# zhizdev/mvdfusion

Measured on AMD Instinct MI355X. Metric: denoising-steps/sec, higher is better.
Workload: dtype f16x3 (f16 MFMA operands split hi+lo, 3 partial products, fp32 accumulate); 1 GPU; BASELINE.json configs[1]: V=4 views x 256^2 images (32x32 latents), D=1, 50-step DDIM (eta 1), cfg 2.5, SD1.x UNet 320ch + 10 view-aligned transformers + GridAttn, random-init (deterministic fill) weights; views=4, latent=32, depth_samples=1, parallelism=single GPU, CFG pair batched as 2V, hipgraph=True, gemm_tuning=mvdfusion_amd/tuned/gemm_f16.json: 426 problems; 0 problems tuned in this run

## Files before the change

include/mvd_hip.h:

```cpp
#ifndef MVD_HIP_H
#define MVD_HIP_H
#include <stddef.h>
#include <stdint.h>
#ifdef __cplusplus
extern "C" {
#endif

typedef void* mvd_stream_t;

#define MVD_VERSION 100
#define MVD_PREC_X1 1
#define MVD_PREC_X3 3
#define MVD_PREC_X4 4

int mvd_version(void);
const char* mvd_last_error(void);
int mvd_operand_format(void);

size_t mvd_packed_weight_bytes(int N, int K);
int mvd_pack_linear_weight(const float* w, int N, int K, int ldw, int geglu, float scale, void* packed,
                           mvd_stream_t stream);
int mvd_pack_linear_weight_t(const float* wt, int N, int K, int ldw, float scale, void* packed, mvd_stream_t stream);
int mvd_pack_conv3x3_weight(const float* w, int Cout, int Cin, int cin_pad, float scale, void* packed,
                            mvd_stream_t stream);
// ... 51 lines not shown
  int ldr;
  void *q_hi, *q_lo, *k_hi, *k_lo, *vt_hi, *vt_lo;
  int heads, dhead, L, Lpad;
  float qscale;
  int splitk;
  float* workspace;
  size_t workspace_elems;
  int cfg;
  long long* gn_stats;
  int gn_hw, gn_groups;
  float* rs_out;
  int* rs_count;
  int rs_ld;
  const float* ln_stats;
  const int* ln_count;
  const float* ln_colsum;
  int ln_ld, ln_dim;
  float ln_eps;
  void* gna_out_sp;
  const float* gna_gamma;
  const float* gna_beta;
  float gna_eps;
  int gna_flags;
  const float* cat_b;
  int cat_cb;
  void* cat_raw_sp;
  const float* acc_scale_dev;
  const struct mvd_prefetch_item_s* pf_items;
  int pf_n;
  int tap_mode;
  const void* A2;
  int lda2, Cin2;
} mvd_gemm_desc;
#define MVD_TAPS_FULL 0
#define MVD_TAPS_UP4 1
#define MVD_TAPS_CENTRE_TAIL 2
#define MVD_GNA_SILU 1
#define MVD_GNA_ROUND_F16 2
#define MVD_GNA_OUT_UNUSED 4

int mvd_gemm(const mvd_gemm_desc* d, mvd_stream_t stream);
int mvd_gemm_cfg_supported(const mvd_gemm_desc* d, int cfg);

int mvd_split_planes(const float* x, void* sp, size_t rows, int cols, int ldx, int ldp, mvd_stream_t stream);
int mvd_split_planes_scaled(const float* x, void* sp, size_t rows, int cols, int ldx, int ldp, const float* scale_dev, mvd_stream_t stream);

int mvd_gemv(const float* W, const float* bias, const float* x, float* y, int M, int N, int K, int ldx, int ldy,
             int act_in, int act_out, mvd_stream_t stream);

int mvd_groupnorm_chunks(int HW);
int mvd_groupnorm_nhwc(const float* x, void* y_sp, const float* gamma, const float* beta, int B, int HW, int C,
                       int groups, float eps, int silu, double* ws, size_t ws_elems, mvd_stream_t stream);
int mvd_groupnorm_from_stats(const float* x, void* y_sp, const float* gamma, const float* beta, const long long* stats, int B, int HW,
                             int C, int groups, float eps, int silu, mvd_stream_t stream);
int mvd_softmax_rows(const float* x, void* y_sp, int rows, int cols, int ldx, float scale, float out_scale,
                     mvd_stream_t stream);

int mvd_layernorm(const float* x, void* y_sp, float* y_f32, const float* w, const float* b, int rows, int C, float eps,
                  int w_plus_one, mvd_stream_t stream);
int mvd_layernorm_groups(const float* x, void* y_sp, float* y_f32, const float* w, const float* b, int ldw, int rows, int rows_per_group,
                         int C, float eps, int w_plus_one, mvd_stream_t stream);

size_t mvd_attn_qk_plane_elems(int B, int heads, int L, int dhead);
size_t mvd_attn_vt_plane_elems(int B, int heads, int L, int dhead);
int mvd_attn_lpad(int L);
int mvd_attention(const void* q_hi, const void* q_lo, const void* k_hi, const void* k_lo, const void* vt_hi,
                  const void* vt_lo, void* out_sp, int ldo, int B, int heads, int L, int Lkeys, int dhead, int prec,
                  mvd_stream_t stream);

int mvd_pixel_cross_attn(const float* q, const float* k, const float* v, void* out_sp, int P, int D, int heads,
                         int dhead, mvd_stream_t stream);

int mvd_unet_input(const float* x, const float* input_latents, void* out_sp, int V, int S, int cpad, int cfg,
                   mvd_stream_t stream);
int mvd_unet_input_scenes(const float* x, const float* input_latents, void* out_sp, int nscene, int V, int S, int cpad, int cfg,
                          mvd_stream_t stream);
int mvd_concat_channels(const float* a, int Ca, const float* b, int Cb, float* out, void* out_sp, int rows, long long* gn_stats,
                        int gn_hw, int gn_groups, mvd_stream_t stream);
int mvd_concat_groupnorm_fits(int Ca, int Cb, int hw, int groups);
int mvd_concat_groupnorm(const float* a, int Ca, const float* b, int Cb, float* out, void* raw_sp, void* y_sp, const float* gamma,
                         const float* beta, long long* gn_stats, int B, int hw, int groups, float eps, int silu, mvd_stream_t stream);
int mvd_area_pool(const float* vol, void* out_sp, int B, int S, int D, int C, int factor, int ldp, mvd_stream_t stream);
int mvd_fill_zero(float* p, size_t n, mvd_stream_t stream);

#define MVD_STEP_STRIDE 8
int mvd_timestep_embedding(const float* steps, const int* iter, const float* freqs, float* out, int dim,
                           mvd_stream_t stream);
int mvd_timestep_embedding_scenes(const float* steps, const int* iter, const float* freqs, float* out, int dim, int nscene,
                                  int steps_scene_stride, mvd_stream_t stream);
int mvd_advance_iter(int* iter, mvd_stream_t stream);

#define MVD_CAM_RECORD 20
#define MVD_TOKEN_DIM 723
#define MVD_TOKEN_LD 736
int mvd_zembed(const float* lat, const float* w, const float* b, float* feat, int N, int S, mvd_stream_t stream);
int mvd_gridattn_tokens(const float* x, const float* depth_noise, const float* steps, const int* iter,
                        const float* grid_lin ,
                        const float* feat, const float* in_feat, const float* cams, const float* in_cam,
                        void* tokens_sp, int V, int q0, int Vq, int S, int D, float depth_scale, float depth_shift,
                        mvd_stream_t stream);
int mvd_gridattn_tokens_scenes(const float* x, const float* depth_noise, const float* steps, const int* iter, const float* grid_lin,
                               const float* feat, const float* in_feat, const float* cams, const float* in_cam, void* tokens_sp,
                               int nscene, int V, int q0, int Vq, int S, int D, float depth_scale, float depth_shift,
                               mvd_stream_t stream);
int mvd_gridattn_tokens_scenes_t(const float* x, const float* depth_noise, const float* steps, const int* iter, const float* grid_lin,
                                 const float* feat, const float* in_feat, const float* cams, const float* in_cam, void* tokens_sp,
                                 int nscene, int V, int q0, int Vq, int S, int D, float depth_scale, float depth_shift,
                                 int steps_scene_stride, mvd_stream_t stream);
int mvd_gridattn_fused_slots(void);
size_t mvd_gridattn_fused_stream_bytes(void);
size_t mvd_gridattn_fused_vec_floats(void);
int mvd_gridattn_fused(const float* x, const float* depth_noise, const float* steps, const int* iter, const float* grid_lin,
                       const float* feat, const float* in_feat, const float* cams, const float* in_cam, const void* wstream,
                       const float* vecs, void* pooled_sp, int V, int q0, int Vq, int S, int D, float depth_scale,
                       float depth_shift, int prec ,
                       mvd_stream_t stream);
int mvd_gridattn_fused_scenes(const float* x, const float* depth_noise, const float* steps, const int* iter, const float* grid_lin,
                              const float* feat, const float* in_feat, const float* cams, const float* in_cam, const void* wstream,
                              const float* vecs, void* pooled_sp, int nscene, int V, int q0, int Vq, int S, int D, float depth_scale,
                              float depth_shift, int prec, mvd_stream_t stream);
int mvd_gridattn_fused_scenes_t(const float* x, const float* depth_noise, const float* steps, const int* iter, const float* grid_lin,
                                const float* feat, const float* in_feat, const float* cams, const float* in_cam, const void* wstream,
                                const float* vecs, void* pooled_sp, int nscene, int V, int q0, int Vq, int S, int D, float depth_scale,
                                float depth_shift, int prec, int steps_scene_stride, int vecs_scene_stride, mvd_stream_t stream);
int mvd_gridattn_tokens_window(const float* x, const float* depth_noise, const float* steps, const int* iter, const float* grid_lin,
                               const float* feat, const float* in_feat, const float* cams, const float* in_cam, void* tokens_sp,
                               int nscene, int V, int q0, int Vq, int S, int D, float depth_scale, float depth_shift,
                               int steps_scene_stride, int window, mvd_stream_t stream);
int mvd_gridattn_fused_window(const float* x, const float* depth_noise, const float* steps, const int* iter, const float* grid_lin,
                              const float* feat, const float* in_feat, const float* cams, const float* in_cam, const void* wstream,
                              const float* vecs, void* pooled_sp, int nscene, int V, int q0, int Vq, int S, int D, float depth_scale,
                              float depth_shift, int prec, int steps_scene_stride, int vecs_scene_stride, int window,
                              mvd_stream_t stream);
int mvd_view_mha(const float* qkv, void* out_sp, int Nseq, int V, int heads, int dhead,
                 mvd_stream_t stream);
int mvd_view_pool(const float* x, const float* w, const float* b, void* out_sp, int Nseq, int V, int C,
                  mvd_stream_t stream);

int mvd_cfg_ddim_update(const float* eps_nhwc, int ldc, float* x, float* x0, float* eps_out,
                        const float* ddim_noise, size_t noise_stride ,
                        const float* steps, const int* iter, int V, int S, int cfg, float cfg_scale, int do_update,
                        mvd_stream_t stream);

int mvd_pin_views(float* x, float* x0, const float* known, const float* noise, size_t noise_stride ,
                  const float* steps, const int* iter, int groups, int group_views, int K, int S, int mode, mvd_stream_t stream);

#define MVD_FUSE_FOREGROUND 1
#define MVD_FUSE_STAGE_AUTO 0
#define MVD_FUSE_STAGE_GLOBAL 1
#define MVD_FUSE_STAGE_LDS 2
int mvd_fuse_points(const float* lat, const float* rgb, const float* cams, const float* ndc_lin, float* xyz, float* color,
                    uint8_t* support, uint8_t* conflict, uint8_t* flags, int nscene, int V, int S, int up, float depth_scale,
                    float depth_shift, float lo, float hi, float tau, int stage, mvd_stream_t stream);
size_t mvd_compact_points_scratch(size_t npts);
int mvd_compact_points(const float* xyz, const float* color, const uint8_t* support, const uint8_t* conflict, const uint8_t* flags,
                       size_t npts, int min_support, int max_conflicts, float* out_xyz, float* out_color, uint8_t* out_support,
                       int* out_index, unsigned* count, void* scratch, size_t scratch_bytes, mvd_stream_t stream);

int mvd_graph_begin(mvd_stream_t stream);
int mvd_graph_end(mvd_stream_t stream, void** graph_exec);
int mvd_graph_launch(void* graph_exec, mvd_stream_t stream);
int mvd_graph_destroy(void* graph_exec);
int mvd_event_create(void** ev);
int mvd_event_record(void* ev, mvd_stream_t stream);
int mvd_event_elapsed_ms(void* start, void* stop, float* ms);
int mvd_event_destroy(void* ev);
// ... 49 lines not shown
```

mvdfusion_amd/csrc/elementwise.hip:

```cpp
#include "common.hpp"
#include "../../include/mvd_hip.h"

namespace {

__device__ __forceinline__ float act_apply(float v, int act) {
  if (act == MVD_ACT_GELU) return gelu_erf(v);
  if (act == MVD_ACT_SILU) return silu_f(v);
  return v;
}

template <int MR>
__global__ __launch_bounds__(256) void gemv_kernel(const float* __restrict__ W, const float* __restrict__ bias,
                                                   const float* __restrict__ x, float* __restrict__ y, int M, int N, int K, int ldx,
                                                   int ldy, int act_in, int act_out) {
  const int lane = threadIdx.x & 63;
  const int n = blockIdx.x * 4 + (threadIdx.x >> 6);
  if (n >= N) return;
  float acc[MR];
#pragma unroll
  for (int m = 0; m < MR; ++m) acc[m] = 0.f;
  const float* wr = W + (size_t)n * K;
  if ((K & 3) == 0) {
    for (int k = lane * 4; k < K; k += 256) {
      const float4 w4 = *(const float4*)(wr + k);
#pragma unroll
      for (int m = 0; m < MR; ++m) {
        if (m < M) {
          float4 x4 = *(const float4*)(x + (size_t)m * ldx + k);
          if (act_in) {
            x4.x = act_apply(x4.x, act_in);
            x4.y = act_apply(x4.y, act_in);
            x4.z = act_apply(x4.z, act_in);
            x4.w = act_apply(x4.w, act_in);
          }
          acc[m] += w4.x * x4.x + w4.y * x4.y + w4.z * x4.z + w4.w * x4.w;
        }
      }
    }
  } else {
    for (int k = lane; k < K; k += 64) {
      const float w1 = wr[k];
#pragma unroll
      for (int m = 0; m < MR; ++m)
        if (m < M) acc[m] += w1 * act_apply(x[(size_t)m * ldx + k], act_in);
    }
  }
#pragma unroll
  for (int m = 0; m < MR; ++m) {
    if (m < M) {
      float v = wave_sum(acc[m]);
      if (lane == 0) {
        if (bias) v += bias[n];
        y[(size_t)m * ldy + n] = act_apply(v, act_out);
      }
    }
  }
}

__global__ __launch_bounds__(256) void unet_input_kernel(const float* __restrict__ x, const float* __restrict__ il,
                                                         u16* __restrict__ out_sp, int V, int Vs, int S, int cpad, int nb) {
  const int SS = S * S;
  const size_t total = (size_t)nb * SS * cpad;
  for (size_t e = (size_t)blockIdx.x * 256 + threadIdx.x; e < total; e += (size_t)gridDim.x * 256) {
    const int c = (int)(e % cpad);
    const int pix = (int)((e / cpad) % SS);
    const int b = (int)(e / ((size_t)cpad * SS));
    const int v = b < V ? b : b - V;
    float o = 0.f;
    if (c < 5) {
      o = x[((size_t)v * 5 + c) * SS + pix];
    } else if (c < 10 && b < V) {
      const float t = il[((size_t)(b / Vs) * 5 + (c - 5)) * SS + pix];
      o = (c < 9) ? t / 0.18215f : t;
    }
    store_sp1(out_sp, e / cpad, cpad, c, o);
  }
}

__global__ __launch_bounds__(256) void concat_kernel(const float4* __restrict__ a, int ca4, const float4* __restrict__ b, int cb4,
                                                     float4* __restrict__ out, u16* __restrict__ out_sp, size_t rows) {
  const int c4 = ca4 + cb4;
  const size_t total = rows * c4;
  for (size_t e = (size_t)blockIdx.x * 256 + threadIdx.x; e < total; e += (size_t)gridDim.x * 256) {
    const size_t r = e / c4;
    const int c = (int)(e - r * c4);
    const float4 v = c < ca4 ? a[r * ca4 + c] : b[r * cb4 + (c - ca4)];
    out[e] = v;
    if (out_sp) store_sp4(out_sp, r, c4 * 4, c * 4, v.x, v.y, v.z, v.w);
  }
}

__global__ __launch_bounds__(256) void concat_stats_kernel(const float4* __restrict__ a, int ca4, const float4* __restrict__ b, int cb4,
                                                           float4* __restrict__ out, u16* __restrict__ out_sp, long long* __restrict__ stats,
                                                           int hw, int groups) {
  __shared__ float cs[2][4][256];
  const int c4n = ca4 + cb4, C = c4n * 4;
  const size_t m0 = (size_t)blockIdx.x * 16;
  const int n0 = blockIdx.y * 256;
  const int c4 = blockIdx.y * 64 + (threadIdx.x & 63), rg = threadIdx.x >> 6;
  float4 s = make_float4(0.f, 0.f, 0.f, 0.f), q = make_float4(0.f, 0.f, 0.f, 0.f);
  if (c4 < c4n) {
    float4 v[4];
#pragma unroll
    for (int r = 0; r < 4; ++r) {
      const size_t row = m0 + rg * 4 + r;
      v[r] = c4 < ca4 ? a[row * ca4 + c4] : b[row * cb4 + (c4 - ca4)];
    }
#pragma unroll
    for (int r = 0; r < 4; ++r) {
      const size_t row = m0 + rg * 4 + r;
      out[row * c4n + c4] = v[r];
      if (out_sp) store_sp4(out_sp, row, C, c4 * 4, v[r].x, v[r].y, v[r].z, v[r].w);
      s.x += v[r].x; s.y += v[r].y; s.z += v[r].z; s.w += v[r].w;
      q.x += v[r].x * v[r].x; q.y += v[r].y * v[r].y; q.z += v[r].z * v[r].z; q.w += v[r].w * v[r].w;
    }
  }
  *(float4*)&cs[0][rg][(threadIdx.x & 63) * 4] = s;
  *(float4*)&cs[1][rg][(threadIdx.x & 63) * 4] = q;
  __syncthreads();
  const int c = threadIdx.x, nn = n0 + c;
  const float cs_ = cs[0][0][c] + cs[0][1][c] + cs[0][2][c] + cs[0][3][c];
  const float cq_ = cs[1][0][c] + cs[1][1][c] + cs[1][2][c] + cs[1][3][c];
  __syncthreads();
  cs[0][0][c] = cs_;
  cs[1][0][c] = cq_;
  __syncthreads();
  if (nn >= C) return;
  const int cg = C / groups;
  const int g = nn / cg, pos = nn - g * cg;
  if (c != 0 && pos != 0) return;
  int len = cg - pos;
  if (len > 256 - c) len = 256 - c;
  float ss = 0.f, qq = 0.f;
  for (int j = 0; j < len; ++j) {
    ss += cs[0][0][c + j];
    qq += cs[1][0][c + j];
  }
  gn_stats_add(stats, (int)(m0 / hw), g, groups, ss, qq);
}

#define MVD_CGN_THREADS 1024
__global__ __launch_bounds__(MVD_CGN_THREADS) void concat_gn_kernel(const float* __restrict__ a, int ca, const float* __restrict__ b, int cb,
                                                                    float* __restrict__ out, u16* __restrict__ raw_sp, u16* __restrict__ y_sp,
                                                                    const float* __restrict__ gamma, const float* __restrict__ beta,
                                                                    long long* __restrict__ stats, int hw, int groups, float eps, int flags) {
  constexpr int NT = MVD_CGN_THREADS, NWV = NT / 64, U = 4;
  extern __shared__ float s_val[];
  __shared__ double s_red[2][NWV];
  __shared__ float s_coef[2][128];
  const int C = ca + cb, cg = C / groups, cg2 = cg >> 1;
  int g, img;
  {
    const int bid = blockIdx.x;
    if ((groups & 7) == 0) {
      const int gpx = groups >> 3, x = bid & 7, r = bid >> 3;
      g = x * gpx + r % gpx;
      img = r / gpx;
    } else {
      g = bid % groups;
// ... 27 lines not shown
        }
      }
#pragma unroll
      for (int u = 0; u < U; ++u) {
        const size_t m = m0 + rr[u];
        const int n = c0 + 2 * jj[u];
        v[u] = *(const float2*)(n < ca ? a + m * ca + n : b + m * cb + (n - ca));
      }
#pragma unroll
      for (int u = 0; u < U; ++u) {
        if (ok[u]) {
          const size_t m = m0 + rr[u];
          const int n = c0 + 2 * jj[u];
          if (out) *(float2*)(out + m * C + n) = v[u];
          if (raw_sp) {
            uint32_t hh, ll;
            split_op16x2(v[u].x, v[u].y, hh, ll);
            u16* pp = raw_sp + sp_index(m, C, n);
            *(uint32_t*)pp = hh;
            *(uint32_t*)(pp + 32) = ll;
          }
          *(float2*)(s_val + 2 * (e0 + u * NT)) = v[u];
          s += v[u].x + v[u].y;
          q += v[u].x * v[u].x + v[u].y * v[u].y;
        }
      }
    }
  }
  {
    const double sd = wave_sum_d((double)s), qd = wave_sum_d((double)q);
    if (lane == 0) {
      s_red[0][wave] = sd;
      s_red[1][wave] = qd;
    }
  }
  __syncthreads();
  double S1 = 0.0, S2 = 0.0;
#pragma unroll
  for (int w = 0; w < NWV; ++w) {
    S1 += s_red[0][w];
    S2 += s_red[1][w];
  }
  const double cnt = (double)hw * cg;
  const double mean = S1 / cnt;
  double var = S2 / cnt - mean * mean;
  if (var < 0.0) var = 0.0;
  const float rstd = (float)(1.0 / sqrt(var + (double)eps));
  if (tid < cg) {
    const float aa = rstd * gamma[c0 + tid];
    s_coef[0][tid] = aa;
    s_coef[1][tid] = beta[c0 + tid] - (float)mean * aa;
  }
  if (tid == 0 && stats) gn_stats_add(stats, img, g, groups, (float)S1, (float)S2);
  __syncthreads();
  {
    int r = rs, j = js;
    for (int e = tid; e < total; e += NT) {
      float2 v = *(const float2*)(s_val + 2 * e);
      v.x = v.x * s_coef[0][2 * j] + s_coef[1][2 * j];
      v.y = v.y * s_coef[0][2 * j + 1] + s_coef[1][2 * j + 1];
      if (flags & 2) {
        v.x = (float)(_Float16)v.x;
        v.y = (float)(_Float16)v.y;
      }
      if (flags & 1) {
        v.x = silu_f(v.x);
        v.y = silu_f(v.y);
      }
      uint32_t hh, ll;
      split_op16x2(v.x, v.y, hh, ll);
      u16* pp = y_sp + sp_index(m0 + r, C, c0 + 2 * j);
      *(uint32_t*)pp = hh;
      *(uint32_t*)(pp + 32) = ll;
      r += dq;
      j += dj;
      if (j >= cg2) {
        j -= cg2;
        ++r;
      }
    }
  }
}

__global__ __launch_bounds__(256) void area_pool_kernel(const float4* __restrict__ vol, u16* __restrict__ out_sp, int B, int S,
                                                        int D, int C4, int f, int ldp) {
  const int So = S / f;
  const size_t total = (size_t)B * So * So * D * C4;
  const float inv = 1.0f / (float)(f * f);
  for (size_t e = (size_t)blockIdx.x * 256 + threadIdx.x; e < total; e += (size_t)gridDim.x * 256) {
    const int c = (int)(e % C4);
    size_t r = e / C4;
    const int d = (int)(r % D);
    r /= D;
    const int ox = (int)(r % So);
    r /= So;
    const int oy = (int)(r % So);
    const int b = (int)(r / So);
    float4 acc = make_float4(0.f, 0.f, 0.f, 0.f);
    for (int dy = 0; dy < f; ++dy)
#pragma unroll 8
      for (int dx = 0; dx < f; ++dx) {
        const float4 v = vol[((((size_t)b * S + oy * f + dy) * S + ox * f + dx) * D + d) * C4 + c];
        acc.x += v.x;
        acc.y += v.y;
        acc.z += v.z;
        acc.w += v.w;
      }
    store_sp4(out_sp, e / C4, ldp, c * 4, acc.x * inv, acc.y * inv, acc.z * inv, acc.w * inv);
  }
}

__global__ __launch_bounds__(256) void fill_zero_kernel(float* p, size_t n) {
  for (size_t e = (size_t)blockIdx.x * 256 + threadIdx.x; e < n; e += (size_t)gridDim.x * 256) p[e] = 0.f;
}

__global__ void timestep_embedding_kernel(const float* __restrict__ steps, const int* __restrict__ iter,
                                          const float* __restrict__ freqs, float* __restrict__ out, int dim, int steps_scene_stride) {
  const float t = steps[((size_t)iter[0] + (size_t)blockIdx.x * steps_scene_stride) * MVD_STEP_STRIDE + 0];
  out += (size_t)blockIdx.x * dim;
  const int half = dim / 2;
  for (int i = threadIdx.x; i < half; i += blockDim.x) {
    const float a = t * freqs[i];
    out[i] = cosf(a);
    out[half + i] = sinf(a);
  }
}

__global__ void advance_iter_kernel(int* iter) {
  if (threadIdx.x == 0) iter[0] += 1;
}

__global__ __launch_bounds__(256) void cfg_ddim_kernel(const float* __restrict__ eps_nhwc, int ldc, float* __restrict__ x,
                                                       float* __restrict__ x0, float* __restrict__ eps_out,
                                                       const float* __restrict__ noise, const float* __restrict__ steps,
                                                       const int* __restrict__ iter, int V, int S, int cfg, float cfg_scale,
                                                       int do_update, size_t noise_stride) {
  const int it = iter[0];
  const float* st = steps + (size_t)it * MVD_STEP_STRIDE;
  const float a_t = st[3], a_prev = st[4], sigma = st[5], s1m = st[6], has_noise = st[7];
  const int SS = S * S;
  const size_t total = (size_t)V * 5 * SS;
  for (size_t e = (size_t)blockIdx.x * 256 + threadIdx.x; e < total; e += (size_t)gridDim.x * 256) {
    const int pix = (int)(e % SS);
    const int c = (int)((e / SS) % 5);
    const int b = (int)(e / ((size_t)5 * SS));
    float ep = eps_nhwc[((size_t)b * SS + pix) * ldc + c];
    if (cfg) {
      const float eu = eps_nhwc[((size_t)(V + b) * SS + pix) * ldc + c];
      ep = eu + cfg_scale * (ep - eu);
    }
    if (eps_out) eps_out[e] = ep;
    if (do_update) {
      const float xv = x[e];
      const float px0 = (xv - s1m * ep) / sqrtf(a_t);
      const float dir = sqrtf(fmaxf(1.0f - a_prev - sigma * sigma, 1e-7f)) * ep;
      float xp = sqrtf(a_prev) * px0 + dir;
      if (has_noise != 0.f) xp = xp + sigma * noise[(size_t)it * noise_stride + e];
      x0[e] = px0;
      x[e] = xp;
    }
  }
}

template <typename T>
__device__ __forceinline__ T pin_axpy(float sa, const T& k, float s1, const T& n);
template <>
__device__ __forceinline__ float pin_axpy<float>(float sa, const float& k, float s1, const float& n) {
  return sa * k + s1 * n;
}
template <>
__device__ __forceinline__ float4 pin_axpy<float4>(float sa, const float4& k, float s1, const float4& n) {
  return make_float4(sa * k.x + s1 * n.x, sa * k.y + s1 * n.y, sa * k.z + s1 * n.z, sa * k.w + s1 * n.w);
}

template <typename T>
__global__ __launch_bounds__(256) void pin_views_kernel(T* __restrict__ x, T* __restrict__ x0, const T* __restrict__ known,
                                                        const T* __restrict__ noise, size_t nstride, const float* __restrict__ steps,
                                                        const int* __restrict__ iter, int group_views, int K, size_t rowlen, size_t total,
                                                        int mode) {
  float sa = 1.f, s1 = 0.f;
  size_t nbase = 0;
  if (mode == 1) {
    const int it = iter[0];
    const float* st = steps + (size_t)it * MVD_STEP_STRIDE;
    sa = st[1];
    s1 = st[6];
    nbase = (size_t)it * nstride;
  }
  for (size_t e = (size_t)blockIdx.x * 256 + threadIdx.x; e < total; e += (size_t)gridDim.x * 256) {
    const size_t p = e / rowlen;
    const size_t off = e - p * rowlen;
    const size_t dst = ((p / K) * group_views + p % K) * rowlen + off;
    const T kv = known[e];
    if (mode == 1) {
      x[dst] = pin_axpy<T>(sa, kv, s1, noise[nbase + e]);
      x0[dst] = kv;
// ... 33 lines not shown
  MVD_CHECK_ARG(x && input_latents && out_sp && cpad % 32 == 0 && V > 0 && S > 0 && cpad >= 10, "mvd_unet_input: bad arguments");
  MVD_CHECK_ARG(nscene >= 1 && (long long)nscene * V <= 0x3fffffff, "mvd_unet_input_scenes: nscene=%d (>= 1)", nscene);
  const int NV = nscene * V;
  const int nb = cfg ? 2 * NV : NV;
  const size_t total = (size_t)nb * S * S * cpad;
  hipLaunchKernelGGL(unet_input_kernel, dim3(grid_for(total)), dim3(256), 0, (hipStream_t)stream, x, input_latents, (u16*)out_sp, NV, V,
                     S, cpad, nb);
  MVD_CHECK_LAUNCH("mvd_unet_input");
  return 0;
}

extern "C" int mvd_unet_input(const float* x, const float* input_latents, void* out_sp, int V, int S, int cpad, int cfg,
                              mvd_stream_t stream) {
  return mvd_unet_input_scenes(x, input_latents, out_sp, 1, V, S, cpad, cfg, stream);
}

extern "C" int mvd_concat_channels(const float* a, int Ca, const float* b, int Cb, float* out, void* out_sp, int rows,
                                   long long* gn_stats, int gn_hw, int gn_groups, mvd_stream_t stream) {
  if (out_sp) MVD_CHECK_ARG((Ca + Cb) % 32 == 0, "mvd_concat_channels: split-planes output needs (Ca+Cb) %% 32 == 0");
  MVD_CHECK_ARG(a && b && out && rows > 0 && Ca > 0 && Cb > 0 && Ca % 4 == 0 && Cb % 4 == 0,
                "mvd_concat_channels: bad arguments (channel counts must be multiples of 4)");
  if (gn_stats) {
    MVD_CHECK_ARG(rows % 16 == 0 && gn_hw > 0 && gn_hw % 16 == 0 && gn_groups > 0 && (Ca + Cb) % gn_groups == 0,
                  "mvd_concat_channels: gn_stats needs rows %% 16 == 0, gn_hw %% 16 == 0, C %% groups == 0");
    hipLaunchKernelGGL(concat_stats_kernel, dim3(rows / 16, (Ca + Cb + 255) / 256), dim3(256), 0, (hipStream_t)stream, (const float4*)a, Ca / 4,
                       (const float4*)b, Cb / 4, (float4*)out, (u16*)out_sp, gn_stats, gn_hw, gn_groups);
    MVD_CHECK_LAUNCH("mvd_concat_channels/stats");
    return 0;
  }
  const size_t total = (size_t)rows * (Ca + Cb) / 4;
  hipLaunchKernelGGL(concat_kernel, dim3(grid_for(total)), dim3(256), 0, (hipStream_t)stream, (const float4*)a, Ca / 4,
                     (const float4*)b, Cb / 4, (float4*)out, (u16*)out_sp, (size_t)rows);
  MVD_CHECK_LAUNCH("mvd_concat_channels");
  return 0;
}

extern "C" int mvd_concat_groupnorm_fits(int Ca, int Cb, int hw, int groups) {
  const int C = Ca + Cb;
  if (groups <= 0 || C % groups || (Ca & 1) || (Cb & 1)) return 0;
  const int cg = C / groups;
  return (cg & 1) == 0 && cg <= 128 && (size_t)hw * cg * 4 <= 128 * 1024 ? 1 : 0;
}

extern "C" int mvd_concat_groupnorm(const float* a, int Ca, const float* b, int Cb, float* out, void* raw_sp, void* y_sp, const float* gamma,
                                    const float* beta, long long* gn_stats, int B, int hw, int groups, float eps, int silu,
                                    mvd_stream_t stream) {
  MVD_CHECK_ARG(a && b && y_sp && gamma && beta && B > 0 && hw > 0, "mvd_concat_groupnorm: null pointer / bad shape");
  MVD_CHECK_ARG((Ca + Cb) % 32 == 0 && mvd_concat_groupnorm_fits(Ca, Cb, hw, groups),
                "mvd_concat_groupnorm: needs (Ca+Cb) %% 32 == 0, even Ca / Cb / group width <= 128 and hw * (C / groups) * 4 <= 128 KiB of LDS "
                "(Ca=%d Cb=%d hw=%d groups=%d): use mvd_concat_channels + mvd_groupnorm_from_stats", Ca, Cb, hw, groups);
  MVD_CHECK_ARG(((uintptr_t)a & 7) == 0 && ((uintptr_t)b & 7) == 0 && ((uintptr_t)out & 7) == 0 && ((uintptr_t)y_sp & 127) == 0 &&
                    ((uintptr_t)raw_sp & 127) == 0, "mvd_concat_groupnorm: alignment");
  const size_t lds = (size_t)hw * ((Ca + Cb) / groups) * 4;
  {
    static unsigned long long raised = 0;
    const hipError_t e = mvd_raise_dynamic_lds((const void*)concat_gn_kernel, 128 * 1024, &raised);
    MVD_CHECK_ARG(e == hipSuccess, "mvd_concat_groupnorm: hipFuncSetAttribute(MaxDynamicSharedMemorySize): %s", hipGetErrorString(e));
  }
  hipLaunchKernelGGL(concat_gn_kernel, dim3(B * groups), dim3(MVD_CGN_THREADS), lds, (hipStream_t)stream, a, Ca, b, Cb, out, (u16*)raw_sp,
                     (u16*)y_sp, gamma, beta, gn_stats, hw, groups, eps, silu);
  MVD_CHECK_LAUNCH("mvd_concat_groupnorm");
  return 0;
}

extern "C" int mvd_area_pool(const float* vol, void* out_sp, int B, int S, int D, int C, int factor, int ldp,
                             mvd_stream_t stream) {
  MVD_CHECK_ARG(vol && out_sp && C % 32 == 0 && B > 0 && S > 0 && D > 0 && C % 4 == 0 && factor >= 1 && S % factor == 0,
                "mvd_area_pool: bad arguments");
  if (ldp == 0) ldp = C;
  MVD_CHECK_ARG(ldp >= C && ldp % 32 == 0 && ((uintptr_t)out_sp & 127) == 0, "mvd_area_pool: ldp=%d must be >= C, %% 32 == 0", ldp);
  const int So = S / factor;
  const size_t total = (size_t)B * So * So * D * (C / 4);
  hipLaunchKernelGGL(area_pool_kernel, dim3(grid_for(total)), dim3(256), 0, (hipStream_t)stream, (const float4*)vol,
                     (u16*)out_sp, B, S, D, C / 4, factor, ldp);
  MVD_CHECK_LAUNCH("mvd_area_pool");
  return 0;
}

extern "C" int mvd_fill_zero(float* p, size_t n, mvd_stream_t stream) {
  MVD_CHECK_ARG(p != nullptr, "mvd_fill_zero: null pointer");
  if (n == 0) return 0;
  hipLaunchKernelGGL(fill_zero_kernel, dim3(grid_for(n)), dim3(256), 0, (hipStream_t)stream, p, n);
  MVD_CHECK_LAUNCH("mvd_fill_zero");
  return 0;
}

extern "C" int mvd_timestep_embedding(const float* steps, const int* iter, const float* freqs, float* out, int dim,
                                      mvd_stream_t stream) {
  MVD_CHECK_ARG(steps && iter && freqs && out && dim > 0 && dim % 2 == 0, "mvd_timestep_embedding: bad arguments");
  hipLaunchKernelGGL(timestep_embedding_kernel, dim3(1), dim3(256), 0, (hipStream_t)stream, steps, iter, freqs, out, dim, 0);
  MVD_CHECK_LAUNCH("mvd_timestep_embedding");
  return 0;
}

extern "C" int mvd_timestep_embedding_scenes(const float* steps, const int* iter, const float* freqs, float* out, int dim, int nscene,
                                             int steps_scene_stride, mvd_stream_t stream) {
  MVD_CHECK_ARG(steps && iter && freqs && out && dim > 0 && dim % 2 == 0, "mvd_timestep_embedding: bad arguments");
  MVD_CHECK_ARG(nscene >= 1 && nscene <= 65535 && steps_scene_stride >= 0 && (nscene > 1 || steps_scene_stride == 0),
                "mvd_timestep_embedding_scenes: nscene=%d (1 ... 65535), steps_scene_stride=%d (>= 0; 0 when nscene = 1)", nscene,
                steps_scene_stride);
  hipLaunchKernelGGL(timestep_embedding_kernel, dim3(nscene), dim3(256), 0, (hipStream_t)stream, steps, iter, freqs, out, dim,
                     steps_scene_stride);
  MVD_CHECK_LAUNCH("mvd_timestep_embedding_scenes");
  return 0;
}

extern "C" int mvd_advance_iter(int* iter, mvd_stream_t stream) {
  MVD_CHECK_ARG(iter != nullptr, "mvd_advance_iter: null pointer");
  hipLaunchKernelGGL(advance_iter_kernel, dim3(1), dim3(64), 0, (hipStream_t)stream, iter);
  MVD_CHECK_LAUNCH("mvd_advance_iter");
  return 0;
}

extern "C" int mvd_cfg_ddim_update(const float* eps_nhwc, int ldc, float* x, float* x0, float* eps_out,
                                   const float* ddim_noise, size_t noise_stride, const float* steps, const int* iter, int V,
                                   int S, int cfg, float cfg_scale, int do_update, mvd_stream_t stream) {
  MVD_CHECK_ARG(eps_nhwc && steps && iter && V > 0 && S > 0 && ldc >= 5, "mvd_cfg_ddim_update: bad arguments");
  if (do_update) MVD_CHECK_ARG(x && x0 && ddim_noise, "mvd_cfg_ddim_update: update needs x, x0, ddim_noise");
  const size_t total = (size_t)V * 5 * S * S;
  hipLaunchKernelGGL(cfg_ddim_kernel, dim3(grid_for(total)), dim3(256), 0, (hipStream_t)stream, eps_nhwc, ldc, x, x0, eps_out,
                     ddim_noise, steps, iter, V, S, cfg, cfg_scale, do_update, noise_stride);
  MVD_CHECK_LAUNCH("mvd_cfg_ddim_update");
  return 0;
}

extern "C" int mvd_pin_views(float* x, float* x0, const float* known, const float* noise, size_t noise_stride, const float* steps,
                             const int* iter, int groups, int group_views, int K, int S, int mode, mvd_stream_t stream) {
  MVD_CHECK_ARG(x && known && groups > 0 && group_views > 0 && S > 0 && (mode == 0 || mode == 1),
                "mvd_pin_views: bad arguments (null x / known, groups=%d, group_views=%d, S=%d, mode=%d)", groups, group_views, S, mode);
  MVD_CHECK_ARG(K > 0 && K <= group_views, "mvd_pin_views: K=%d pinned views of a %d-view group (0 < K <= group_views)", K, group_views);
  MVD_CHECK_ARG((long long)groups * group_views <= 0x3fffffff, "mvd_pin_views: groups * group_views too large");
  const size_t row = (size_t)5 * S * S;
  if (mode == 1)
    MVD_CHECK_ARG(x0 && noise && steps && iter && noise_stride >= (size_t)groups * K * row,
                  "mvd_pin_views: mode 1 needs x0, noise, steps, iter and noise_stride >= groups * K * 5 * S * S");
  const size_t total = (size_t)groups * K * row;
  hipStream_t s = (hipStream_t)stream;
  if (((size_t)S * S) % 4 == 0) {
    MVD_CHECK_ARG(((uintptr_t)x & 15) == 0 && ((uintptr_t)known & 15) == 0, "mvd_pin_views: x / known must be 16-byte aligned");
    if (mode == 1)
      MVD_CHECK_ARG(((uintptr_t)x0 & 15) == 0 && ((uintptr_t)noise & 15) == 0 && noise_stride % 4 == 0,
                    "mvd_pin_views: x0 / noise must be 16-byte aligned and noise_stride a multiple of 4");
    hipLaunchKernelGGL(pin_views_kernel<float4>, dim3(grid_for(total / 4)), dim3(256), 0, s, (float4*)x, (float4*)x0, (const float4*)known,
                       (const float4*)noise, noise_stride / 4, steps, iter, group_views, K, row / 4, total / 4, mode);
  } else {
    hipLaunchKernelGGL(pin_views_kernel<float>, dim3(grid_for(total)), dim3(256), 0, s, x, x0, known, noise, noise_stride, steps, iter,
                       group_views, K, row, total, mode);
  }
  MVD_CHECK_LAUNCH("mvd_pin_views");
  return 0;
}
```

mvdfusion_amd/csrc/gemm.hip:

```cpp
#include "gemm_device.hpp"

namespace {

__global__ __launch_bounds__(256) void splitk_reduce_kernel(GemmParams p) {
  const mvd_gemm_desc& d = p.d;
  const size_t MN = (size_t)d.M * d.N;
  if (d.epi == MVD_EPI_GEGLU) {
    const size_t total = (size_t)d.M * (d.N >> 1);
    for (size_t e = (size_t)blockIdx.x * 256 + threadIdx.x; e < total; e += (size_t)gridDim.x * 256) {
      const int m = (int)(e / (d.N >> 1));
      const int col = (int)(e - (size_t)m * (d.N >> 1));
      const int pv = (col >> 4) * 32 + (col & 15);
      float v = 0.f, g = 0.f;
      for (int z = 0; z < p.splits; ++z) {
        v += d.workspace[z * MN + (size_t)m * d.N + pv];
        g += d.workspace[z * MN + (size_t)m * d.N + pv + 16];
      }
      epi_geglu_elem(d, m, pv, v, g);
    }
    return;
  }
  if (d.epi == MVD_EPI_STORE) {
    const size_t MN4 = MN >> 2;
    const float inv = 1.0f / gemm_acc_scale(d);
// ... 138 lines not shown
  const int rs = tid / cg2, js = tid - rs * cg2;
  const int r0 = tid < total ? rs : 0, j0 = tid < total ? js : 0;
  const float* const zero2 = (const float*)g_zero_page;
  const bool has_bias = d.bias != nullptr, has_bb = d.bias_b != nullptr, has_res = d.res != nullptr;
  const float ascale = gemm_acc_scale(d);
  float s = 0.f, q = 0.f;
  {
    int r = rs, j = js;
    for (int e0 = tid; e0 < total; e0 += NT * U) {
      int rr[U], jj[U];
      bool ok[U];
#pragma unroll
      for (int u = 0; u < U; ++u) {
        ok[u] = e0 + u * NT < total;
        rr[u] = ok[u] ? r : r0;
        jj[u] = ok[u] ? j : j0;
        r += dq;
        j += dj;
        if (j >= cg2) {
          j -= cg2;
          ++r;
        }
      }
      float2 acc[U], tb[U], tbb[U], tr[U];
      float2 t[ZC][U];
      const int nz0 = p.splits < ZC ? p.splits : ZC;
      bool own[U];
      float2 tc[U];
#pragma unroll
      for (int u = 0; u < U; ++u) {
        const int m = m0 + rr[u], nn = c0 + 2 * jj[u];
        own[u] = nn < d.N;
        const int n = own[u] ? nn : 0;
        tb[u] = *(const float2*)(has_bias ? d.bias + n : zero2);
        tbb[u] = *(const float2*)(has_bb ? d.bias_b + (size_t)(m / d.rows_per_batch) * d.ldbb + n : zero2);
        tr[u] = *(const float2*)(has_res ? d.res + (size_t)m * d.ldr + n : zero2);
        tc[u] = *(const float2*)(own[u] ? zero2 : d.cat_b + (size_t)m * d.cat_cb + (nn - d.N));
#pragma unroll
        for (int z = 0; z < ZC; ++z) {
          const float* w = d.workspace + (size_t)(z < nz0 ? z : 0) * MN + (size_t)m * d.N + n;
          t[z][u] = *(const float2*)w;
        }
      }
#pragma unroll
      for (int u = 0; u < U; ++u) {
        acc[u] = make_float2(0.f, 0.f);
#pragma unroll
        for (int z = 0; z < ZC; ++z)
          if (z < nz0) {
            acc[u].x += t[z][u].x;
            acc[u].y += t[z][u].y;
          }
      }
      for (int zb = ZC; zb < p.splits; zb += ZC) {
        const int nz = p.splits - zb < ZC ? p.splits - zb : ZC;
#pragma unroll
        for (int u = 0; u < U; ++u) {
          const int m = m0 + rr[u], n = own[u] ? c0 + 2 * jj[u] : 0;
#pragma unroll
          for (int z = 0; z < ZC; ++z) t[z][u] = *(const float2*)(d.workspace + (size_t)(zb + (z < nz ? z : 0)) * MN + (size_t)m * d.N + n);
        }
#pragma unroll
        for (int u = 0; u < U; ++u)
#pragma unroll
          for (int z = 0; z < ZC; ++z)
            if (z < nz) {
              acc[u].x += t[z][u].x;
              acc[u].y += t[z][u].y;
            }
      }
#pragma unroll
      for (int u = 0; u < U; ++u) {
        float2 v = acc[u];
        v.x = v.x * ascale + tb[u].x + tbb[u].x + tr[u].x;
        v.y = v.y * ascale + tb[u].y + tbb[u].y + tr[u].y;
        if (!own[u]) v = tc[u];
        if (ok[u]) {
          const int m = m0 + rr[u], n = c0 + 2 * jj[u];
          if (put_out && own[u]) *(float2*)(d.out + (size_t)m * d.ldo + n) = v;
          if (d.cat_raw_sp) {
            uint32_t hh, ll;
            split_op16x2(v.x, v.y, hh, ll);
            u16* pp = (u16*)d.cat_raw_sp + sp_index((size_t)m, CT, n);
            *(uint32_t*)pp = hh;
            *(uint32_t*)(pp + 32) = ll;
          }
          *(float2*)(s_val + 2 * (e0 + u * NT)) = v;
          s += v.x + v.y;
          q += v.x * v.x + v.y * v.y;
        }
      }
    }
  }
  unsigned pf_sink = 0;
  if (d.pf_items != nullptr) {
    const __attribute__((address_space(4))) mvd_prefetch_item* tab = (const __attribute__((address_space(4))) mvd_prefetch_item*)d.pf_items;
    const int gw = blockIdx.x * NWV + wave, GW = gridDim.x * NWV;
    for (int it = 0; it < d.pf_n; ++it) {
      const unsigned char* base = (const unsigned char*)tab[it].ptr;
      const long lines = (long)((tab[it].bytes + 127) >> 7);
      for (long l = (long)gw * 64 + lane; l < lines; l += (long)GW * 64) {
        const unsigned char* a = base + (l << 7);
        asm volatile("global_load_dword %0, %1, off" : "+v"(pf_sink) : "v"(a) : "memory");
      }
    }
  }
  {
    const double sd = wave_sum_d((double)s), qd = wave_sum_d((double)q);
    if (lane == 0) {
      s_red[0][wave] = sd;
      s_red[1][wave] = qd;
    }
  }
  __syncthreads();
  double S1 = 0.0, S2 = 0.0;
#pragma unroll
  for (int w = 0; w < NWV; ++w) {
    S1 += s_red[0][w];
    S2 += s_red[1][w];
  }
  const double cnt = (double)HW * cg;
  const double mean = S1 / cnt;
  double var = S2 / cnt - mean * mean;
  if (var < 0.0) var = 0.0;
  const float rstd = (float)(1.0 / sqrt(var + (double)d.gna_eps));
  if (tid < cg) {
    const float a = rstd * d.gna_gamma[c0 + tid];
    s_coef[0][tid] = a;
    s_coef[1][tid] = d.gna_beta[c0 + tid] - (float)mean * a;
  }
  if (tid == 0 && d.gn_stats) gn_stats_add(d.gn_stats, b, g, G, (float)S1, (float)S2);
  __syncthreads();
  u16* const ysp = (u16*)d.gna_out_sp;
  const int fl = d.gna_flags;
  {
    int r = rs, j = js;
    for (int e = tid; e < total; e += NT) {
      float2 v = *(const float2*)(s_val + 2 * e);
      v.x = v.x * s_coef[0][2 * j] + s_coef[1][2 * j];
      v.y = v.y * s_coef[0][2 * j + 1] + s_coef[1][2 * j + 1];
      if (fl & MVD_GNA_ROUND_F16) {
        v.x = (float)(_Float16)v.x;
        v.y = (float)(_Float16)v.y;
      }
      if (fl & MVD_GNA_SILU) {
        v.x = silu_f(v.x);
        v.y = silu_f(v.y);
      }
      uint32_t hh, ll;
      split_op16x2(v.x, v.y, hh, ll);
      u16* pp = ysp + sp_index((size_t)(m0 + r), CT, c0 + 2 * j);
      *(uint32_t*)pp = hh;
      *(uint32_t*)(pp + 32) = ll;
      r += dq;
      j += dj;
      if (j >= cg2) {
        j -= cg2;
        ++r;
      }
    }
  }
  asm volatile("" ::"v"(pf_sink));
}

struct TileInfo {
  int bm, bn, waves;
// ... 143 lines not shown
  }
  if (d.gn_stats)
    MVD_CHECK_ARG(d.epi == MVD_EPI_STORE && d.n_store == d.N && d.M % 16 == 0 && d.gn_hw > 0 && d.gn_hw % 16 == 0 && d.gn_groups > 0 &&
                      d.N % d.gn_groups == 0,
                  "mvd_gemm: gn_stats needs MVD_EPI_STORE, n_store == N, M %% 16 == 0, gn_hw %% 16 == 0, N %% gn_groups == 0 (N=%d M=%d hw=%d)",
                  d.N, d.M, d.gn_hw);
  if (d.gna_out_sp)
    MVD_CHECK_ARG(d.gn_stats && d.out && d.ldo == d.N && d.gna_gamma && d.gna_beta && d.N % 32 == 0 && d.M % d.gn_hw == 0 &&
                      ((uintptr_t)d.gna_out_sp & 127) == 0,
                  "mvd_gemm: gna_out_sp (GroupNorm apply behind the GEMM) needs gn_stats, out with ldo == N, gamma / beta, N %% 32 == 0, M %% gn_hw == 0");
  if (d.cat_b)
    MVD_CHECK_ARG(d.gna_out_sp && d.cat_cb > 0 && d.cat_cb % 2 == 0 && (d.N + d.cat_cb) % 32 == 0 && (d.N + d.cat_cb) % d.gn_groups == 0 &&
                      ((uintptr_t)d.cat_b & 7) == 0 && ((uintptr_t)d.cat_raw_sp & 127) == 0 &&
                      mvd_concat_groupnorm_fits(d.N, d.cat_cb, d.gn_hw, d.gn_groups),
                  "mvd_gemm: cat_b (GroupNorm over [out | cat_b]) needs gna_out_sp, an even cat_cb, (N + cat_cb) %% 32 == 0 and a shape "
                  "mvd_concat_groupnorm_fits() accepts (N=%d cat_cb=%d hw=%d)", d.N, d.cat_cb, d.gn_hw);
  long long* const gna_stats = d.gn_stats;
  if (d.cat_b) d.gn_stats = nullptr;
  if (d.b_mode == MVD_B_PLANES)
    MVD_CHECK_ARG(d.ldb >= d.K && d.ldb % 32 == 0, "mvd_gemm: B planes need ldb=%d >= K=%d, a multiple of 32", d.ldb, d.K);
  else
    MVD_CHECK_ARG(d.b_mode == MVD_B_PACKED, "mvd_gemm: bad b_mode %d", d.b_mode);
  if (d.acc_scale == 0.f) d.acc_scale = 1.f;
  p.nk = d.K / 32;
  p.nt16 = d.N / 16;
  int tile, loop = 0, order = -1;
  MVD_CHECK_ARG(d.cfg >= 0 && d.cfg <= MVD_GEMM_CFG_STRIDE * MVD_GEMM_TILES, "mvd_gemm: bad cfg %d", d.cfg);
  if (d.cfg >= 1) {
    tile = (d.cfg - 1) / MVD_GEMM_CFG_STRIDE;
    loop = ((d.cfg - 1) % MVD_GEMM_CFG_STRIDE) >> 1;
    order = (d.cfg - 1) & 1;
    MVD_CHECK_ARG(cfg_supported(d, d.cfg), "mvd_gemm: cfg %d (tile %d, loop %d) does not serve this problem (include/mvd_hip.h: cfg)", d.cfg, tile,
                  loop);
  } else {
    const long tiles128 = (long)cdiv(d.M, 128) * cdiv(d.N, 128);
    tile = (tiles128 >= 128 && (d.N >= 512 || d.K >= 2048)) ? 1 : 0;
  }
  const TileInfo& ti = kTiles[tile];
  p.tiles_n = cdiv(d.N, ti.bn);
  p.tiles_m = cdiv(d.M, ti.bm);
  const bool up4 = d.a_mode == MVD_A_CONV3X3 && d.tap_mode == MVD_TAPS_UP4;
  if (up4) {
    p.up4_mq = d.B * d.Hin * d.Win;
    p.up4_tpp = cdiv(p.up4_mq, ti.bm);
    p.tiles_m = 4 * p.up4_tpp;
  }
  if (order < 0) {
    const int est_tm = up4 ? p.up4_tpp : p.tiles_m;
    const double W = (double)d.N * d.K * 4.0;
    const double A = (double)(up4 ? p.up4_mq : d.M) * d.K * 4.0 / (d.a_mode == MVD_A_CONV3X3 ? (up4 ? 4.0 : 9.0) : 1.0);
    const double rep_m = est_tm < 8 ? est_tm : 8, rep_n = p.tiles_n < 8 ? p.tiles_n : 8;
    order = (W + A * rep_n) < (W * rep_m + A) ? 1 : 0;
  }
  p.m_fastest = order;
  int splits = d.splitk;
  const long tiles = (long)p.tiles_m * p.tiles_n;
  if (splits == 0) splits = choose_splits(tiles, p.nk, ti, loop, (size_t)d.M * d.N);
  if (splits < 1) splits = 1;
  if (splits > p.nk) splits = p.nk;
  if (splits > 1) {
    if (d.workspace == nullptr) splits = 1;
    else {
      const size_t cap = d.workspace_elems / ((size_t)d.M * d.N);
      if ((size_t)splits > cap) splits = cap < 1 ? 1 : (int)cap;
    }
  }
  p.kt_per_split = cdiv(p.nk, splits);
  if (loop == 6) p.kt_per_split = 9 * cdiv(p.nk / 9, splits);
  p.splits = cdiv(p.nk, p.kt_per_split);
  hipStream_t s = (hipStream_t)stream;
  bool launched;
  if (loop == 6) launched = mvd_gemm_launch_patch(tile, p, s, patch_shares(d, ti));
  else if (loop == 7) launched = mvd_gemm_launch_ws(tile, p, s);
  else if (tile == 0) launched = mvd_gemm_launch_plain_t0(loop, p, s);
  else if (tile == 1) launched = mvd_gemm_launch_plain_t1(loop, p, s);
  else if (tile == 2) launched = mvd_gemm_launch_plain_t2(loop, p, s);
  else if (tile == 3) launched = mvd_gemm_launch_plain_t3(loop, p, s);
  else launched = mvd_gemm_launch_plain_t4(loop, p, s);
  MVD_CHECK_ARG(launched, "mvd_gemm: no kernel for tile %d loop %d", tile, loop);
  MVD_CHECK_LAUNCH("mvd_gemm");
  const int gna_ct = d.N + (d.cat_b ? d.cat_cb : 0);
  const int gna_cg = d.gna_out_sp ? gna_ct / d.gn_groups : 0;
  const size_t gna_lds = (size_t)d.gn_hw * gna_cg * 4;
  const bool gna_fused = d.gna_out_sp && p.splits > 1 && !d.rs_out && !d.out_sp && !d.colscale && d.act == MVD_ACT_NONE && (gna_cg & 1) == 0 &&
                         gna_cg <= 128 && gna_lds <= 128 * 1024 && d.ldo % 2 == 0 && (!d.res || d.ldr % 2 == 0) && (!d.bias_b || d.ldbb % 2 == 0) &&
                         d.N % 2 == 0;
  if (gna_fused) {
    {
      static unsigned long long raised = 0;
      const hipError_t e = mvd_raise_dynamic_lds((const void*)splitk_gn_kernel, 128 * 1024, &raised);
      MVD_CHECK_ARG(e == hipSuccess, "mvd_gemm: hipFuncSetAttribute(MaxDynamicSharedMemorySize): %s", hipGetErrorString(e));
    }
    p.d.gn_stats = gna_stats;
    if (loop == 7) p.d.pf_items = nullptr;
    hipLaunchKernelGGL(splitk_gn_kernel, dim3((d.M / d.gn_hw) * d.gn_groups), dim3(MVD_GNK_THREADS), gna_lds, s, p);
    MVD_CHECK_LAUNCH("mvd_gemm/splitk_gn");
    return 0;
  }
  if (p.splits > 1) {
    if (d.rs_out) {
      hipLaunchKernelGGL(splitk_reduce_rows_kernel, dim3(cdiv(d.M, 4), cdiv(d.N, 256)), dim3(256), 0, s, p);
    } else if (d.gn_stats) {
      const int spans = (d.N + 255) / 256;
      if ((d.M / 16) * spans >= 1024)
        hipLaunchKernelGGL(splitk_reduce_stats_kernel<4>, dim3(d.M / 16, spans), dim3(256), 0, s, p);
      else
        hipLaunchKernelGGL(splitk_reduce_stats_kernel<2>, dim3(d.M / 8, spans), dim3(256), 0, s, p);
    } else {
      const size_t total = (size_t)d.M * d.N;
      int blocks = (int)((total + 255) / 256);
      if (blocks > 2048) blocks = 2048;
      hipLaunchKernelGGL(splitk_reduce_kernel, dim3(blocks), dim3(256), 0, s, p);
    }
    MVD_CHECK_LAUNCH("mvd_gemm/splitk_reduce");
  }
  if (d.gna_out_sp && d.cat_b)
    return mvd_concat_groupnorm(d.out, d.N, d.cat_b, d.cat_cb, nullptr, d.cat_raw_sp, d.gna_out_sp, d.gna_gamma, d.gna_beta, gna_stats,
                                d.M / d.gn_hw, d.gn_hw, d.gn_groups, d.gna_eps, d.gna_flags & (MVD_GNA_SILU | MVD_GNA_ROUND_F16), stream);
  if (d.gna_out_sp)
    return mvd_groupnorm_from_stats(d.out, d.gna_out_sp, d.gna_gamma, d.gna_beta, d.gn_stats, d.M / d.gn_hw, d.gn_hw, d.N, d.gn_groups,
                                    d.gna_eps, d.gna_flags & (MVD_GNA_SILU | MVD_GNA_ROUND_F16), stream);
  return 0;
}

namespace {
__global__ __launch_bounds__(256) void pack_kernel(const float* __restrict__ w, u16* __restrict__ out, int N, int K,
                                                   int Np, int Kp, int ldw, int geglu, int conv_cin, int trans,
                                                   float scale) {
  const int nt16 = Np >> 4;
  const size_t total = (size_t)(Kp >> 5) * nt16 * 64;
  for (size_t e = (size_t)blockIdx.x * 256 + threadIdx.x; e < total; e += (size_t)gridDim.x * 256) {
    const size_t mt = e >> 6;
    const int l = (int)(e & 63);
    const int kt = (int)(mt / nt16), nt = (int)(mt - (size_t)kt * nt16);
    const int n = nt * 16 + (l & 15);
    const int k = kt * 32 + (l >> 4) * 8;
    int src_n = n;
    if (geglu) {
      const int blk = n >> 5, within = n & 31;
      src_n = within < 16 ? blk * 16 + within : (N >> 1) + blk * 16 + (within - 16);
    }
    float v[8];
#pragma unroll
    for (int j = 0; j < 8; ++j) v[j] = 0.f;
    if (src_n < N) {
      if (conv_cin > 0) {
        const int cb = kt / 9, tap = kt - cb * 9;
        const int ci0 = cb * 32 + (k & 31);
#pragma unroll
        for (int j = 0; j < 8; ++j)
          if (ci0 + j < conv_cin) v[j] = w[((size_t)src_n * conv_cin + ci0 + j) * 9 + tap];
      } else if (trans) {
#pragma unroll
        for (int j = 0; j < 8; ++j)
          if (k + j < K) v[j] = w[(size_t)(k + j) * ldw + src_n];
      } else {
        const float* src = w + (size_t)src_n * ldw + k;
        if (k + 7 < K && (ldw & 3) == 0 && ((uintptr_t)w & 15) == 0) {
          const float4 a = *(const float4*)src, b = *(const float4*)(src + 4);
          v[0] = a.x; v[1] = a.y; v[2] = a.z; v[3] = a.w; v[4] = b.x; v[5] = b.y; v[6] = b.z; v[7] = b.w;
        } else {
#pragma unroll
          for (int j = 0; j < 8; ++j)
            if (k + j < K) v[j] = src[j];
        }
      }
    }
// ... 87 lines not shown
```

mvdfusion_amd/csrc/gridattn.hip:

```cpp
#include "gridattn_common.hpp"

namespace {

__device__ __forceinline__ float harmonic(const float* vec, int dim, int e) {
  const int n = dim * 7;
  if (e >= 2 * n) return vec[e - 2 * n];
  const int ee = e < n ? e : e - n;
  const int di = ee / 7, k = ee - di * 7;
  const float w = 0.1f * (float)(1 << k);
  const float a = vec[di] * w;
  return e < n ? sinf(a) : cosf(a);
}
__device__ __forceinline__ void embed105(const Plucker& pl, float depth, int lane, float& v0, float& v1) {
  const float p6[6] = {pl.a, pl.b, pl.c, pl.d, pl.e, pl.f}, dp[1] = {depth};
  const int e0 = lane, e1 = lane + 64;
  v0 = e0 < 90 ? harmonic(p6, 6, e0) : harmonic(dp, 1, e0 - 90);
  v1 = e1 >= 105 ? 0.f : e1 < 90 ? harmonic(p6, 6, e1) : harmonic(dp, 1, e1 - 90);
}

__global__ __launch_bounds__(256) void tokens_kernel(GridGeom g, const float* __restrict__ feat, const float* __restrict__ in_feat,
                                                     u16* __restrict__ tok) {
  const int lane = threadIdx.x & 63;
  const int S = g.S, SS = S * S, W = slots_per_point(g);
  const size_t pt = (size_t)blockIdx.x * 4 + (threadIdx.x >> 6);
  if (pt >= num_points(g)) return;
  const GeomPoint q = decode_point(g, pt, wave_scene(g, pt));
  const Cam cb = view_cam(g, q, q.b);
  float X[3], dir[3];
  const float depth = world_point(g, q, cb, X, dir);
  float qe0, qe1;
  embed105(plucker(dir[0], dir[1], dir[2], cb.C), depth, lane, qe0, qe1);
  const float4 fin = bilinear4(in_feat + (size_t)q.scene * SS * 256, view_taps(input_cam(g, q), X, S), lane * 4);
  for_each_slot(g, q.b, [&](int slot, int vr) {
    const Cam cv = view_cam(g, q, vr);
    const float4 fr = bilinear4(feat + (size_t)(q.gv0 + vr) * SS * 256, view_taps(cv, X, S), lane * 4);
    const Plucker rpl = plucker_to(cv, X);
    float re0, re1;
    embed105(rpl, rpl.norm, lane, re0, re1);
    const size_t row = pt * W + slot;
    store_sp4(tok, row, MVD_TOKEN_LD, lane * 4, fr.x, fr.y, fr.z, fr.w);
    store_sp4(tok, row, MVD_TOKEN_LD, 256 + lane * 4, fin.x, fin.y, fin.z, fin.w);
    store_sp1(tok, row, MVD_TOKEN_LD, 512 + lane, re0);
    if (lane + 64 < 105) store_sp1(tok, row, MVD_TOKEN_LD, 512 + lane + 64, re1);
    store_sp1(tok, row, MVD_TOKEN_LD, 617 + lane, qe0);
    if (lane + 64 < 105) store_sp1(tok, row, MVD_TOKEN_LD, 617 + lane + 64, qe1);
    if (lane < MVD_TOKEN_LD - 722) store_sp1(tok, row, MVD_TOKEN_LD, 722 + lane, lane == 0 ? 1.0f : 0.0f);
  });
}

__global__ __launch_bounds__(256) void zembed_kernel(const float* __restrict__ lat, const float* __restrict__ w,
                                                     const float* __restrict__ bias, float* __restrict__ feat, int N, int SS) {
  const int lane = threadIdx.x & 63;
  const size_t p = (size_t)blockIdx.x * 4 + (threadIdx.x >> 6);
  if (p >= (size_t)N * SS) return;
  const int n = (int)(p / SS), pix = (int)(p % SS);
  float in[5];
#pragma unroll
  for (int c = 0; c < 5; ++c) in[c] = lat[((size_t)n * 5 + c) * SS + pix];
  float o[4];
#pragma unroll
  for (int j = 0; j < 4; ++j) {
    const int ch = lane * 4 + j;
    float a = 0.f;
#pragma unroll
    for (int c = 0; c < 5; ++c) a += in[c] * w[ch * 5 + c];
    o[j] = gelu_erf(a + bias[ch]);
  }
  *(float4*)(feat + p * 256 + lane * 4) = make_float4(o[0], o[1], o[2], o[3]);
}

__device__ __forceinline__ void scatter4(long long* __restrict__ acc, const Taps& t, int ch, float4 g, float scale) {
#pragma unroll
  for (int k = 0; k < 4; ++k) {
    if (t.pix[k] < 0) continue;
    unsigned long long* p = (unsigned long long*)(acc + (size_t)t.pix[k] * 256 + ch);
    const float w = t.w[k] * scale;
    atomicAdd(p + 0, (unsigned long long)(long long)llrintf(g.x * w));
    atomicAdd(p + 1, (unsigned long long)(long long)llrintf(g.y * w));
    atomicAdd(p + 2, (unsigned long long)(long long)llrintf(g.z * w));
    atomicAdd(p + 3, (unsigned long long)(long long)llrintf(g.w * w));
  }
}

__global__ __launch_bounds__(256) void tokens_bwd_kernel(GridGeom g, const float* __restrict__ dtok, int ldt, long long* __restrict__ dfeat,
                                                         long long* __restrict__ din_feat, float scale) {
  const int lane = threadIdx.x & 63;
  const int S = g.S, SS = S * S, W = slots_per_point(g);
  const size_t pt = (size_t)blockIdx.x * 4 + (threadIdx.x >> 6);
  if (pt >= num_points(g)) return;
  const GeomPoint q = decode_point(g, pt, wave_scene(g, pt));
  float X[3], dir[3];
  world_point(g, q, view_cam(g, q, q.b), X, dir);
  float4 gin = make_float4(0.f, 0.f, 0.f, 0.f);
  for_each_slot(g, q.b, [&](int slot, int vr) {
    const float* row = dtok + (pt * W + slot) * (size_t)ldt;
    const float4 gr = *(const float4*)(row + lane * 4);
    scatter4(dfeat + (size_t)(q.gv0 + vr) * SS * 256, view_taps(view_cam(g, q, vr), X, S), lane * 4, gr, scale);
    const float4 gi = *(const float4*)(row + 256 + lane * 4);
    gin.x += gi.x; gin.y += gi.y; gin.z += gi.z; gin.w += gi.w;
  });
  scatter4(din_feat + (size_t)q.scene * SS * 256, view_taps(input_cam(g, q), X, S), lane * 4, gin, scale);
}

}

extern "C" int mvd_zembed(const float* lat, const float* w, const float* b, float* feat, int N, int S, mvd_stream_t stream) {
  MVD_CHECK_ARG(lat && w && b && feat && N > 0 && S > 0, "mvd_zembed: bad arguments");
  const size_t npix = (size_t)N * S * S;
  hipLaunchKernelGGL(zembed_kernel, dim3(cdiv(npix, 4)), dim3(256), 0, (hipStream_t)stream, lat, w, b, feat, N, S * S);
  MVD_CHECK_LAUNCH("mvd_zembed");
  return 0;
}

extern "C" int mvd_gridattn_tokens_window(const float* x, const float* depth_noise, const float* steps, const int* iter,
                                          const float* grid_lin, const float* feat, const float* in_feat, const float* cams,
                                          const float* in_cam, void* tokens_sp, int nscene, int V, int q0, int Vq, int S, int D,
                                          float depth_scale, float depth_shift, int steps_scene_stride, int window, mvd_stream_t stream) {
  const GridGeom g = {x, depth_noise, steps, iter, grid_lin, cams, in_cam, nscene, V, q0, Vq, S, D, depth_scale, depth_shift, steps_scene_stride, window};
  if (const int e = check_geom("mvd_gridattn_tokens_window", g)) return e;
  MVD_CHECK_ARG(feat && in_feat && tokens_sp, "mvd_gridattn_tokens_window: null pointer");
  const size_t npts = num_points(g);
  MVD_CHECK_ARG((npts + 3) / 4 <= 0x7fffffff, "mvd_gridattn_tokens_window: grid too large");
  hipLaunchKernelGGL(tokens_kernel, dim3(cdiv(npts, 4)), dim3(256), 0, (hipStream_t)stream, g, feat, in_feat, (u16*)tokens_sp);
  MVD_CHECK_LAUNCH("mvd_gridattn_tokens_window");
  return 0;
}

extern "C" int mvd_gridattn_tokens_scenes_t(const float* x, const float* depth_noise, const float* steps, const int* iter,
                                            const float* grid_lin, const float* feat, const float* in_feat, const float* cams,
                                            const float* in_cam, void* tokens_sp, int nscene, int V, int q0, int Vq, int S, int D,
                                            float depth_scale, float depth_shift, int steps_scene_stride, mvd_stream_t stream) {
  return mvd_gridattn_tokens_window(x, depth_noise, steps, iter, grid_lin, feat, in_feat, cams, in_cam, tokens_sp, nscene, V, q0, Vq, S, D,
                                    depth_scale, depth_shift, steps_scene_stride, 0, stream);
}

extern "C" int mvd_gridattn_tokens_scenes(const float* x, const float* depth_noise, const float* steps, const int* iter,
                                          const float* grid_lin, const float* feat, const float* in_feat, const float* cams,
                                          const float* in_cam, void* tokens_sp, int nscene, int V, int q0, int Vq, int S, int D,
                                          float depth_scale, float depth_shift, mvd_stream_t stream) {
  return mvd_gridattn_tokens_scenes_t(x, depth_noise, steps, iter, grid_lin, feat, in_feat, cams, in_cam, tokens_sp, nscene, V, q0, Vq, S,
                                      D, depth_scale, depth_shift, 0, stream);
}

extern "C" int mvd_gridattn_tokens(const float* x, const float* depth_noise, const float* steps, const int* iter,
                                   const float* grid_lin, const float* feat, const float* in_feat, const float* cams,
                                   const float* in_cam, void* tokens_sp, int V, int q0, int Vq, int S, int D, float depth_scale,
                                   float depth_shift, mvd_stream_t stream) {
  return mvd_gridattn_tokens_scenes(x, depth_noise, steps, iter, grid_lin, feat, in_feat, cams, in_cam, tokens_sp, 1, V, q0, Vq, S, D,
                                    depth_scale, depth_shift, stream);
}

// ... 34 lines not shown
```

mvdfusion_amd/csrc/gridattn_common.hpp:

```cpp
#pragma once
#include "common.hpp"
#include "../../include/mvd_hip.h"

namespace {

struct GridGeom {
  const float *x, *depth_noise, *steps;
  const int* iter;
  const float *grid_lin, *cams, *in_cam;
  int nscene, V, q0, Vq, S, D;
  float depth_scale, depth_shift;
  int steps_scene_stride, window;
};

__host__ __device__ inline int slots_per_point(const GridGeom& g) { return g.window ? g.window : g.V; }
__host__ __device__ inline size_t num_points(const GridGeom& g) { return (size_t)g.nscene * g.Vq * g.S * g.S * g.D; }
__host__ __device__ inline int window_view(int b, int j, int W, int V) { return ((b + j - W / 2) % V + V) % V; }

inline int check_geom(const char* fn, const GridGeom& g) {
  MVD_CHECK_ARG(g.x && g.depth_noise && g.steps && g.iter && g.grid_lin && g.cams && g.in_cam, "%s: null pointer", fn);
  MVD_CHECK_ARG(g.nscene >= 1, "%s: nscene=%d (>= 1)", fn, g.nscene);
  MVD_CHECK_ARG(g.steps_scene_stride >= 0 && (g.nscene > 1 || g.steps_scene_stride == 0),
                "%s: steps_scene_stride=%d (>= 0; 0 when nscene = 1)", fn, g.steps_scene_stride);
  MVD_CHECK_ARG(g.window == 0 || (g.window >= 1 && (g.window & 1)), "%s: window=%d (0 = all views, else odd)", fn, g.window);
  MVD_CHECK_ARG(g.V > 0 && slots_per_point(g) <= 16, "%s: %d rows per point outside [1, 16] (V=%d, window=%d)", fn, slots_per_point(g), g.V,
                g.window);
  MVD_CHECK_ARG(g.S > 1 && g.D > 0, "%s: bad shape S=%d, D=%d", fn, g.S, g.D);
  MVD_CHECK_ARG(g.q0 >= 0 && g.Vq > 0 && g.q0 + g.Vq <= g.V, "%s: bad query-view range [%d, %d) of %d", fn, g.q0, g.q0 + g.Vq, g.V);
  MVD_CHECK_ARG((size_t)g.nscene * g.V <= 0x7fffffff, "%s: grid too large", fn);
  return 0;
}

struct GeomPoint {
  int scene, b, pix, d;
  int gv0;
  size_t srow, noise;
};
__device__ __forceinline__ int wave_scene(const GridGeom& g, size_t pt) {
  return __builtin_amdgcn_readfirstlane((int)(pt / ((size_t)g.D * g.S * g.S)) / g.Vq);
}
__device__ __forceinline__ GeomPoint decode_point(const GridGeom& g, size_t pt, int scene) {
  const int SS = g.S * g.S;
  GeomPoint q;
  q.scene = scene;
  q.d = (int)(pt % g.D);
  q.pix = (int)((pt / g.D) % SS);
  q.b = g.q0 + (int)(pt / ((size_t)g.D * SS)) - scene * g.Vq;
  q.gv0 = scene * g.V;
  const int it = g.iter[0];
  q.srow = (size_t)it + (size_t)scene * g.steps_scene_stride;
  q.noise = (((size_t)it * g.nscene * g.V + q.gv0 + q.b) * g.D + q.d) * SS + q.pix;
  return q;
}

template <class F>
__device__ __forceinline__ void for_each_slot(const GridGeom& g, int b, F&& f) {
  const int W = slots_per_point(g);
  int vr = g.window ? window_view(b, 0, W, g.V) : 0;
  for (int slot = 0; slot < W; ++slot, vr = vr + 1 == g.V ? 0 : vr + 1) f(slot, vr);
}

struct Cam {
  float R[9], T[3], f[2], p[2], C[3];
};

__device__ __forceinline__ Cam load_cam(const float* rec) {
  Cam c;
#pragma unroll
  for (int i = 0; i < 9; ++i) c.R[i] = rec[i];
#pragma unroll
  for (int i = 0; i < 3; ++i) c.T[i] = rec[9 + i];
  c.f[0] = rec[12];
  c.f[1] = rec[13];
  c.p[0] = rec[14];
  c.p[1] = rec[15];
#pragma unroll
  for (int i = 0; i < 3; ++i) c.C[i] = rec[16 + i];
  return c;
}
__device__ __forceinline__ Cam view_cam(const GridGeom& g, const GeomPoint& q, int view) {
  return load_cam(g.cams + (size_t)(q.gv0 + view) * MVD_CAM_RECORD);
}
__device__ __forceinline__ Cam input_cam(const GridGeom& g, const GeomPoint& q) { return load_cam(g.in_cam + (size_t)q.scene * MVD_CAM_RECORD); }

__device__ __forceinline__ void unproject(const Cam& c, float x, float y, float d, float* w) {
  const float xc[3] = {(x - c.p[0]) * d / c.f[0] - c.T[0], (y - c.p[1]) * d / c.f[1] - c.T[1], d - c.T[2]};
#pragma unroll
// ... 99 lines not shown
```

mvdfusion_amd/engine.py:

```python
import os

import torch

from . import hip


GN_SLOTS = 256
GN_SLOT_ELEMS = 64 * 32 * 2


class Workspace:

    def __init__(self, device):
        self.device = torch.device(device)
        self.bufs = {}
        self.frozen = False

    def get(self, tag, shape, dtype=torch.float32, zero=False):
        key = (tag, tuple(int(s) for s in shape), dtype)
        t = self.bufs.get(key)
        if t is None:
            assert not self.frozen, f"workspace buffer {key} requested during graph capture (the eager warm-up step must " \
                                    "allocate every buffer the captured step uses)"
            t = (torch.zeros if zero else torch.empty)(key[1], dtype=dtype, device=self.device)
            self.bufs[key] = t
        return t

    def planes(self, tag, rows, cols):
        assert cols % 32 == 0, (tag, cols)
        return self.get(tag, (rows, 2 * cols), torch.int16)

    def attn_planes(self, B, heads, L, dhead):
        key = ("attn_planes", B, heads, L, dhead)
        t = self.bufs.get(key)
        if t is None:
            assert not self.frozen, f"attention planes {key} requested during graph capture"
            t = hip.alloc_attn_planes(B, heads, L, dhead, self.device)
            self.bufs[key] = t
        return t

    def nbytes(self):
        n = 0
        for v in self.bufs.values():
            for t in (v if isinstance(v, tuple) else (v,)):
                n += t.numel() * t.element_size()
        return n


class Ctx:
    gn_from_producer = True
    ln_fold = True
    gn_fuse = True

    def __init__(self, device, prec=hip.PREC_X4, policy=None):
        self.device = torch.device(device)
        self.ws = Workspace(device)
        self.prec = prec
        self.policy = dict(policy or {})
        self.B = 0
        self.D = 1
        self.context = None
        self.vol_levels = None
        self.emb_bias = None
        self._rot = {}
        self.capturing = False
        self.gemm_ws = torch.empty(64 * 1024 * 1024, dtype=torch.float32, device=self.device)
        self.gn_arena = torch.zeros(GN_SLOTS * GN_SLOT_ELEMS, dtype=torch.int64, device=self.device)
        self._gn_next = 0
        self._gn = {}
        self._rs = {}
        self.next_gn = None
        self._gn_done = {}
        self._unwritten = set()
        self.next_cat = None
        self._cat_done = set()
        self.keep_fp32 = False

    def begin_step(self):
        self._rot.clear()
        self._gn.clear()
        self._gn_done.clear()
        self._unwritten.clear()
        self._cat_done.clear()
        self.next_gn = None
        self.next_cat = None
        self._gn_next = 0
        if self.gn_from_producer:
            hip.check(hip.lib().mvd_fill_zero(hip.ptr(self.gn_arena), self.gn_arena.numel() * 2, hip.stream()))

    def gn_slot(self, out, B, HW, C):
        n = B * 32 * 2
        if n > GN_SLOT_ELEMS or self._gn_next >= GN_SLOTS:
            return None
        st = self.gn_arena[self._gn_next * GN_SLOT_ELEMS:self._gn_next * GN_SLOT_ELEMS + n]
        self._gn_next += 1
        self._gn[out.data_ptr()] = (st, B, HW, C)
        return st

    def _forget(self, out):
        ptr = out.data_ptr()
        self._gn.pop(ptr, None)
        self._unwritten.discard(ptr)
        if self._gn_done:
            for k in [k for k in self._gn_done if k[0] == ptr]:
                del self._gn_done[k]

    def row_stats(self, tag, rows, width):
        key = (tag, int(rows), int(width))
        rs = self._rs.get(key)
        if rs is None:
            assert not self.ws.frozen, f"row statistics {key} requested during graph capture"
            rs = hip.RowStats(rows, width, self.device)
            self._rs[key] = rs
        return rs

    def act(self, shape):
        key = tuple(int(s) for s in shape)
        i = self._rot.get(key, 0)
        self._rot[key] = (i + 1) % 3
        return self.ws.get(f"act{i}", key)

    def prec_of(self, kind):
        return self.policy.get(kind, self.prec)

    def ln_fold_enabled(self):
        return (self.ln_fold and hip.OPERAND_FORMAT == "f16" and self.prec_of("qkv") >= hip.PREC_X3 and
                self.prec_of("geglu") >= hip.PREC_X3 and self.prec_of("proj") >= hip.PREC_X3)

    def gemm(self, A, W, out, gn=None, kind=None, gn_apply=None, **kw):
        kw.setdefault("prec", self.prec_of(kind))
        kw.setdefault("workspace", self.gemm_ws)
        applied = False
        if out is not None:
            self._forget(out)
            handled = False
            if gn is not None and gn_apply is None and self.next_cat is not None and self.gn_fuse and self.gn_from_producer and \
                    gn[1] % 16 == 0 and out.is_contiguous():
                sk, cat, catp, norm, pname, silu = self.next_cat
                N, cb = out.shape[-1], sk.shape[-1]
                if norm.num_groups == 32 and norm.num_channels == N + cb and sk.shape[0] == out.shape[0] == gn[0] * gn[1] and \
                        sk.is_contiguous() and hip.lib().mvd_concat_groupnorm_fits(N, cb, gn[1], 32):
                    st = self.gn_slot(cat, gn[0], gn[1], N + cb)
                    if st is not None:
                        planes = self.ws.planes(pname, out.shape[0], N + cb)
                        kw.update(gn_stats=st, gn_hw=gn[1], gn_groups=32, cat=(sk, catp),
                                  gn_apply=(norm.weight, norm.bias, norm.eps, (hip.GNA_SILU if silu else 0) | hip.GNA_OUT_UNUSED, planes))
                        self._gn.pop(cat.data_ptr(), None)
                        self._gn_done[(cat.data_ptr(), id(norm))] = (planes, bool(silu))
                        self._unwritten.add(cat.data_ptr())
                        self._unwritten.add(out.data_ptr())
                        self._cat_done.add(cat.data_ptr())
                        handled = True
            if not handled and gn is not None and self.gn_from_producer and gn[1] % 16 == 0 and out.shape[-1] % 32 == 0:
                st = self.gn_slot(out, gn[0], gn[1], out.shape[-1])
                if st is not None:
                    kw.update(gn_stats=st, gn_hw=gn[1], gn_groups=32)
                    if gn_apply is not None and self.gn_fuse and gn_apply[0].num_groups == 32 and out.is_contiguous():
                        norm, planes, silu, unused = gn_apply
                        kw["gn_apply"] = (norm.weight, norm.bias, norm.eps, (hip.GNA_SILU if silu else 0) | (hip.GNA_OUT_UNUSED if unused else 0),
                                          planes)
                        applied = True
                    elif gn_apply is None and self.next_gn is not None and self.gn_fuse and out.is_contiguous():
                        norm, pname, silu = self.next_gn
                        if norm.num_groups == 32 and norm.num_channels == out.shape[-1] and out.shape[0] == gn[0] * gn[1]:
                            planes = self.ws.planes(pname, out.shape[0], out.shape[-1])
                            kw["gn_apply"] = (norm.weight, norm.bias, norm.eps, hip.GNA_SILU if silu else 0, planes)
                            self._gn_done[(out.data_ptr(), id(norm))] = (planes, bool(silu))
        if gn is not None:
            if os.environ.get("MVD_GN_DEBUG") and not self.capturing:
                print(f"[gn] kind={kind} M={out.shape[0]} N={out.shape[-1]} explicit={gn_apply is not None} hint={self.next_gn is not None} "
                      f"cat={self.next_cat is not None} -> fused_apply={'gn_apply' in kw} cat={'cat' in kw}", flush=True)
            if gn_apply is None:
                self.next_gn = None
                self.next_cat = None
        r = hip.gemm(A, W, out, **kw)
        if gn_apply is not None and not applied:
            self.groupnorm(out, gn_apply[1], gn_apply[0], gn[0], gn[1], out.shape[-1], gn_apply[2])
        return r

    def groupnorm(self, x, y, norm, B, HW, C, silu):
        done = self._gn_done.pop((x.data_ptr(), id(norm)), None)
        if done is not None and done[0].data_ptr() == y.data_ptr() and done[0].shape == y.shape and done[1] == bool(silu) and silu in (True, False):
            return y
        if x.data_ptr() in self._unwritten:
            raise RuntimeError("GroupNorm of a tensor whose fused producer left the fp32 data unwritten (Ctx.concat(need_out=False))")
        ent = self._gn.get(x.data_ptr())
        if ent is not None and ent[1:] == (B, HW, C) and norm.num_groups == 32:
            return hip.groupnorm_from_stats(x, y, norm.weight, norm.bias, ent[0], B, HW, C, norm.eps, silu)
        ws = self.ws.get("gn_ws", (B * hip.lib().mvd_groupnorm_chunks(HW) * 32 * 2,), torch.float64)
        return hip.groupnorm(x, y, norm.weight, norm.bias, B, HW, C, norm.eps, silu, ws)

    def concat(self, a, ca, b, cb, out, out_planes, B, HW, gn_apply=None, need_out=True):
        self._forget(out)
        st = None
        if gn_apply is not None and self.gn_fuse and self.gn_from_producer and HW % 16 == 0 and (ca + cb) % 32 == 0 and \
                gn_apply[0].num_groups == 32 and gn_apply[0].num_channels == ca + cb and \
                hip.lib().mvd_concat_groupnorm_fits(ca, cb, HW, 32):
            norm, pname, silu = gn_apply
            st = self.gn_slot(out, B, HW, ca + cb)
            planes = self.ws.planes(pname, B * HW, ca + cb)
            hip.check(hip.lib().mvd_concat_groupnorm(hip.ptr(a), ca, hip.ptr(b), cb, hip.ptr(out) if need_out else None, hip.ptr(out_planes),
                                                     hip.ptr(planes), hip.ptr(norm.weight), hip.ptr(norm.bias),
                                                     hip.ptr(st) if st is not None else None, B, HW, 32, norm.eps, 1 if silu else 0,
                                                     hip.stream()))
            if not need_out:
                self._gn.pop(out.data_ptr(), None)
                self._unwritten.add(out.data_ptr())
            self._gn_done[(out.data_ptr(), id(norm))] = (planes, bool(silu))
            return out
        if self.gn_from_producer and HW % 16 == 0 and (ca + cb) % 32 == 0:
            st = self.gn_slot(out, B, HW, ca + cb)
        hip.check(hip.lib().mvd_concat_channels(hip.ptr(a), ca, hip.ptr(b), cb, hip.ptr(out), hip.ptr(out_planes), B * HW,
                                                hip.ptr(st) if st is not None else None, HW, 32, hip.stream()))
        return out

    def layernorm(self, x, y, norm, rows, C):
        return hip.layernorm(x, y, norm.weight, norm.bias, rows, C, norm.eps)

    def gemv_rows(self, W, bias, x, y, act_in=hip.ACT_NONE, act_out=hip.ACT_NONE):
        for r in range(0, x.shape[0], 16):
            hip.gemv(W, bias, x[r:r + 16], y[r:r + 16], act_in, act_out)
        return y


def ddim_step_table(scheduler_tables, ddim, iters):
    rows = []
    for index in iters:
        t = int(ddim["timesteps"][index])
        sac = float(scheduler_tables["sqrt_alphas_cumprod"][t])
        s1m = float(scheduler_tables["sqrt_one_minus_alphas_cumprod"][t])
        dstd = (scheduler_tables["sqrt_one_minus_alphas_cumprod"][t] / scheduler_tables["sqrt_alphas_cumprod"][t] / 10.0)
        rows.append([float(t), sac, float(dstd), float(ddim["alphas"][index]), float(ddim["alphas_prev"][index]),
                     float(ddim["sigmas"][index]), float(ddim["sqrt_one_minus_alphas"][index]),
                     1.0 if index > 0 else 0.0])
        del s1m
    return torch.tensor(rows, dtype=torch.float32)
```

mvdfusion_amd/hip.py:

```python
import ctypes as C
import os

import torch

_HERE = os.path.dirname(os.path.abspath(__file__))
LIB_PATHS = {"f16": os.path.join(_HERE, "csrc", "libmvd_hip.so"), "bf16": os.path.join(_HERE, "csrc", "libmvd_hip_bf16.so")}
if os.environ.get("MVD_HIP_LIB"):
    LIB_PATHS["f16"] = os.environ["MVD_HIP_LIB"]
LIB_PATH = LIB_PATHS["f16"]
OPERAND_FORMAT = os.environ.get("MVD_OPERAND_FORMAT", "f16")

PREC_X1, PREC_X3, PREC_X4 = 1, 3, 4
PREC_KINDS = ("conv", "skip", "proj", "qkv", "attn", "out", "geglu", "ffproj", "xattn", "ga")


def parse_precision(name):
    base, _, over = name.partition(":")
    names = {"f16": ("f16", PREC_X1), "bf16": ("bf16", PREC_X1), "f16x3": ("f16", PREC_X3), "f16x4": ("f16", PREC_X4),
             "bf16x3": ("bf16", PREC_X3), "bf16x4": ("bf16", PREC_X4)}
    if base not in names:
        raise ValueError(f"precision '{name}': base must be one of {sorted(names)}")
    fmt, default = names[base]
    policy = {}
    for item in filter(None, over.split(",")):
        k, _, v = item.partition("=")
        k = k.strip()
        if k not in PREC_KINDS or int(v) not in (PREC_X1, PREC_X3, PREC_X4):
            raise ValueError(f"precision policy '{name}': '{item}' is not <kind>=<1|3|4> with kind in {PREC_KINDS}")
        policy[k] = int(v)
    return fmt, default, policy
A_DENSE, A_CONV3X3 = 0, 1
TAPS_FULL, TAPS_CENTRE_TAIL = 0, 2
TAPS_UP4 = 1
EPI_STORE, EPI_GEGLU, EPI_QKV = 0, 1, 2
ACT_NONE, ACT_GELU, ACT_SILU, ACT_QUICKGELU = 0, 1, 2, 3
STEP_STRIDE = 8
CAM_RECORD = 20
TOKEN_DIM, TOKEN_LD = 723, 736
FUSE_FOREGROUND = 1
FUSE_STAGE_AUTO, FUSE_STAGE_GLOBAL, FUSE_STAGE_LDS = 0, 1, 2

_vp, _i, _f, _sz = C.c_void_p, C.c_int, C.c_float, C.c_size_t
c_void_p = C.c_void_p


class GemmDesc(C.Structure):
    _fields_ = [
        ("M", _i), ("N", _i), ("K", _i),
        ("A", _vp), ("lda", _i), ("a_mode", _i),
        ("B", _i), ("Hin", _i), ("Win", _i), ("Cin", _i), ("Hout", _i), ("Wout", _i), ("stride", _i), ("upsample", _i), ("no_pad_tl", _i),
        ("Wp", _vp), ("b_mode", _i), ("ldb", _i), ("acc_scale", _f), ("prec", _i),
        ("epi", _i), ("act", _i), ("out", _vp), ("ldo", _i), ("out_sp", _vp), ("ldp", _i),
        ("n_store", _i),
        ("bias", _vp), ("bias_b", _vp), ("rows_per_batch", _i), ("ldbb", _i), ("colscale", _vp), ("res", _vp), ("ldr", _i),
        ("q_hi", _vp), ("q_lo", _vp), ("k_hi", _vp), ("k_lo", _vp), ("vt_hi", _vp), ("vt_lo", _vp),
        ("heads", _i), ("dhead", _i), ("L", _i), ("Lpad", _i), ("qscale", _f),
        ("splitk", _i), ("workspace", _vp), ("workspace_elems", _sz), ("cfg", _i),
        ("gn_stats", _vp), ("gn_hw", _i), ("gn_groups", _i),
        ("rs_out", _vp), ("rs_count", _vp), ("rs_ld", _i),
        ("ln_stats", _vp), ("ln_count", _vp), ("ln_colsum", _vp), ("ln_ld", _i), ("ln_dim", _i), ("ln_eps", _f),
        ("gna_out_sp", _vp), ("gna_gamma", _vp), ("gna_beta", _vp), ("gna_eps", _f), ("gna_flags", _i),
        ("cat_b", _vp), ("cat_cb", _i), ("cat_raw_sp", _vp),
        ("acc_scale_dev", _vp), ("pf_items", _vp), ("pf_n", _i),
        ("tap_mode", _i), ("A2", _vp), ("lda2", _i), ("Cin2", _i),
    ]


class PrefetchItem(C.Structure):
    _fields_ = [("ptr", _vp), ("bytes", C.c_ulonglong), ("start_after", _i), ("consumer", _i)]


SIGNATURES = {
    "mvd_version": (_i, []),
    "mvd_last_error": (C.c_char_p, []),
    "mvd_packed_weight_bytes": (_sz, [_i, _i]),
    "mvd_operand_format": (_i, []),
    "mvd_pack_linear_weight": (_i, [_vp, _i, _i, _i, _i, _f, _vp, _vp]),
    "mvd_pack_linear_weight_t": (_i, [_vp, _i, _i, _i, _f, _vp, _vp]),
    "mvd_pack_conv3x3_weight": (_i, [_vp, _i, _i, _i, _f, _vp, _vp]),
    "mvd_gemm": (_i, [C.POINTER(GemmDesc), _vp]),
    "mvd_gemm_cfg_supported": (_i, [C.POINTER(GemmDesc), _i]),
    "mvd_split_planes": (_i, [_vp, _vp, _sz, _i, _i, _i, _vp]),
    "mvd_gemv": (_i, [_vp, _vp, _vp, _vp, _i, _i, _i, _i, _i, _i, _i, _vp]),
    "mvd_groupnorm_chunks": (_i, [_i]),
    "mvd_groupnorm_nhwc": (_i, [_vp, _vp, _vp, _vp, _i, _i, _i, _i, _f, _i, _vp, _sz, _vp]),
    "mvd_layernorm": (_i, [_vp, _vp, _vp, _vp, _vp, _i, _i, _f, _i, _vp]),
    "mvd_layernorm_groups": (_i, [_vp, _vp, _vp, _vp, _vp, _i, _i, _i, _i, _f, _i, _vp]),
    "mvd_softmax_rows": (_i, [_vp, _vp, _i, _i, _i, _f, _f, _vp]),
    "mvd_attn_qk_plane_elems": (_sz, [_i, _i, _i, _i]),
    "mvd_attn_vt_plane_elems": (_sz, [_i, _i, _i, _i]),
    "mvd_attn_lpad": (_i, [_i]),
    "mvd_attention": (_i, [_vp] * 7 + [_i, _i, _i, _i, _i, _i, _i, _vp]),
    "mvd_pixel_cross_attn": (_i, [_vp, _vp, _vp, _vp, _i, _i, _i, _i, _vp]),
    "mvd_unet_input": (_i, [_vp, _vp, _vp, _i, _i, _i, _i, _vp]),
    "mvd_unet_input_scenes": (_i, [_vp, _vp, _vp, _i, _i, _i, _i, _i, _vp]),
    "mvd_concat_channels": (_i, [_vp, _i, _vp, _i, _vp, _vp, _i, _vp, _i, _i, _vp]),
    "mvd_concat_groupnorm_fits": (_i, [_i, _i, _i, _i]),
    "mvd_concat_groupnorm": (_i, [_vp, _i, _vp, _i, _vp, _vp, _vp, _vp, _vp, _vp, _i, _i, _i, _f, _i, _vp]),
    "mvd_transpose_planes": (_i, [_vp, _i, _i, _i, _i, _vp, _i, _vp]),
    "mvd_im2col3x3_t_planes": (_i, [_vp, _i, _i, _i, _i, _vp, _i, _vp]),
    "mvd_col_sum_workspace_doubles": (_sz, [_i, _i]),
    "mvd_col_sum": (_i, [_vp, _i, _i, _i, _vp, _vp, _sz, _vp]),
    "mvd_col_sum_groups_workspace_doubles": (_sz, [_i, _i, _i]),
    "mvd_col_sum_groups": (_i, [_vp, _i, _i, _i, _i, _vp, _vp, _sz, _vp]),
    "mvd_col_sum_pow2": (_i, [_vp, _i, _i, _i, _vp, _vp, _sz, _vp, _vp, _vp]),
    "mvd_gridattn_tokens_backward": (_i, [_vp, _vp, _vp, _vp, _vp, _vp, _vp, _vp, _i, _vp, _vp, _f, _i, _i, _i, _i, _i, _f, _f, _vp]),
    "mvd_gridattn_tokens_backward_scenes": (_i, [_vp, _vp, _vp, _vp, _vp, _vp, _vp, _vp, _i, _vp, _vp, _f, _i, _i, _i, _i, _i, _i, _f, _f, _i,
                                                 _vp]),
    "mvd_gridattn_tokens_backward_window": (_i, [_vp, _vp, _vp, _vp, _vp, _vp, _vp, _vp, _i, _vp, _vp, _f, _i, _i, _i, _i, _i, _i, _f, _f, _i,
                                                 _i, _vp]),
    "mvd_layernorm_backward": (_i, [_vp, _vp, _vp, _i, _i, _f, _vp, _vp, _vp]),
    "mvd_layernorm_backward_groups": (_i, [_vp, _vp, _vp, _i, _i, _i, _i, _f, _vp, _vp, _vp, _vp, _vp, _sz, _vp]),
    "mvd_geglu_backward": (_i, [_vp, _vp, _i, _i, _vp, _vp]),
    "mvd_act_planes": (_i, [_vp, _vp, _vp, _sz, _i, _i, _i, _i, _i, _vp]),
    "mvd_act_backward": (_i, [_vp, _vp, _vp, _sz, _i, _vp]),
    "mvd_attention_backward": (_i, [_vp, _vp, _vp, _vp, _i, _i, _i, _i, _vp, _vp, _vp, _vp, _sz, _vp]),
    "mvd_pixel_cross_attn_backward": (_i, [_vp, _vp, _vp, _vp, _i, _i, _i, _i, _vp, _vp, _vp, _vp]),
    "mvd_groupnorm_backward": (_i, [_vp, _vp, _vp, _vp, _i, _i, _i, _i, _f, _i, _vp, _vp, _vp, _vp, _sz, _vp]),
    "mvd_groupnorm_from_stats": (_i, [_vp, _vp, _vp, _vp, _vp, _i, _i, _i, _i, _f, _i, _vp]),
    "mvd_area_pool": (_i, [_vp, _vp, _i, _i, _i, _i, _i, _i, _vp]),
    "mvd_fill_zero": (_i, [_vp, _sz, _vp]),
    "mvd_pow2_scale": (_i, [_vp, _sz, _vp, _vp, _vp]),
    "mvd_split_planes_scaled": (_i, [_vp, _vp, _sz, _i, _i, _i, _vp, _vp]),
    "mvd_transpose_planes_scaled": (_i, [_vp, _i, _i, _i, _vp, _i, _vp, _vp]),
    "mvd_adamw_multi": (_i, [_vp, _i, _i, _f, _f, _f, _f, _f, _f, _f, _f, _vp]),
    "mvd_timestep_embedding": (_i, [_vp, _vp, _vp, _vp, _i, _vp]),
    "mvd_timestep_embedding_scenes": (_i, [_vp, _vp, _vp, _vp, _i, _i, _i, _vp]),
    "mvd_advance_iter": (_i, [_vp, _vp]),
    "mvd_zembed": (_i, [_vp, _vp, _vp, _vp, _i, _i, _vp]),
    "mvd_gridattn_tokens": (_i, [_vp] * 10 + [_i, _i, _i, _i, _i, _f, _f, _vp]),
    "mvd_gridattn_tokens_scenes": (_i, [_vp] * 10 + [_i, _i, _i, _i, _i, _i, _f, _f, _vp]),
    "mvd_gridattn_tokens_scenes_t": (_i, [_vp] * 10 + [_i, _i, _i, _i, _i, _i, _f, _f, _i, _vp]),
    "mvd_gridattn_fused_slots": (_i, []),
    "mvd_gridattn_fused_stream_bytes": (_sz, []),
    "mvd_gridattn_fused_vec_floats": (_sz, []),
    "mvd_gridattn_fused": (_i, [_vp] * 12 + [_i, _i, _i, _i, _i, _f, _f, _i, _vp]),
    "mvd_gridattn_fused_scenes": (_i, [_vp] * 12 + [_i, _i, _i, _i, _i, _i, _f, _f, _i, _vp]),
    "mvd_gridattn_fused_scenes_t": (_i, [_vp] * 12 + [_i, _i, _i, _i, _i, _i, _f, _f, _i, _i, _i, _vp]),
    "mvd_gridattn_tokens_window": (_i, [_vp] * 10 + [_i, _i, _i, _i, _i, _i, _f, _f, _i, _i, _vp]),
    "mvd_gridattn_fused_window": (_i, [_vp] * 12 + [_i, _i, _i, _i, _i, _i, _f, _f, _i, _i, _i, _i, _vp]),
    "mvd_view_mha": (_i, [_vp, _vp, _i, _i, _i, _i, _vp]),
    "mvd_view_pool": (_i, [_vp, _vp, _vp, _vp, _i, _i, _i, _vp]),
    "mvd_cfg_ddim_update": (_i, [_vp, _i, _vp, _vp, _vp, _vp, _sz, _vp, _vp, _i, _i, _i, _f, _i, _vp]),
    "mvd_pin_views": (_i, [_vp, _vp, _vp, _vp, _sz, _vp, _vp, _i, _i, _i, _i, _i, _vp]),
    "mvd_fuse_points": (_i, [_vp] * 9 + [_i, _i, _i, _i, _f, _f, _f, _f, _f, _i, _vp]),
    "mvd_compact_points_scratch": (_sz, [_sz]),
    "mvd_compact_points": (_i, [_vp] * 5 + [_sz, _i, _i, _vp, _vp, _vp, _vp, _vp, _vp, _sz, _vp]),
    "mvd_graph_begin": (_i, [_vp]),
    "mvd_graph_end": (_i, [_vp, C.POINTER(_vp)]),
    "mvd_graph_launch": (_i, [_vp, _vp]),
    "mvd_graph_destroy": (_i, [_vp]),
    "mvd_event_create": (_i, [C.POINTER(_vp)]),
    "mvd_event_record": (_i, [_vp, _vp]),
    "mvd_event_elapsed_ms": (_i, [_vp, _vp, C.POINTER(_f)]),
    "mvd_event_destroy": (_i, [_vp]),
}

_lib = None


def lib():
    global _lib
    if _lib is None:
        path = LIB_PATHS[OPERAND_FORMAT]
        if not os.path.exists(path):
            raise RuntimeError(
                f"{path} not found: build it with `python -m mvdfusion_amd.csrc.build` "
                "(or `python -c 'import __graft_entry__ as g; g.build()'`). mvdfusion_amd has no CPU fallback.")
        l = C.CDLL(path)
        for name, (res, args) in SIGNATURES.items():
            fn = getattr(l, name)
            fn.restype, fn.argtypes = res, args
        assert l.mvd_operand_format() == {"f16": 0xf16, "bf16": 0xbf16}[OPERAND_FORMAT]
        _lib = l
        load_default_tuned()
    return _lib


def set_operand_format(fmt):
    global OPERAND_FORMAT
    assert fmt in LIB_PATHS
    if _lib is not None and fmt != OPERAND_FORMAT:
        raise RuntimeError(f"operand format already fixed to {OPERAND_FORMAT} for this process")
    OPERAND_FORMAT = fmt


def check(rc):
    if rc != 0:
        raise RuntimeError(f"mvd_hip error {rc}: {lib().mvd_last_error().decode()}")


try:
    _raw_stream = torch._C._cuda_getCurrentRawStream
    _cur_device = torch._C._cuda_getDevice
except AttributeError:
    _raw_stream = None


def stream():
    if _raw_stream is not None:
        return C.c_void_p(_raw_stream(_cur_device()))
    return C.c_void_p(torch.cuda.current_stream().cuda_stream)


# ... 785 lines not shown
```

mvdfusion_amd/unet.py:

```python
import math

import torch
import torch.nn as nn

from . import hip
from .attention import SpatialTransformer, ViewAlignedFeatureTransformer
from .engine import Ctx


class GroupNorm32(nn.GroupNorm):
    pass


def normalization(channels):
    return GroupNorm32(32, channels)


class TimestepBlock(nn.Module):
    pass


class Upsample(nn.Module):
    def __init__(self, channels, use_conv, dims=2, out_channels=None, padding=1):
        super().__init__()
        self.channels, self.out_channels = channels, out_channels or channels
        self.conv = nn.Conv2d(self.channels, self.out_channels, 3, padding=padding)
        self._p = self._p4 = None

    def run(self, ctx, x, H, W, out=None):
        if hip.use_up4(ctx.B, H, W, training=ctx.keep_fp32):
            if self._p4 is None:
                self._p4 = hip.pack_conv3x3_up4(self.conv.weight, self.conv.bias)
            wp = self._p4
        else:
            if self._p is None:
                self._p = hip.pack_conv3x3(self.conv.weight, self.conv.bias)
            wp = self._p
        if out is None:
            out = ctx.act((ctx.B * 4 * H * W, self.out_channels))
        xp = hip.split_planes(x, ctx.ws.planes("updown.x", ctx.B * H * W, self.channels))
        ctx.gemm(xp, wp, out, conv=dict(B=ctx.B, Hin=H, Win=W, Cin=self.channels, Hout=2 * H, Wout=2 * W,
                                            stride=1, upsample=1), gn=(ctx.B, 4 * H * W), kind="conv")
        return out, 2 * H, 2 * W


class Downsample(nn.Module):
    def __init__(self, channels, use_conv, dims=2, out_channels=None, padding=1):
        super().__init__()
        self.channels, self.out_channels = channels, out_channels or channels
        self.op = nn.Conv2d(self.channels, self.out_channels, 3, stride=2, padding=padding)
        self._p = None

    def run(self, ctx, x, H, W, out=None):
        if self._p is None:
            self._p = hip.pack_conv3x3(self.op.weight, self.op.bias)
        Ho, Wo = H // 2, W // 2
        if out is None:
            out = ctx.act((ctx.B * Ho * Wo, self.out_channels))
        xp = hip.split_planes(x, ctx.ws.planes("updown.x", ctx.B * H * W, self.channels))
        ctx.gemm(xp, self._p, out, conv=dict(B=ctx.B, Hin=H, Win=W, Cin=self.channels, Hout=Ho, Wout=Wo, stride=2,
                                            upsample=0), gn=(ctx.B, Ho * Wo), kind="conv")
        return out, Ho, Wo


class ResBlock(TimestepBlock):

    def __init__(self, channels, emb_channels, dropout, out_channels=None, dims=2, use_checkpoint=False,
                 use_scale_shift_norm=False):
        super().__init__()
        assert not use_scale_shift_norm
        self.channels, self.out_channels = channels, out_channels or channels
        self.in_layers = nn.Sequential(normalization(channels), nn.SiLU(),
                                       nn.Conv2d(channels, self.out_channels, 3, padding=1))
        self.emb_layers = nn.Sequential(nn.SiLU(), nn.Linear(emb_channels, self.out_channels))
        self.out_layers = nn.Sequential(normalization(self.out_channels), nn.SiLU(), nn.Dropout(p=dropout),
                                        nn.Conv2d(self.out_channels, self.out_channels, 3, padding=1))
        self.skip_connection = nn.Identity() if self.out_channels == channels else \
            nn.Conv2d(channels, self.out_channels, 1)
        self._p = None

    def packed(self, fuse_skip=True):
        c1, c2, sk = self.in_layers[2], self.out_layers[3], self.skip_connection
        fuse = bool(fuse_skip) and not isinstance(sk, nn.Identity)
        if self._p is None:
            self._p = (hip.pack_conv3x3(c1.weight, None), None, None)
        if self._p[1] is None or bool(self._p[1].tail_cin) != fuse:
            w2 = hip.pack_conv3x3_tail(c2.weight, c2.bias, sk.weight, sk.bias) if fuse else hip.pack_conv3x3(c2.weight, c2.bias)
            wsk = None if fuse or isinstance(sk, nn.Identity) else hip.pack_linear(sk.weight, sk.bias)
            self._p = (self._p[0], w2, wsk)
        return self._p

    def run(self, ctx, x, H, W, out=None, x_planes=None):
        B, Ci, Co = ctx.B, self.channels, self.out_channels
        M = B * H * W
        w1, w2, wsk = self.packed(fuse_skip=ctx.prec_of("skip") == ctx.prec_of("conv"))
        geo = dict(B=B, Hin=H, Win=W, Hout=H, Wout=W, stride=1, upsample=0)
        a = ctx.ws.planes("res.a", M, Ci)
        ctx.groupnorm(x, a, self.in_layers[0], B, H * W, Ci, silu=True)
        h = ctx.ws.get("res.h", (M, Co))
        a2 = ctx.ws.planes("res.a2", M, Co)
        eb = ctx.emb_bias[self]
        ctx.gemm(a, w1, h, conv=dict(Cin=Ci, **geo), bias=False, bias_b=eb, rows_per_batch=M // eb.shape[0],
                 gn=(B, H * W), kind="conv",
                 gn_apply=(self.out_layers[0], a2, True, True))
        if (wsk is not None or w2.tail_cin) and x_planes is None:
            x_planes = hip.split_planes(x, ctx.ws.planes("res.xp", M, Ci))
        if out is None:
            out = ctx.act((M, Co))
        if w2.tail_cin:
            ctx.gemm(a2, w2, out, conv=dict(Cin=Co, **geo), a2=x_planes, gn=(B, H * W), kind="conv")
            return out
        skip = x
        if wsk is not None:
            skip = ctx.ws.get("res.skip", (M, Co))
            ctx.gemm(x_planes, wsk, skip, kind="skip")
        ctx.gemm(a2, w2, out, conv=dict(Cin=Co, **geo), res=skip, gn=(B, H * W), kind="conv")
        return out


def gn_hint(layer):
    from .attention import SpatialTransformer, ViewAlignedFeatureTransformer
    if isinstance(layer, tuple):
        return layer
    if isinstance(layer, ResBlock):
        return layer.in_layers[0], "res.a", True
    if isinstance(layer, SpatialTransformer):
        return layer.norm, "tf.n", False
    if isinstance(layer, ViewAlignedFeatureTransformer):
        return layer.aligned_attn_norm, "tf.n", False
    return None


class TimestepEmbedSequential(nn.Sequential, TimestepBlock):
    def run(self, ctx, x, H, W, out=None, x_planes=None, next_layer=None, next_cat=None):
        n = len(self)
        for i, layer in enumerate(self):
            dst = out if i == n - 1 else None
            ctx.next_gn = gn_hint(self[i + 1] if i + 1 < n else next_layer)
            ctx.next_cat = next_cat if i == n - 1 else None
            if isinstance(layer, (Upsample, Downsample)):
                x, H, W = layer.run(ctx, x, H, W, out=dst)
            elif isinstance(layer, ResBlock):
                x = layer.run(ctx, x, H, W, out=dst, x_planes=x_planes if i == 0 else None)
            else:
                x = layer.run(ctx, x, H, W, out=dst)
            ctx.next_gn = None
            ctx.next_cat = None
        return x, H, W


class _StemConv(nn.Conv2d):
    _p = None

    def run(self, ctx, x, H, W, out):
        if self._p is None:
            self._p = hip.pack_conv3x3(self.weight, self.bias)
        ctx.gemm(x, self._p, out, conv=dict(B=ctx.B, Hin=H, Win=W, Cin=self._p.conv_cin, Hout=H, Wout=W, stride=1,
                                            upsample=0), gn=(ctx.B, H * W), kind="conv")
        return out


class UNetModel(nn.Module):
    def __init__(self, image_size, in_channels, model_channels, out_channels, num_res_blocks, attention_resolutions,
                 dropout=0, channel_mult=(1, 2, 4, 8), conv_resample=True, dims=2, num_classes=None,
                 use_checkpoint=False, use_fp16=False, num_heads=-1, num_head_channels=-1, num_heads_upsample=-1,
                 use_scale_shift_norm=False, resblock_updown=False, use_new_attention_order=False,
                 use_spatial_transformer=True, use_view_aligned_transformer=True, transformer_depth=1,
                 context_dim=None, n_embed=None, legacy=True):
        super().__init__()
        assert use_view_aligned_transformer and use_spatial_transformer and context_dim is not None
        assert dims == 2 and num_classes is None and not resblock_updown and n_embed is None and conv_resample
        assert num_heads != -1 and num_head_channels == -1, "this build supports the num_heads form (configs/*.yaml)"
        if isinstance(context_dim, (list, tuple)) or type(context_dim).__name__ == "ListConfig":
            context_dim = list(context_dim)[0]
        channel_mult = tuple(channel_mult)
        attention_resolutions = tuple(attention_resolutions)
        self.image_size, self.in_channels, self.model_channels = image_size, in_channels, model_channels
        self.out_channels, self.num_res_blocks, self.channel_mult = out_channels, num_res_blocks, channel_mult
        self.attention_resolutions, self.num_heads, self.context_dim = attention_resolutions, num_heads, context_dim
        ted = model_channels * 4
        self.time_embed = nn.Sequential(nn.Linear(model_channels, ted), nn.SiLU(), nn.Linear(ted, ted))

        def res(cin, cout):
            return ResBlock(cin, ted, dropout, out_channels=cout, use_checkpoint=use_checkpoint)

        def st(c):
            return SpatialTransformer(c, num_heads, c // num_heads, depth=transformer_depth, context_dim=context_dim)

        def vaft(c):
            return ViewAlignedFeatureTransformer(c, num_heads, c // num_heads, depth=transformer_depth,
                                                 context_dim=context_dim, image_size=image_size)

        self.input_blocks = nn.ModuleList([TimestepEmbedSequential(_StemConv(in_channels, model_channels, 3, padding=1))])
        skip_chans = [model_channels]
        ch, ds = model_channels, 1
        for level, mult in enumerate(channel_mult):
            for _ in range(num_res_blocks):
                layers = [res(ch, mult * model_channels)]
                ch = mult * model_channels
                if ds in attention_resolutions:
                    layers.append(st(ch))
                self.input_blocks.append(TimestepEmbedSequential(*layers))
                skip_chans.append(ch)
            if level != len(channel_mult) - 1:
                self.input_blocks.append(TimestepEmbedSequential(Downsample(ch, True, out_channels=ch)))
                skip_chans.append(ch)
                ds *= 2
        self.middle_block = TimestepEmbedSequential(res(ch, ch), st(ch), vaft(ch), res(ch, ch))
        self.output_blocks = nn.ModuleList([])
        for level, mult in list(enumerate(channel_mult))[::-1]:
            for i in range(num_res_blocks + 1):
                layers = [res(ch + skip_chans.pop(), model_channels * mult)]
                ch = model_channels * mult
                if ds in attention_resolutions:
                    layers += [st(ch), vaft(ch)]
                if level and i == num_res_blocks:
                    layers.append(Upsample(ch, True, out_channels=ch))
                    ds //= 2
                self.output_blocks.append(TimestepEmbedSequential(*layers))
        self.out = nn.Sequential(normalization(ch), nn.SiLU(), nn.Conv2d(model_channels, out_channels, 3, padding=1))
        self._head = None
        self._temb = None
        self._xattn = None
        self._head_saved = None
        self._record = None

    def get_cross_attn_parameters(self, finetune_cross_attn, finetune_view_attn):
        out = []
        for name, p in self.named_parameters():
            if finetune_cross_attn and any(k in name for k in (".norm.", ".proj_in.", ".transformer_blocks.", ".proj_out.")):
                out.append(p)
            if finetune_view_attn and ".aligned_attn_" in name:
                out.append(p)
        return out

    def disable_unet_grad(self):
        for name, p in self.named_parameters():
            if ".aligned_attn_" not in name:
                p.requires_grad_(False)

    def _resblocks(self):
        return [m for m in self.modules() if isinstance(m, ResBlock)]

    def time_biases(self, ctx, t_sin):
        if self._temb is None:
            blocks = self._resblocks()
            w = torch.cat([b.emb_layers[1].weight.detach() for b in blocks], 0).contiguous()
            bias = torch.cat([b.emb_layers[1].bias.detach() + b.in_layers[2].bias.detach() for b in blocks], 0).contiguous()
            offs, o = {}, 0
            for b in blocks:
                offs[b] = (o, o + b.out_channels)
                o += b.out_channels
            self._temb = (w, bias, offs)
        w, bias, offs = self._temb
        ted = self.model_channels * 4
        R = t_sin.shape[0]
        e1, emb = ctx.ws.get("temb.e1", (R, ted)), ctx.ws.get("temb.emb", (R, ted))
        out = ctx.ws.get("temb.bias", (R, w.shape[0]))
        ctx.gemv_rows(self.time_embed[0].weight, self.time_embed[0].bias, t_sin, e1, act_out=hip.ACT_SILU)
        ctx.gemv_rows(self.time_embed[2].weight, self.time_embed[2].bias, e1, emb)
        ctx.gemv_rows(w, bias, emb, out, act_in=hip.ACT_SILU)
        ctx.emb_bias = {b: out[:, lo:hi] for b, (lo, hi) in offs.items()}

    def cross_attn_vectors(self, ctx):
        if self._xattn is None:
            sts = [m for m in self.modules() if isinstance(m, SpatialTransformer)]
            ws, bs, offs, o = [], [], {}, 0
            for st in sts:
                a2 = st.transformer_blocks[0].attn2
                wo, wv = a2.to_out[0].weight.detach().double(), a2.to_v.weight.detach().double()
                ws.append((wo @ wv).float())
                bs.append(a2.to_out[0].bias.detach().float())
                offs[st] = (o, o + st.in_channels)
                o += st.in_channels
            self._xattn = (torch.cat(ws, 0).contiguous(), torch.cat(bs, 0).contiguous(), offs, o)
        w, bias, offs, total = self._xattn
        out = ctx.ws.get("xattn.vec", (ctx.context.shape[0], total))
        ctx.gemv_rows(w, bias, ctx.context, out)
        ctx.xattn_vec = {st: out[:, lo:hi] for st, (lo, hi) in offs.items()}

    def run(self, ctx, x_in, t_sin, S):
        B = ctx.B
        self.time_biases(ctx, t_sin)
        self.cross_attn_vectors(ctx)
        hs = []
        H = W = S
        h = x_in
        rec = self._record
        for bi, blk in enumerate(self.input_blocks):
            if rec is not None:
                rec.append((blk, h.clone(), H, W, 0))
            if bi == 0:
                o = ctx.ws.get("hs0", (B * H * W, self.model_channels))
                ctx.next_gn = gn_hint(self.input_blocks[1][0])
                h = blk[0].run(ctx, h, H, W, o)
                ctx.next_gn = None
            else:
                last = blk[-1]
                Ho, Wo = (H // 2, W // 2) if isinstance(last, Downsample) else (H, W)
                co = last.out_channels if isinstance(last, (ResBlock, Downsample)) else last.in_channels
                o = ctx.ws.get(f"hs{bi}", (B * Ho * Wo, co))
                nxt = self.input_blocks[bi + 1][0] if bi + 1 < len(self.input_blocks) else self.middle_block[0]
                h, H, W = blk.run(ctx, h, H, W, out=o, next_layer=nxt)
            hs.append((h, H, W))
        if rec is not None:
            rec.append((self.middle_block, h.clone(), H, W, 0))
        keep = rec is not None or ctx.keep_fp32

        def cat_hint(nblk, co, Hn, Wn):
            first = nblk[0]
            if keep or not isinstance(first, ResBlock) or isinstance(first.skip_connection, nn.Identity):
                return None
            nsk = hs[-1][0]
            Mn = B * Hn * Wn
            return (nsk, ctx.ws.get("cat", (Mn, co + nsk.shape[-1])), ctx.ws.planes("catp", Mn, co + nsk.shape[-1])) + gn_hint(first)

        def out_geometry(blk, H, W):
            last = blk[-1]
            co = last.out_channels if isinstance(last, (ResBlock, Upsample)) else last.in_channels
            return (co, 2 * H, 2 * W) if isinstance(last, Upsample) else (co, H, W)

        h, H, W = self.middle_block.run(ctx, h, H, W, next_cat=cat_hint(self.output_blocks[0], *out_geometry(self.middle_block, H, W)))
        for bi, blk in enumerate(self.output_blocks):
            sk, _, _ = hs.pop()
            M = B * H * W
            ca, cb = h.shape[-1], sk.shape[-1]
            cat = ctx.ws.get("cat", (M, ca + cb))
            catp = ctx.ws.planes("catp", M, ca + cb)
            first = blk[0]
            if cat.data_ptr() in ctx._cat_done:
                ctx._cat_done.discard(cat.data_ptr())
            else:
                need_cat = keep or not isinstance(first, ResBlock) or isinstance(first.skip_connection, nn.Identity)
                ctx.concat(h, ca, sk, cb, cat, catp, B, H * W, gn_apply=gn_hint(first), need_out=need_cat)
            if rec is not None:
                rec.append((blk, cat.clone(), H, W, ca))
            last_blk = bi + 1 == len(self.output_blocks)
            h, H, W = blk.run(ctx, cat, H, W, x_planes=catp, next_layer=(self.out[0], "res.a", True) if last_blk else None,
                              next_cat=None if last_blk else cat_hint(self.output_blocks[bi + 1], *out_geometry(blk, H, W)))
        if self._head is None:
            self._head = hip.pack_conv3x3(self.out[2].weight, self.out[2].bias)
        M = B * H * W
        a = ctx.ws.planes("res.a", M, self.model_channels)
        ctx.groupnorm(h, a, self.out[0], B, H * W, self.model_channels, silu=True)
        y = ctx.ws.get("head", (M, 8))
        ctx.gemm(a, self._head, y, conv=dict(B=B, Hin=H, Win=W, Cin=self.model_channels, Hout=H, Wout=W, stride=1,
                                             upsample=0), ldo=8, kind="conv")
        self._head_saved = (h, a)
        return y


class UNetWrapper(nn.Module):

    def __init__(self, unet_config, unet_path=None, drop_conditions=False, drop_scheme="default", use_zero_123=False,
                 finetune_unet=False, finetune_cross_attn=False, finetune_view_attn=True, remove_keys=()):
        super().__init__()
        params = unet_config.get("params", unet_config) if hasattr(unet_config, "get") else unet_config
        self.unet_model = UNetModel(**dict(params))
        if unet_path:
            from .load_model import load_unet_checkpoint
            load_unet_checkpoint(self.unet_model, unet_path, remove_keys=remove_keys)
        if not finetune_unet:
            self.unet_model.disable_unet_grad()
        self.drop_conditions, self.drop_scheme, self.use_zero_123 = drop_conditions, drop_scheme, use_zero_123
        self.finetune_unet, self.finetune_cross_attn, self.finetune_view_attn = \
            finetune_unet, finetune_cross_attn, finetune_view_attn

    def get_trainable_parameters(self):
        if self.finetune_unet:
            return self.unet_model.parameters()
        return self.unet_model.get_cross_attn_parameters(finetune_cross_attn=self.finetune_cross_attn,
                                                         finetune_view_attn=self.finetune_view_attn)

    def level_channels(self):
        u = self.unet_model
        return [u.model_channels * m for m in u.channel_mult]

    def level0_operand(self, ctx, B, S, D):
        rows = B * S * S * D
        if D == 1:
            c0 = self.level_channels()[0]
            return ctx.ws.get("ovol0", (rows, 2 * (c0 + 768)), torch.int16, zero=True), c0
        return ctx.ws.get("vol0", (rows, 2 * 768), torch.int16, zero=True), 0

    def volume_pyramid(self, ctx, vol, B, S, D):
        levels = [self.level0_operand(ctx, B, S, D)]
        Cc = vol.shape[-1]
        chans = self.level_channels()
        for i in range(1, len(self.unet_model.channel_mult)):
            f = 2 ** i
            rows = B * (S // f) * (S // f) * D
            if D == 1:
                ld, col = chans[i] + Cc, chans[i]
                o = ctx.ws.get(f"ovol{i}", (rows, 2 * ld), torch.int16, zero=True)
            else:
                ld, col = Cc, 0
                o = ctx.ws.planes(f"vol{i}", rows, Cc)
            hip.check(hip.lib().mvd_area_pool(hip.ptr(vol), hip.c_void_p(o.data_ptr() + 4 * col), B, S, D, Cc, f, ld, hip.stream()))
            levels.append((o, col))
        return levels
```

mvdfusion_amd/view_attn_efficient2.py:

```python
import torch
import torch.nn as nn

from . import hip
from .cameras import pack_cameras


_G4_VEC_BLOCK, _G4_VEC_MISC = 3328, 3 * 3328


def window_size(keep_top_k_views, top_k):
    return 2 * (int(top_k) // 2) + 1 if keep_top_k_views else 0


def window_view_table(V, top_k):
    half = int(top_k) // 2
    return (torch.arange(-half, half + 1)[:, None] + torch.arange(int(V))[None, :]) % int(V)


_MT_INDEX = {}


def _microtile_index(dev):
    t = _MT_INDEX.get(str(dev))
    if t is None:
# ... 104 lines not shown
        if self._p is None:
            self._p = (hip.pack_linear(self.attn.qkv.weight, self.attn.qkv.bias),
                       hip.pack_linear(self.attn.proj.weight, self.attn.proj.bias),
                       hip.pack_linear(self.mlp.fc1.weight, self.mlp.fc1.bias),
                       hip.pack_linear(self.mlp.fc2.weight, self.mlp.fc2.bias))
        return self._p

    def run(self, ctx, h, h_alt, c, T, V):
        C = self.hidden_size
        wqkv, wproj, wfc1, wfc2 = self.packed()
        lin = self.adaLN_modulation[1]
        mod = ctx.ws.get("ga.mod", (1, 6 * C))
        hip.gemv(lin.weight, lin.bias, c, mod, act_in=hip.ACT_SILU)
        sh1, sc1, g1, sh2, sc2, g2 = (mod[0, i * C:(i + 1) * C] for i in range(6))
        ln = ctx.ws.planes("ga.ln", T, C)
        hip.layernorm(h, ln, sc1, sh1, T, C, eps=1e-6, w_plus_one=True)
        qkv = ctx.ws.get("ga.qkv", (T, 3 * C))
        ctx.gemm(ln, wqkv, qkv, kind="ga")
        att = ctx.ws.planes("ga.att", T, C)
        hip.check(hip.lib().mvd_view_mha(hip.ptr(qkv), hip.ptr(att), T // V, V, self.num_heads, C // self.num_heads,
                                         hip.stream()))
        ctx.gemm(att, wproj, h_alt, res=h, colscale=g1, kind="ga")
        hip.layernorm(h_alt, ln, sc2, sh2, T, C, eps=1e-6, w_plus_one=True)
        f1 = ctx.ws.planes("ga.f1", T, wfc1.N)
        ctx.gemm(ln, wfc1, None, act=hip.ACT_GELU, out_planes=f1, kind="ga")
        ctx.gemm(f1, wfc2, h, res=h_alt, colscale=g2, kind="ga")
        return h


class AggregationTransformer(nn.Module):
    def __init__(self, hidden_size, num_layers=3, num_heads=8, mlp_ratio=2.0, use_t=False):
        super().__init__()
        if not use_t:
            raise NotImplementedError
        self.use_t = use_t
        self.layer_list = nn.ModuleList([DiTBlock(hidden_size, num_heads=num_heads, mlp_ratio=mlp_ratio)
                                         for _ in range(num_layers)])
        self.weight_layer = nn.Linear(hidden_size, 1)


class _TimestepEmbedder(nn.Module):
    def __init__(self, hidden_size, frequency_embedding_size=256):
        super().__init__()
        self.mlp = nn.Sequential(nn.Linear(frequency_embedding_size, hidden_size, bias=True), nn.SiLU(),
                                 nn.Linear(hidden_size, hidden_size, bias=True))


class GridAttn(nn.Module):
    def __init__(self, input_size=32, in_channels=4, hidden_size=256, output_dim=768, num_heads=8, mlp_ratio=2.0,
                 num_layers=3, side_length=32, world_scale=0.6, z_near_far_scale=0.8, depth_scale=2.0,
                 depth_shift=0.5, n_pts_per_ray=3, use_t=True, keep_top_k_views=False, top_k=4, device="cpu"):
        super().__init__()
        self.keep_top_k_views, self.top_k = bool(keep_top_k_views), int(top_k)
        assert not self.keep_top_k_views or 1 <= self.window <= 16, f"top_k={top_k}: the window {self.window} exceeds 16 rows per 3-D point"
        assert hidden_size == 256, "the token kernel is specialised for 256-channel feature maps"
        assert in_channels == 5, "mvd_zembed reads 4 VAE + 1 depth latent channels (configs/*.yaml: in_channels: 5)"
        self.input_size, self.hidden_size, self.output_dim = input_size, hidden_size, output_dim
        self.depth_scale, self.depth_shift, self.n_pts_per_ray = depth_scale, depth_shift, n_pts_per_ray
        self.z_near_far_scale = z_near_far_scale
        self.z_embedder = nn.Sequential(nn.Linear(in_channels, 256), nn.GELU())
        self.t_embedder = _TimestepEmbedder(hidden_size)
        self.use_t = use_t
        self.pre_layer_b = nn.Sequential(nn.Linear(256 * 2 + 90 * 2 + 15 * 2 + 1, hidden_size), nn.GELU())
        self.aggregation_transformer = AggregationTransformer(hidden_size, num_layers, num_heads, mlp_ratio, use_t)
        self.final_layer_b = nn.Linear(hidden_size, output_dim)
        for blk in self.aggregation_transformer.layer_list:
            nn.init.constant_(blk.adaLN_modulation[-1].weight, 0)
            nn.init.constant_(blk.adaLN_modulation[-1].bias, 0)
        self._p = None
        self._fused = None

    def packed(self):
        if self._p is None:
            self._p = (hip.pack_linear(self.pre_layer_b[0].weight, self.pre_layer_b[0].bias),
                       hip.pack_linear(self.final_layer_b.weight, self.final_layer_b.bias))
        return self._p

    def packed_fused(self, device):
        if self._fused is None:
            stream, vecs = pack_fused_stream(self, bf16=hip.OPERAND_FORMAT == "bf16")
            self._fused = (stream.to(device), vecs.to(device))
        return self._fused

    @property
    def window(self):
        return window_size(self.keep_top_k_views, self.top_k)

    def rows_per_point(self, V):
        return self.window or int(V)

    def fused_supported(self, V, T):
        blocks = self.aggregation_transformer.layer_list
        R = self.rows_per_point(V)
        Vp = 1 << max(R - 1, 0).bit_length()
        return (V >= 1 and 1 <= R <= 16 and (T // R * Vp) % 64 == 0 and T % R == 0 and self.hidden_size == 256 and len(blocks) == 3 and
                all(b.num_heads == 8 and b.mlp.fc1.out_features == 512 for b in blocks))

    def run(self, ctx, x, depth_noise, steps, it, cams_rec, in_cam_rec, input_latents, c, vol_out, V, S, D, q0=0, Vq=None,
            vol_planes=None, vol_planes_col=0, fused=None, depth_src=None, depth_steps=None, scenes=1, steps_scene_stride=0):
        Vq = V if Vq is None else Vq
        N = int(scenes)
        L = hip.lib()
        assert x.shape[1] == 5, "depth wise efficient attention requires 4+1 channels"
        assert N == 1 or (N > 1 and x.shape[0] == N * V and input_latents.shape[0] == N and q0 == 0 and Vq == V), \
            (N, V, q0, Vq, tuple(x.shape), tuple(input_latents.shape))
        w_pre, w_fin = self.packed()
        z = self.z_embedder[0]
        feat = ctx.ws.get("ga.feat", (N * V, S, S, 256))
        in_feat = ctx.ws.get("ga.infeat", (N, S, S, 256))
        hip.check(L.mvd_zembed(hip.ptr(x), hip.ptr(z.weight), hip.ptr(z.bias), hip.ptr(feat), N * V, S, hip.stream()))
        hip.check(L.mvd_zembed(hip.ptr(input_latents), hip.ptr(z.weight), hip.ptr(z.bias), hip.ptr(in_feat), N, S,
                               hip.stream()))
        nseq = N * Vq * S * S * D
        W = self.window
        R = self.rows_per_point(V)
        T = nseq * R
        dsrc = x if depth_src is None else depth_src
        dsteps = steps if depth_steps is None else depth_steps
        assert (depth_src is None) == (depth_steps is None) and dsrc.shape == x.shape
        grid_lin = ctx.ws.bufs.get(("ga.lin", S))
        if grid_lin is None:
            half = 1.0 / float(S)
            grid_lin = torch.linspace(1.0 - half, -1.0 + half, S, dtype=torch.float32).to(ctx.device)
            ctx.ws.bufs[("ga.lin", S)] = grid_lin
        if fused is None:
            fused = self.fused_supported(V, T // N)
        sst = int(steps_scene_stride)
        if sst:
            assert N > 1 and c.shape[0] == N, (N, tuple(c.shape))
            if fused is False or not self.fused_supported(V, T // N):
                raise NotImplementedError(f"GridAttn.run: per-scene timesteps need the fused aggregation kernel (V={V}, T={T // N} per scene); "
                                          "the unfused chain shares one adaLN modulation")
            fused = True
        if fused:
            assert self.fused_supported(V, T // N), (V, T // N)
            stream, vecs = self.packed_fused(ctx.device)
            nv = vecs.numel()
            vecs = vecs.view(1, nv)
            if sst:
                vecs = ctx.ws.get("ga.vecs_scenes", (N, nv)).copy_(vecs.expand(N, nv))
            for bi, blk in enumerate(self.aggregation_transformer.layer_list):
                lin = blk.adaLN_modulation[1]
                ctx.gemv_rows(lin.weight, lin.bias, c, vecs[:, bi * _G4_VEC_BLOCK:bi * _G4_VEC_BLOCK + 1536], act_in=hip.ACT_SILU)
            pool = ctx.ws.planes("ga.pool", nseq, self.hidden_size)
            hip.check(L.mvd_gridattn_fused_window(hip.ptr(dsrc), hip.ptr(depth_noise), hip.ptr(dsteps), hip.ptr(it), hip.ptr(grid_lin),
                                                  hip.ptr(feat), hip.ptr(in_feat), hip.ptr(cams_rec), hip.ptr(in_cam_rec), hip.ptr(stream),
                                                  hip.ptr(vecs), hip.ptr(pool), N, V, q0, Vq, S, D, float(self.depth_scale),
                                                  float(self.depth_shift), 3 if ctx.prec_of("ga") == 3 else 4, sst, sst * nv, W, hip.stream()))
            ctx.gemm(pool, w_fin, vol_out, M=nseq, out_planes=vol_planes, out_planes_col=vol_planes_col, kind="ga")
            return vol_out
        tokens = ctx.ws.planes("ga.tokens", T, hip.TOKEN_LD)
        hip.check(L.mvd_gridattn_tokens_window(hip.ptr(dsrc), hip.ptr(depth_noise), hip.ptr(dsteps), hip.ptr(it), hip.ptr(grid_lin),
                                               hip.ptr(feat), hip.ptr(in_feat), hip.ptr(cams_rec), hip.ptr(in_cam_rec),
                                               hip.ptr(tokens), N, V, q0, Vq, S, D, float(self.depth_scale), float(self.depth_shift),
                                               0, W, hip.stream()))
        h = ctx.ws.get("ga.h", (T, self.hidden_size))
        h_alt = ctx.ws.get("ga.h_alt", (T, self.hidden_size))
        ctx.gemm(tokens, w_pre, h, act=hip.ACT_GELU, kind="ga")
        for blk in self.aggregation_transformer.layer_list:
            h = blk.run(ctx, h, h_alt, c, T, R)
        wl = self.aggregation_transformer.weight_layer
        pool = ctx.ws.planes("ga.pool", nseq, self.hidden_size)
        hip.check(L.mvd_view_pool(hip.ptr(h), hip.ptr(wl.weight), hip.ptr(wl.bias), hip.ptr(pool), nseq, R, self.hidden_size,
                                  hip.stream()))
        ctx.gemm(pool, w_fin, vol_out, M=nseq, out_planes=vol_planes, out_planes_col=vol_planes_col, kind="ga")
        return vol_out
```

mvdfusion_amd/viewfusion_zero_depth_rgb.py:

```python
import math

import torch
import torch.nn as nn

from . import hip
from .cameras import Cameras, get_camera_slice, get_relative_camera, pack_cameras
from .engine import Ctx, ddim_step_table
from .sampler import DDIMSampler
from .scheduler import DDPMScheduler
from .unet import UNetWrapper
from .view_attn_efficient2 import GridAttn

import os

PREFETCH_WEIGHTS = os.environ.get("MVD_PREFETCH", "ws")
PREFETCH_OPTIONS = {k: int(v) for k, v in (kv.split("=") for kv in os.environ.get("MVD_PREFETCH_OPTS", "").split(",") if kv)}


def _sinusoid_freqs(dim, max_period=10000):
    half = dim // 2
    return torch.exp(-math.log(max_period) * torch.arange(start=0, end=half, dtype=torch.float32) / half)


class StepEngine:

    def __init__(self, model, V, S, D, cfg, device, prec, q0=0, Vq=None, policy=None, scenes=1):
        self.m, self.V, self.S, self.D, self.cfg = model, V, S, D, bool(cfg)
        self.q0, self.Vq = q0, (V if Vq is None else Vq)
        self.N = N = int(scenes)
        if N < 1 or (N > 1 and (self.q0 != 0 or self.Vq != V)):
            raise ValueError(f"StepEngine(scenes={scenes}, q0={q0}, Vq={Vq}, V={V}): view-parallel sharding is single-scene only")
        NV = N * V
        self.ctx = Ctx(device, prec, policy)
        dev = self.ctx.device
        B = 2 * N * self.Vq if cfg else N * self.Vq
        self.B = B
        z = lambda *s: torch.zeros(*s, dtype=torch.float32, device=dev)
        self.x = z(NV, 5, S, S)
        self.x0 = z(NV, 5, S, S)
        self.eps = z(NV, 5, S, S)
        self.input_latents = z(N, 5, S, S)
        self.clip_v_embed = z(NV, 796)
        self.cams = z(NV, hip.CAM_RECORD)
        self.in_cam = z(N, hip.CAM_RECORD)
        self.context = z(B, 768)
        self.vol = z(B * S * S * D, 768)
        self.vol_planes, self.vol_col = model.unet_model.level0_operand(self.ctx, B, S, D)
        self.x_in = torch.zeros(B * S * S, 2 * 32, dtype=torch.int16, device=dev)
        self.iter = torch.zeros(1, dtype=torch.int32, device=dev)
        self.steps = z(1, hip.STEP_STRIDE)
        self.steps_nodiv = z(1, hip.STEP_STRIDE)
        self.prev = z(NV, 5, S, S)
        self.depth_mode = 0
        self.pin = None
        self.known = z(1, 5, S, S)
        self.pin_noise = None
        self.depth_noise = z(1, NV, D, S, S)
        self.ddim_noise = z(1, NV, 5, S, S)
        self.f256 = _sinusoid_freqs(256).to(dev)
        self.funet = _sinusoid_freqs(model.unet_model.unet_model.model_channels).to(dev)
        self.graphs = {}
        self.prefetchers = {}
        self.drop_masks = None
        self.n_rows = 1
        self.steps_scene_stride = 0
        self.done = 0

    def set_conditioning(self, batch_cameras, input_latents, input_cameras, clip_v_embed):
        self.set_conditioning_scenes([(batch_cameras, input_latents, input_cameras, clip_v_embed)])

    def set_conditioning_scenes(self, conds):
        if len(conds) != self.N:
            raise ValueError(f"set_conditioning_scenes: {len(conds)} scenes for a {self.N}-scene engine")
        V, S = self.V, self.S
        for n, (bc, il, ic, ce) in enumerate(conds):
            self.cams[n * V:(n + 1) * V].copy_(pack_cameras(bc).to(self.cams.device))
            self.in_cam[n:n + 1].copy_(pack_cameras(ic).to(self.cams.device))
            self.input_latents[n:n + 1].copy_(il.reshape(1, 5, S, S))
            self.clip_v_embed[n * V:(n + 1) * V].copy_(ce.reshape(V, 796))

    def set_schedule(self, steps_table, depth_noise, ddim_noise):
        self._set_tables(steps_table, depth_noise, ddim_noise, scene_stride=0)

    def set_schedule_scenes(self, steps_table, depth_noise, ddim_noise=None):
        if self.cfg:
            raise ValueError("StepEngine.set_schedule_scenes: per-scene timesteps need a cfg=False engine (the training step); "
                             "guided sampling steps share one timestep")
        if tuple(steps_table.shape) != (self.N, hip.STEP_STRIDE):
            raise ValueError(f"StepEngine.set_schedule_scenes: step table {tuple(steps_table.shape)} for {self.N} scenes "
                             f"(expected ({self.N}, {hip.STEP_STRIDE}))")
        if ddim_noise is None:
            ddim_noise = torch.zeros(1, self.N * self.V, 5, self.S, self.S)
        self._set_tables(steps_table, depth_noise, ddim_noise, scene_stride=1 if self.N > 1 else 0)

    def _set_tables(self, steps_table, depth_noise, ddim_noise, scene_stride):
        dev = self.ctx.device
        if self.steps.shape != steps_table.shape:
            self.graphs.clear()
            self.prefetchers.clear()
            self.steps = steps_table.to(dev).contiguous()
            self.steps_nodiv = self.steps.clone()
            self.depth_noise = depth_noise.to(dev).contiguous()
            self.ddim_noise = ddim_noise.to(dev).contiguous()
        else:
            self.steps.copy_(steps_table)
            self.depth_noise.copy_(depth_noise)
            self.ddim_noise.copy_(ddim_noise)
        self.steps_nodiv.copy_(self.steps)
        self.steps_nodiv[:, 1] = 1.0
        self.steps_scene_stride = scene_stride
        self.n_rows = int(steps_table.shape[0]) - (self.N - 1) * scene_stride
        self.rewind()

    def set_pin(self, mode, known, noise=None):
        dev = self.ctx.device
        nk = int(known.shape[0])
        K = nk // self.N
        if mode not in (0, 1) or K < 1 or K * self.N != nk or K > self.V or tuple(known.shape[1:]) != (5, self.S, self.S):
            raise ValueError(f"StepEngine.set_pin: mode {mode}, known {tuple(known.shape)} for {self.N} scene(s) of {self.V} views at "
                             f"S = {self.S} (expected (N*K, 5, S, S), 1 <= K <= V)")
        if mode == 1 and (noise is None or tuple(noise.shape) != (int(self.steps.shape[0]), nk, 5, self.S, self.S)):
            raise ValueError(f"StepEngine.set_pin: mode 1 needs noise ({int(self.steps.shape[0])}, {nk}, 5, {self.S}, {self.S}), got "
                             f"{None if noise is None else tuple(noise.shape)}")
        if self.known.shape != known.shape:
            self.graphs.clear()
            self.prefetchers.clear()
            self.known = known.to(dev, torch.float32).contiguous().clone()
        else:
            self.known.copy_(known)
        if mode == 1:
            if self.pin_noise is None or self.pin_noise.shape != noise.shape:
                self.graphs.clear()
                self.prefetchers.clear()
                self.pin_noise = noise.to(dev, torch.float32).contiguous().clone()
            else:
                self.pin_noise.copy_(noise)
        self.pin = (int(mode), K)

    def clear_pin(self):
        self.pin = None

    def rewind(self, it=0):
        assert 0 <= it < self.n_rows
        self.iter.fill_(it)
        self.done = it

    def depth_geo(self):
        if self.depth_mode == 0:
            return self.x, self.steps
        return (self.x0 if self.depth_mode == 1 else self.prev), self.steps_nodiv

    def enqueue(self, cfg_scale, do_update, prefetcher=None):
        m, ctx, L = self.m, self.ctx, hip.lib()
        V, S, D, B, q0, Vq, N = self.V, self.S, self.D, self.B, self.q0, self.Vq, self.N
        NVq = N * Vq
        ctx.B, ctx.D = B, D
        ctx.begin_step()
        st = hip.stream
        sst, R = self.steps_scene_stride, self.t_rows
        if sst and do_update:
            raise ValueError("StepEngine: per-scene timesteps (set_schedule_scenes) are a training step: no DDIM update")
        if self.pin is not None:
            mode, K = self.pin
            pn = self.pin_noise if mode == 1 else None
            hip.check(L.mvd_pin_views(hip.ptr(self.x), hip.ptr(self.x0), hip.ptr(self.known), hip.ptr(pn), N * K * 5 * S * S,
                                      hip.ptr(self.steps), hip.ptr(self.iter), N, V, K, S, mode, st()))
        ts = ctx.ws.get("vf.tsin", (R, 256))
        te1 = ctx.ws.get("vf.te1", (R, 256))
        c = ctx.ws.get("vf.c", (R, 256))
        hip.check(L.mvd_timestep_embedding_scenes(hip.ptr(self.steps), hip.ptr(self.iter), hip.ptr(self.f256), hip.ptr(ts), 256, R, sst,
                                                  st()))
        ctx.gemv_rows(m.time_embed[0].weight, m.time_embed[0].bias, ts, te1, act_out=hip.ACT_SILU)
        ctx.gemv_rows(m.time_embed[2].weight, m.time_embed[2].bias, te1, c)
        dsrc, dsteps = self.depth_geo()
        m.view_attn.run(ctx, self.x, self.depth_noise, self.steps, self.iter, self.cams, self.in_cam,
                        self.input_latents, c, self.vol, V, S, D, q0=q0, Vq=Vq, vol_planes=self.vol_planes,
                        vol_planes_col=self.vol_col, depth_src=None if self.depth_mode == 0 else dsrc,
                        depth_steps=None if self.depth_mode == 0 else dsteps, scenes=N, steps_scene_stride=sst)
        p = m.cc_projection
        c1 = ctx.ws.get("vf.cc1", (NVq, 768))
        c2 = ctx.ws.get("vf.cc2", (NVq, 768))
        ctx.gemv_rows(p[0].weight, p[0].bias, self.clip_v_embed[q0:q0 + NVq], c1, act_out=hip.ACT_SILU)
        ctx.gemv_rows(p[2].weight, p[2].bias, c1, c2, act_out=hip.ACT_SILU)
        ctx.gemv_rows(p[4].weight, p[4].bias, c2, self.context[:NVq])
        if self.drop_masks is not None:
            clip_m, vol_m, cat_m = self.drop_masks
            self.context[:NVq] *= clip_m[:, None]
            self.vol.view(B, -1)[:NVq] *= vol_m[:, None]
            vp = self.vol_planes.view(B, S * S * D, -1)
            vp[:NVq, :, 2 * self.vol_col:] *= vol_m.to(torch.int16)[:, None, None]
        ctx.context = self.context
        xq, x0q, epsq = self.x[q0:q0 + NVq], self.x0[q0:q0 + NVq], self.eps[q0:q0 + NVq]
        hip.check(L.mvd_unet_input_scenes(hip.ptr(xq), hip.ptr(self.input_latents), hip.ptr(self.x_in), N, Vq, S, 32,
                                          int(self.cfg), st()))
        if self.drop_masks is not None:
            xin = self.x_in.view(B, S * S, 64)
            cm = self.drop_masks[2].to(torch.int16)[:, None, None]
            xin[:NVq, :, 5:10] *= cm
            xin[:NVq, :, 37:42] *= cm
        unet = m.unet_model.unet_model
        ctx.vol_levels = m.unet_model.volume_pyramid(ctx, self.vol.view(B, S, S, D, 768), B, S, D)
        tsu = ctx.ws.get("vf.tsin_unet", (R, unet.model_channels))
        hip.check(L.mvd_timestep_embedding_scenes(hip.ptr(self.steps), hip.ptr(self.iter), hip.ptr(self.funet), hip.ptr(tsu),
                                                  unet.model_channels, R, sst, st()))
        y = unet.run(ctx, self.x_in, tsu, S)
        hip.check(L.mvd_cfg_ddim_update(hip.ptr(y), 8, hip.ptr(xq), hip.ptr(x0q), hip.ptr(epsq),
                                        hip.ptr(self.ddim_noise[:, q0:q0 + NVq]), N * V * 5 * S * S, hip.ptr(self.steps),
                                        hip.ptr(self.iter), NVq, S, int(self.cfg), float(cfg_scale), int(do_update), st()))
        if do_update:
            hip.check(L.mvd_advance_iter(hip.ptr(self.iter), st()))

    @property
    def t_rows(self):
        return self.N if self.steps_scene_stride else 1

    def step(self, cfg_scale, do_update, use_graph=True):
        key = (float(cfg_scale), bool(do_update), int(self.depth_mode), self.steps_scene_stride, self.pin)
        if self.done >= self.n_rows:
            raise IndexError(f"StepEngine.step: iteration {self.done} is past the {self.n_rows}-row step table "
                             "(set_schedule() / rewind() before stepping again)")
        if do_update:
            self.done += 1
        if not use_graph:
            return self.enqueue(cfg_scale, do_update)
        g = self.graphs.get(key)
        if g is None:
            it0 = self.iter.clone()
            x_keep, x0_keep = self.x.clone(), self.x0.clone()
            hip.AUTOTUNE = True
            try:
                self.enqueue(cfg_scale, do_update)
            finally:
                hip.AUTOTUNE = False
                hip.release_tuning_buffers()
            torch.cuda.synchronize()
            pf = None
            if PREFETCH_WEIGHTS == "ws":
                pf = hip.WeightPrefetcher(self.x.device, **PREFETCH_OPTIONS)
                self.iter.copy_(it0)
                self.x.copy_(x_keep)
                self.x0.copy_(x0_keep)
                with pf.following(record=True):
                    self.enqueue(cfg_scale, do_update)
                torch.cuda.synchronize()
            self.iter.copy_(it0)
            self.x.copy_(x_keep)
            self.x0.copy_(x0_keep)
            g = hip.Graph()
            self.ctx.ws.frozen = True
            try:
                with g:
                    if pf is None:
                        self.enqueue(cfg_scale, do_update)
                    else:
                        with pf.following():
                            self.enqueue(cfg_scale, do_update, prefetcher=pf)
            finally:
                self.ctx.ws.frozen = False
            self.graphs[key] = g
            self.prefetchers[key] = pf
        g.launch()


class _HipTrainingLoss(torch.autograd.Function):

    @staticmethod
    def forward(ctx, model, batch, trainer_config, names, *params):
        loss, grads = model.gradients(batch, trainer_config, noise_source=getattr(model, "_noise_source", None), only_trainable=True)
        ctx.grads = [grads.get(n) for n in names]
        ctx.shapes = [p.shape for p in params]
        return loss.clone()

    @staticmethod
    def backward(ctx, grad_out):
        if getattr(ctx, "_scaled", False):
            raise RuntimeError("_HipTrainingLoss.backward ran twice on one node: the step's gradient buffers were already scaled in place "
                               "(call model(batch, cfg) again instead of retain_graph=True)")
        ctx._scaled = True
        live, seen, spans = [], set(), []
        for g in ctx.grads:
            if g is None:
                continue
            key = (g.untyped_storage().data_ptr(), g.storage_offset(), tuple(g.shape), tuple(g.stride()))
            if key in seen:
                continue
            seen.add(key)
            live.append(g)
            spans.append((g.data_ptr(), g.data_ptr() + g.numel() * g.element_size()) if g.is_contiguous() else None)
        disjoint = all(sp is not None for sp in spans)
        if disjoint:
            srt = sorted(spans)
            disjoint = all(srt[i][1] <= srt[i + 1][0] for i in range(len(srt) - 1))
        if live and disjoint:
            torch._foreach_mul_(live, grad_out.to(live[0].dtype))
            pick = lambda g: g
        else:
            pick = lambda g: g * grad_out.to(g.dtype)
        outs = [torch.zeros(s, dtype=grad_out.dtype, device=grad_out.device) if g is None else pick(g).reshape(s)
                for g, s in zip(ctx.grads, ctx.shapes)]
        return (None, None, None, None, *outs)


class ViewFusion(nn.Module):
    def __init__(self, view_attn_config, unet_config, ddpm_config, vae_config=None, unet_path="", vae_path="",
                 clip_path="", unet_cc_path="", z_scale_factor=0.18215, vae_max_batch=8, objective="noise",
                 loss_type="l2", embed_camera_pose=True, finetune_projection=False, finetune_unet=False,
                 finetune_cross_attn=True, finetune_view_attn=True, feed_prev_depth=False, drop_conditions=False,
                 vae=None, clip_image_encoder=None, precision=None, reference_eval_dropout=False, overwrite_x_noisy=False, **kwargs):
        super().__init__()
        assert embed_camera_pose, "this build implements the embed_camera_pose=True configuration of configs/*.yaml"
        self.finetune_projection, self.finetune_unet, self.z_scale_factor = finetune_projection, finetune_unet, z_scale_factor
        self.vae_max_batch, self.objective, self.loss_type = vae_max_batch, objective, loss_type
        self.embed_camera_pose, self.finetune_cross_attn, self.finetune_view_attn = \
            embed_camera_pose, finetune_cross_attn, finetune_view_attn
        self.feed_prev_depth, self.drop_conditions = feed_prev_depth, drop_conditions
        self.reference_eval_dropout = bool(reference_eval_dropout)
        from .configs import DEFAULT_PRECISION
        precision = precision or DEFAULT_PRECISION
        fmt, self.precision, self.precision_policy = hip.parse_precision(precision)
        hip.set_operand_format(fmt)
        self.precision_name = precision

        def params(cfg):
            return dict(cfg.get("params", cfg)) if hasattr(cfg, "get") else dict(cfg)

        self.view_attn = GridAttn(**params(view_attn_config))
        self.unet_model = UNetWrapper(unet_config, unet_path=unet_path or None, drop_conditions=drop_conditions,
                                      drop_scheme="default", finetune_unet=finetune_unet,
                                      finetune_cross_attn=finetune_cross_attn, finetune_view_attn=finetune_view_attn,
                                      use_zero_123=True,
                                      remove_keys=["input_blocks.0.0.weight", "out.2.weight", "out.2.bias"])
        self.scheduler = DDPMScheduler(**params(ddpm_config))
        if vae is not None:
            self.vae = vae
        elif vae_config is not None:
            from .load_model import instantiate_from_config
            self.vae = instantiate_from_config(vae_config)
            if vae_path:
                sd = torch.load(vae_path, map_location="cpu")
                sd = sd.get("state_dict", sd)
                self.vae.load_state_dict({k.replace("first_stage_model.", ""): v for k, v in sd.items()}, strict=False)
        if clip_image_encoder is not None:
            self.clip_image_encoder = clip_image_encoder
        elif clip_path:
            from .encoders import FrozenCLIPImageEmbedder
            self.clip_image_encoder = FrozenCLIPImageEmbedder(model=clip_path, precision=precision)
            for prm in self.clip_image_encoder.parameters():
                prm.requires_grad_(False)
        self.cc_projection = nn.Sequential(nn.Linear(768 + 14 * 2, 768), nn.SiLU(True), nn.Linear(768, 768),
                                           nn.SiLU(True), nn.Linear(768, 768))
        nn.init.eye_(list(self.cc_projection.parameters())[0][:768, :768])
        nn.init.zeros_(list(self.cc_projection.parameters())[1])
        self.time_embed_dim = 256
        self.time_embed = nn.Sequential(nn.Linear(256, 256), nn.SiLU(True), nn.Linear(256, 256))
        self.register_buffer("_device", torch.tensor([0.0]), persistent=False)
        self.latent_size = int(self.view_attn.input_size)
        self.ddim = DDIMSampler(self, ddim_num_steps=50, ddim_discretize="uniform", ddim_eta=1.0,
                                latent_size=self.latent_size, z_dim=4, feed_prev_depth=feed_prev_depth,
                                overwrite_x_noisy=overwrite_x_noisy)
        self._engines = {}
        self._packed_sig = None
        assert self.finetune_view_attn is True, "must finetune new view attention layers"

    train_autotune_min_flops = 2.0e9

    def invalidate_packed(self, keep_engines=False):
        hip.drop_packed_caches(self)
        hip.forget_param_maxima()
        if keep_engines:
            for e in self._engines.values():
                e.graphs.clear()
                e.prefetchers.clear()
        else:
            self._engines.clear()

    def load_state_dict(self, state_dict, strict=True, **kw):
        r = super().load_state_dict(state_dict, strict=strict, **kw)
        self.invalidate_packed()
        self._packed_sig = None
        return r

    def _apply(self, fn, *a, **kw):
        r = super()._apply(fn, *a, **kw)
        if "_engines" in self.__dict__:
            self.invalidate_packed()
            self._packed_sig = None
        return r

    def engine(self, V, S, D, cfg, q0=0, Vq=None, scenes=1):
        if int(scenes) < 1:
            raise ValueError(f"engine(scenes={scenes}): at least one scene")
        if int(scenes) > 1 and (q0 != 0 or (Vq is not None and Vq != V)):
            raise ValueError(f"engine(V={V}, q0={q0}, Vq={Vq}, scenes={scenes}): view-parallel sharding is single-scene only")
        sig = hip.params_signature(self)
        if sig != self._packed_sig:
            if self._packed_sig is not None:
                dev_now = self._device.device
                same_dev = all(e.ctx.device == dev_now for e in self._engines.values())
                self.invalidate_packed(keep_engines=same_dev)
            self._packed_sig = sig
            hip.register_param_maxima(self.parameters())
        if Vq is not None and Vq <= 0:
            raise ValueError(f"engine(V={V}, q0={q0}, Vq={Vq}): a rank must own at least one query view")
        key = (V, S, D, bool(cfg), q0, Vq) if int(scenes) == 1 else (V, S, D, bool(cfg), q0, Vq, int(scenes))
        e = self._engines.get(key)
        if e is None:
            dev = self._device.device
            if dev.type != "cuda":
                raise RuntimeError("mvdfusion_amd.ViewFusion runs on the GPU only (model.cuda() first); "
                                   "there is no CPU path in the product")
            e = StepEngine(self, V, S, D, cfg, dev, self.precision, q0=q0, Vq=Vq, policy=self.precision_policy, scenes=int(scenes))
            self._engines[key] = e
        return e

    def _print_parameter_count(self):
        va = sum(p.numel() for p in self.view_attn.parameters())
        un = sum(p.numel() for p in self.unet_model.get_trainable_parameters())
        uf = sum(p.numel() for p in self.unet_model.parameters())
        tp = sum(p.numel() for p in self.time_embed.parameters())
        pp = sum(p.numel() for p in self.cc_projection.parameters()) if self.finetune_projection else 0
        print(f"view_attn {va * 1e-6:.2f}M | unet trainable {un * 1e-6:.2f}M / full {uf * 1e-6:.2f}M | "
              f"total trainable {(va + un + tp + pp) * 1e-6:.2f}M / full {(va + uf + tp + pp) * 1e-6:.2f}M")

    @torch.no_grad()
    def encode_clip(self, x):
        return self.clip_image_encoder.encode(x)

    @torch.no_grad()
    def encode(self, x):
        return self.vae.encode(torch.clip(x * 2 - 1.0, -1.0, 1.0)).mode() * self.z_scale_factor

    @torch.no_grad()
    def decode(self, z):
        return torch.clip((self.vae.decode(z * 1 / self.z_scale_factor) + 1.0) / 2.0, 0.0, 1.0).clip(0.0, 1.0)

    def prepare_batch(self, batch, trainer_config, generator=None):
        images = batch["images"]
        dev = images.device
        Bn, _, H, W = images.shape
        n_in, n_tr = trainer_config["input_batch_size"], trainer_config["train_batch_size"]
        if trainer_config["random_views"]:
            rand = torch.randperm(Bn, generator=generator) if generator is not None else torch.randperm(Bn)
        else:
            rand = torch.linspace(0, Bn - 1, n_in + n_tr).long()
        in_idx, b_idx = rand[:n_in], rand[n_in:n_in + n_tr]
        input_latents = self.encode(images[in_idx])
        batch_latents = self.encode(images[b_idx])
        area = lambda d: torch.nn.functional.interpolate(d, scale_factor=0.125, mode="area")
        in_depth = torch.zeros_like(area(torch.zeros((n_in, 1, H, W), device=dev)))
        input_latents = torch.cat((input_latents, in_depth), dim=1)
        if "depths" in batch:
            b_depth = torch.clip(batch["depths"][b_idx].to(dev) * 2 - 1.0, -1.0, 1.0)
        else:
            b_depth = torch.zeros((n_tr, 1, H, W), device=dev)
        batch_latents = torch.cat((batch_latents, area(b_depth)), dim=1)
# ... 303 lines not shown
```

Before: 123.9 steps/s.

## Precompute per-step conditioning tables and fuse step prologue kernels into one launch

Precomputes the timestep-dependent conditioning for every DDIM row: time embeddings, time-bias tables, adaLN modulations and the CLIP camera projection. At each step a single prologue kernel gathers the current row, zeroes the GN arena, computes the z-embedding and builds the UNet input, replacing several small launches and gemvs. It also adds a fused multi-level area-pool pyramid kernel and lets GEMMs write split-precision planes for the next consumer directly. This cuts per-step launch and small-kernel overhead, at the cost of table memory and extra invalidation logic when weights change.

```diff
diff --git a/include/mvd_hip.h b/include/mvd_hip.h
--- a/include/mvd_hip.h
+++ b/include/mvd_hip.h
@@ -157,6 +157,19 @@
                          const float* beta, long long* gn_stats, int B, int hw, int groups, float eps, int silu, mvd_stream_t stream);
 int mvd_area_pool(const float* vol, void* out_sp, int B, int S, int D, int C, int factor, int ldp, mvd_stream_t stream);
 int mvd_fill_zero(float* p, size_t n, mvd_stream_t stream);
+#define MVD_PYRAMID_MAX_LEVELS 4
+int mvd_area_pool_pyramid(const float* vol, void* const* out_sp, const int* ldp, const int* factors, int nlev, int B, int S, int D, int C,
+                          mvd_stream_t stream);
+#define MVD_PROLOGUE_MAX_GATHERS 16
+typedef struct mvd_row_gather {
+  const float* src;
+  float* dst;
+  long long len;
+  long long stride;
+} mvd_row_gather;
+int mvd_step_prologue(float* zero_p, size_t zero_n, const mvd_row_gather* gathers, int n_gather, size_t gather_total, const int* iter,
+                      const float* z_lat, const float* z_w, const float* z_b, float* z_feat, int z_n, const float* u_x, const float* u_il,
+                      void* u_out_sp, int nscene, int V, int cpad, int cfg, int S, mvd_stream_t stream);
 
 #define MVD_STEP_STRIDE 8
 int mvd_timestep_embedding(const float* steps, const int* iter, const float* freqs, float* out, int dim,
diff --git a/mvdfusion_amd/csrc/elementwise.hip b/mvdfusion_amd/csrc/elementwise.hip
--- a/mvdfusion_amd/csrc/elementwise.hip
+++ b/mvdfusion_amd/csrc/elementwise.hip
@@ -1,4 +1,5 @@
 #include "common.hpp"
+#include "gridattn_common.hpp"
 #include "../../include/mvd_hip.h"
 
 namespace {
@@ -57,11 +58,11 @@
   }
 }
 
-__global__ __launch_bounds__(256) void unet_input_kernel(const float* __restrict__ x, const float* __restrict__ il,
-                                                         u16* __restrict__ out_sp, int V, int Vs, int S, int cpad, int nb) {
+__device__ __forceinline__ void unet_input_range(const float* __restrict__ x, const float* __restrict__ il, u16* __restrict__ out_sp, int V,
+                                                 int Vs, int S, int cpad, int nb, int blk, int nblk) {
   const int SS = S * S;
   const size_t total = (size_t)nb * SS * cpad;
-  for (size_t e = (size_t)blockIdx.x * 256 + threadIdx.x; e < total; e += (size_t)gridDim.x * 256) {
+  for (size_t e = (size_t)blk * 256 + threadIdx.x; e < total; e += (size_t)nblk * 256) {
     const int c = (int)(e % cpad);
     const int pix = (int)((e / cpad) % SS);
     const int b = (int)(e / ((size_t)cpad * SS));
@@ -75,6 +76,11 @@
     }
     store_sp1(out_sp, e / cpad, cpad, c, o);
   }
+}
+
+__global__ __launch_bounds__(256) void unet_input_kernel(const float* __restrict__ x, const float* __restrict__ il,
+                                                         u16* __restrict__ out_sp, int V, int Vs, int S, int cpad, int nb) {
+  unet_input_range(x, il, out_sp, V, Vs, S, cpad, nb, blockIdx.x, gridDim.x);
 }
 
 __global__ __launch_bounds__(256) void concat_kernel(const float4* __restrict__ a, int ca4, const float4* __restrict__ b, int cb4,
@@ -268,12 +274,12 @@
   }
 }
 
-__global__ __launch_bounds__(256) void area_pool_kernel(const float4* __restrict__ vol, u16* __restrict__ out_sp, int B, int S,
-                                                        int D, int C4, int f, int ldp) {
+__device__ __forceinline__ void area_pool_range(const float4* __restrict__ vol, u16* __restrict__ out_sp, int B, int S, int D, int C4, int f,
+                                                int ldp, int blk, int nblk) {
   const int So = S / f;
   const size_t total = (size_t)B * So * So * D * C4;
   const float inv = 1.0f / (float)(f * f);
-  for (size_t e = (size_t)blockIdx.x * 256 + threadIdx.x; e < total; e += (size_t)gridDim.x * 256) {
+  for (size_t e = (size_t)blk * 256 + threadIdx.x; e < total; e += (size_t)nblk * 256) {
     const int c = (int)(e % C4);
     size_t r = e / C4;
     const int d = (int)(r % D);
@@ -296,8 +302,76 @@
   }
 }
 
-__global__ __launch_bounds__(256) void fill_zero_kernel(float* p, size_t n) {
-  for (size_t e = (size_t)blockIdx.x * 256 + threadIdx.x; e < n; e += (size_t)gridDim.x * 256) p[e] = 0.f;
+__global__ __launch_bounds__(256) void area_pool_kernel(const float4* __restrict__ vol, u16* __restrict__ out_sp, int B, int S,
+                                                        int D, int C4, int f, int ldp) {
+  area_pool_range(vol, out_sp, B, S, D, C4, f, ldp, blockIdx.x, gridDim.x);
+}
+
+struct PyramidArgs {
+  u16* out[MVD_PYRAMID_MAX_LEVELS];
+  int ldp[MVD_PYRAMID_MAX_LEVELS];
+  int f[MVD_PYRAMID_MAX_LEVELS];
+  int blk0[MVD_PYRAMID_MAX_LEVELS + 1];
+  int nlev;
+};
+
+__global__ __launch_bounds__(256) void area_pool_pyramid_kernel(const float4* __restrict__ vol, PyramidArgs a, int B, int S, int D, int C4) {
+  const int blk = blockIdx.x;
+#pragma unroll
+  for (int l = 0; l < MVD_PYRAMID_MAX_LEVELS; ++l)
+    if (l < a.nlev && blk >= a.blk0[l] && blk < a.blk0[l + 1])
+      area_pool_range(vol, a.out[l], B, S, D, C4, a.f[l], a.ldp[l], blk - a.blk0[l], a.blk0[l + 1] - a.blk0[l]);
+}
+
+__device__ __forceinline__ void fill_zero_range(float* p, size_t n, int blk, int nblk) {
+  for (size_t e = (size_t)blk * 256 + threadIdx.x; e < n; e += (size_t)nblk * 256) p[e] = 0.f;
+}
+
+__global__ __launch_bounds__(256) void fill_zero_kernel(float* p, size_t n) { fill_zero_range(p, n, blockIdx.x, gridDim.x); }
+
+struct PrologueArgs {
+  float* zero_p;
+  size_t zero_n;
+  const mvd_row_gather* gathers;
+  int n_gather;
+  size_t gather_total;
+  const int* iter;
+  const float* z_lat;
+  const float* z_w;
+  const float* z_b;
+  float* z_feat;
+  int z_n;
+  const float* u_x;
+  const float* u_il;
+  u16* u_out;
+  int u_V, u_Vs, u_cpad, u_nb;
+  int S;
+  int b_zero, b_gather, b_zembed, b_input;
+};
+
+__global__ __launch_bounds__(256) void step_prologue_kernel(PrologueArgs a) {
+  const int blk = blockIdx.x;
+  if (blk < a.b_zero) {
+    fill_zero_range(a.zero_p, a.zero_n, blk, a.b_zero);
+  } else if (blk < a.b_gather) {
+    const size_t row = (size_t)a.iter[0];
+    const int nblk = a.b_gather - a.b_zero;
+    for (size_t e = (size_t)(blk - a.b_zero) * 256 + threadIdx.x; e < a.gather_total; e += (size_t)nblk * 256) {
+      size_t off = e;
+      for (int j = 0; j < a.n_gather; ++j) {
+        const size_t len = (size_t)a.gathers[j].len;
+        if (off < len) {
+          a.gathers[j].dst[off] = a.gathers[j].src[row * (size_t)a.gathers[j].stride + off];
+          break;
+        }
+        off -= len;
+      }
+    }
+  } else if (blk < a.b_zembed) {
+    zembed_wave(a.z_lat, a.z_w, a.z_b, a.z_feat, a.z_n, a.S * a.S, (size_t)(blk - a.b_gather) * 4 + (threadIdx.x >> 6), threadIdx.x & 63);
+  } else if (blk < a.b_input) {
+    unet_input_range(a.u_x, a.u_il, a.u_out, a.u_V, a.u_Vs, a.S, a.u_cpad, a.u_nb, blk - a.b_zembed, a.b_input - a.b_zembed);
+  }
 }
 
 __global__ void timestep_embedding_kernel(const float* __restrict__ steps, const int* __restrict__ iter,
@@ -497,6 +571,85 @@
   if (n == 0) return 0;
   hipLaunchKernelGGL(fill_zero_kernel, dim3(grid_for(n)), dim3(256), 0, (hipStream_t)stream, p, n);
   MVD_CHECK_LAUNCH("mvd_fill_zero");
+  return 0;
+}
+
+extern "C" int mvd_area_pool_pyramid(const float* vol, void* const* out_sp, const int* ldp, const int* factors, int nlev, int B, int S,
+                                     int D, int C, mvd_stream_t stream) {
+  MVD_CHECK_ARG(vol && out_sp && ldp && factors && nlev >= 1 && nlev <= MVD_PYRAMID_MAX_LEVELS,
+                "mvd_area_pool_pyramid: null pointer or nlev=%d outside 1 ... %d", nlev, MVD_PYRAMID_MAX_LEVELS);
+  MVD_CHECK_ARG(C % 32 == 0 && B > 0 && S > 0 && D > 0, "mvd_area_pool_pyramid: bad shape");
+  PyramidArgs a = {};
+  a.nlev = nlev;
+  a.blk0[0] = 0;
+  for (int l = 0; l < nlev; ++l) {
+    const int f = factors[l], ld = ldp[l] == 0 ? C : ldp[l];
+    MVD_CHECK_ARG(f >= 1 && S % f == 0, "mvd_area_pool_pyramid: level %d: factor %d does not divide S=%d", l, f, S);
+    MVD_CHECK_ARG(out_sp[l] && ld >= C && ld % 32 == 0 && ((uintptr_t)out_sp[l] & 127) == 0,
+                  "mvd_area_pool_pyramid: level %d: ldp=%d must be >= C, %% 32 == 0, out_sp 128-byte aligned", l, ld);
+    const int So = S / f;
+    a.out[l] = (u16*)out_sp[l];
+    a.ldp[l] = ld;
+    a.f[l] = f;
+    a.blk0[l + 1] = a.blk0[l] + grid_for((size_t)B * So * So * D * (C / 4));
+  }
+  hipLaunchKernelGGL(area_pool_pyramid_kernel, dim3(a.blk0[nlev]), dim3(256), 0, (hipStream_t)stream, (const float4*)vol, a, B, S, D, C / 4);
+  MVD_CHECK_LAUNCH("mvd_area_pool_pyramid");
+  return 0;
+}
+
+extern "C" int mvd_step_prologue(float* zero_p, size_t zero_n, const mvd_row_gather* gathers, int n_gather, size_t gather_total,
+                                 const int* iter, const float* z_lat, const float* z_w, const float* z_b, float* z_feat, int z_n,
+                                 const float* u_x, const float* u_il, void* u_out_sp, int nscene, int V, int cpad, int cfg, int S,
+                                 mvd_stream_t stream) {
+  MVD_CHECK_ARG(S > 0, "mvd_step_prologue: S=%d", S);
+  PrologueArgs a = {};
+  a.S = S;
+  int nb = 0;
+  if (zero_p && zero_n) {
+    a.zero_p = zero_p;
+    a.zero_n = zero_n;
+    nb += grid_for(zero_n);
+  }
+  a.b_zero = nb;
+  if (n_gather > 0) {
+    MVD_CHECK_ARG(gathers && iter && gather_total > 0 && n_gather <= MVD_PROLOGUE_MAX_GATHERS,
+                  "mvd_step_prologue: %d gather records need the records, iter and their total length (at most %d records)", n_gather,
+                  MVD_PROLOGUE_MAX_GATHERS);
+    a.gathers = gathers;
+    a.n_gather = n_gather;
+    a.gather_total = gather_total;
+    a.iter = iter;
+    nb += grid_for(gather_total);
+  }
+  a.b_gather = nb;
+  if (z_lat) {
+    MVD_CHECK_ARG(z_w && z_b && z_feat && z_n > 0, "mvd_step_prologue: z-embedding needs w, b, feat and z_n > 0");
+    a.z_lat = z_lat;
+    a.z_w = z_w;
+    a.z_b = z_b;
+    a.z_feat = z_feat;
+    a.z_n = z_n;
+    nb += cdiv((size_t)z_n * S * S, 4);
+  }
+  a.b_zembed = nb;
+  if (u_x) {
+    MVD_CHECK_ARG(u_il && u_out_sp && cpad % 32 == 0 && cpad >= 10 && V > 0 && nscene >= 1 && (long long)nscene * V <= 0x3fffffff,
+                  "mvd_step_prologue: UNet input needs input_latents, out_sp, cpad %% 32 == 0, V > 0, nscene >= 1");
+    const int NV = nscene * V;
+    a.u_x = u_x;
+    a.u_il = u_il;
+    a.u_out = (u16*)u_out_sp;
+    a.u_V = NV;
+    a.u_Vs = V;
+    a.u_cpad = cpad;
+    a.u_nb = cfg ? 2 * NV : NV;
+    nb += grid_for((size_t)a.u_nb * S * S * cpad);
+  }
+  a.b_input = nb;
+  if (nb == 0) return 0;
+  hipLaunchKernelGGL(step_prologue_kernel, dim3(nb), dim3(256), 0, (hipStream_t)stream, a);
+  MVD_CHECK_LAUNCH("mvd_step_prologue");
   return 0;
 }
 
diff --git a/mvdfusion_amd/csrc/gemm.hip b/mvdfusion_amd/csrc/gemm.hip
--- a/mvdfusion_amd/csrc/gemm.hip
+++ b/mvdfusion_amd/csrc/gemm.hip
@@ -244,6 +244,13 @@
             uint32_t hh, ll;
             split_op16x2(v.x, v.y, hh, ll);
             u16* pp = (u16*)d.cat_raw_sp + sp_index((size_t)m, CT, n);
+            *(uint32_t*)pp = hh;
+            *(uint32_t*)(pp + 32) = ll;
+          }
+          if (d.out_sp) {
+            uint32_t hh, ll;
+            split_op16x2(v.x, v.y, hh, ll);
+            u16* pp = (u16*)d.out_sp + sp_index((size_t)m, d.ldp, n);
             *(uint32_t*)pp = hh;
             *(uint32_t*)(pp + 32) = ll;
           }
@@ -553,7 +560,7 @@
   const int gna_ct = d.N + (d.cat_b ? d.cat_cb : 0);
   const int gna_cg = d.gna_out_sp ? gna_ct / d.gn_groups : 0;
   const size_t gna_lds = (size_t)d.gn_hw * gna_cg * 4;
-  const bool gna_fused = d.gna_out_sp && p.splits > 1 && !d.rs_out && !d.out_sp && !d.colscale && d.act == MVD_ACT_NONE && (gna_cg & 1) == 0 &&
+  const bool gna_fused = d.gna_out_sp && p.splits > 1 && !d.rs_out && !(d.out_sp && d.cat_b) && !d.colscale && d.act == MVD_ACT_NONE && (gna_cg & 1) == 0 &&
                          gna_cg <= 128 && gna_lds <= 128 * 1024 && d.ldo % 2 == 0 && (!d.res || d.ldr % 2 == 0) && (!d.bias_b || d.ldbb % 2 == 0) &&
                          d.N % 2 == 0;
   if (gna_fused) {
diff --git a/mvdfusion_amd/csrc/gridattn.hip b/mvdfusion_amd/csrc/gridattn.hip
--- a/mvdfusion_amd/csrc/gridattn.hip
+++ b/mvdfusion_amd/csrc/gridattn.hip
@@ -50,23 +50,7 @@
 
 __global__ __launch_bounds__(256) void zembed_kernel(const float* __restrict__ lat, const float* __restrict__ w,
                                                      const float* __restrict__ bias, float* __restrict__ feat, int N, int SS) {
-  const int lane = threadIdx.x & 63;
-  const size_t p = (size_t)blockIdx.x * 4 + (threadIdx.x >> 6);
-  if (p >= (size_t)N * SS) return;
-  const int n = (int)(p / SS), pix = (int)(p % SS);
-  float in[5];
-#pragma unroll
-  for (int c = 0; c < 5; ++c) in[c] = lat[((size_t)n * 5 + c) * SS + pix];
-  float o[4];
-#pragma unroll
-  for (int j = 0; j < 4; ++j) {
-    const int ch = lane * 4 + j;
-    float a = 0.f;
-#pragma unroll
-    for (int c = 0; c < 5; ++c) a += in[c] * w[ch * 5 + c];
-    o[j] = gelu_erf(a + bias[ch]);
-  }
-  *(float4*)(feat + p * 256 + lane * 4) = make_float4(o[0], o[1], o[2], o[3]);
+  zembed_wave(lat, w, bias, feat, N, SS, (size_t)blockIdx.x * 4 + (threadIdx.x >> 6), threadIdx.x & 63);
 }
 
 __device__ __forceinline__ void scatter4(long long* __restrict__ acc, const Taps& t, int ch, float4 g, float scale) {
diff --git a/mvdfusion_amd/csrc/gridattn_common.hpp b/mvdfusion_amd/csrc/gridattn_common.hpp
--- a/mvdfusion_amd/csrc/gridattn_common.hpp
+++ b/mvdfusion_amd/csrc/gridattn_common.hpp
@@ -3,6 +3,25 @@
 #include "../../include/mvd_hip.h"
 
 namespace {
+
+__device__ __forceinline__ void zembed_wave(const float* __restrict__ lat, const float* __restrict__ w, const float* __restrict__ bias,
+                                            float* __restrict__ feat, int N, int SS, size_t p, int lane) {
+  if (p >= (size_t)N * SS) return;
+  const int n = (int)(p / SS), pix = (int)(p % SS);
+  float in[5];
+#pragma unroll
+  for (int c = 0; c < 5; ++c) in[c] = lat[((size_t)n * 5 + c) * SS + pix];
+  float o[4];
+#pragma unroll
+  for (int j = 0; j < 4; ++j) {
+    const int ch = lane * 4 + j;
+    float a = 0.f;
+#pragma unroll
+    for (int c = 0; c < 5; ++c) a += in[c] * w[ch * 5 + c];
+    o[j] = gelu_erf(a + bias[ch]);
+  }
+  *(float4*)(feat + p * 256 + lane * 4) = make_float4(o[0], o[1], o[2], o[3]);
+}
 
 struct GridGeom {
   const float *x, *depth_noise, *steps;
diff --git a/mvdfusion_amd/engine.py b/mvdfusion_amd/engine.py
--- a/mvdfusion_amd/engine.py
+++ b/mvdfusion_amd/engine.py
@@ -75,18 +75,27 @@
         self.next_cat = None
         self._cat_done = set()
         self.keep_fp32 = False
-
-    def begin_step(self):
+        self.next_planes = None
+        self._planes_done = {}
+
+    def begin_step(self, zero_arena=True):
         self._rot.clear()
         self._gn.clear()
         self._gn_done.clear()
         self._unwritten.clear()
         self._cat_done.clear()
+        self._planes_done.clear()
         self.next_gn = None
         self.next_cat = None
+        self.next_planes = None
         self._gn_next = 0
-        if self.gn_from_producer:
-            hip.check(hip.lib().mvd_fill_zero(hip.ptr(self.gn_arena), self.gn_arena.numel() * 2, hip.stream()))
+        if self.gn_from_producer and zero_arena:
+            hip.check(hip.lib().mvd_fill_zero(*self.arena_span(), hip.stream()))
+
+    def arena_span(self):
+        if not self.gn_from_producer:
+            return None, 0
+        return hip.ptr(self.gn_arena), self.gn_arena.numel() * 2
 
     def gn_slot(self, out, B, HW, C):
         n = B * 32 * 2
@@ -101,6 +110,7 @@
         ptr = out.data_ptr()
         self._gn.pop(ptr, None)
         self._unwritten.discard(ptr)
+        self._planes_done.pop(ptr, None)
         if self._gn_done:
             for k in [k for k in self._gn_done if k[0] == ptr]:
                 del self._gn_done[k]
@@ -166,6 +176,12 @@
                             planes = self.ws.planes(pname, out.shape[0], out.shape[-1])
                             kw["gn_apply"] = (norm.weight, norm.bias, norm.eps, hip.GNA_SILU if silu else 0, planes)
                             self._gn_done[(out.data_ptr(), id(norm))] = (planes, bool(silu))
+            if gn is not None and gn_apply is None and self.next_planes is not None and not self.keep_fp32 and "out_planes" not in kw and \
+                    "cat" not in kw and out.is_contiguous() and out.shape[-1] == self.next_planes[2] and \
+                    self.next_planes[1] in (None, out.shape[0]):
+                planes = self.ws.planes(self.next_planes[0], out.shape[0], out.shape[-1])
+                kw["out_planes"] = planes
+                self._planes_done[out.data_ptr()] = planes
         if gn is not None:
             if os.environ.get("MVD_GN_DEBUG") and not self.capturing:
                 print(f"[gn] kind={kind} M={out.shape[0]} N={out.shape[-1]} explicit={gn_apply is not None} hint={self.next_gn is not None} "
@@ -173,6 +189,7 @@
             if gn_apply is None:
                 self.next_gn = None
                 self.next_cat = None
+                self.next_planes = None
         r = hip.gemm(A, W, out, **kw)
         if gn_apply is not None and not applied:
             self.groupnorm(out, gn_apply[1], gn_apply[0], gn[0], gn[1], out.shape[-1], gn_apply[2])
@@ -189,6 +206,13 @@
             return hip.groupnorm_from_stats(x, y, norm.weight, norm.bias, ent[0], B, HW, C, norm.eps, silu)
         ws = self.ws.get("gn_ws", (B * hip.lib().mvd_groupnorm_chunks(HW) * 32 * 2,), torch.float64)
         return hip.groupnorm(x, y, norm.weight, norm.bias, B, HW, C, norm.eps, silu, ws)
+
+    def planes_of(self, x, name, rows, cols):
+        done = self._planes_done.pop(x.data_ptr(), None)
+        planes = self.ws.planes(name, rows, cols)
+        if done is not None and done.data_ptr() == planes.data_ptr() and done.shape == planes.shape:
+            return planes
+        return hip.split_planes(x, planes)
 
     def concat(self, a, ca, b, cb, out, out_planes, B, HW, gn_apply=None, need_out=True):
         self._forget(out)
diff --git a/mvdfusion_amd/hip.py b/mvdfusion_amd/hip.py
--- a/mvdfusion_amd/hip.py
+++ b/mvdfusion_amd/hip.py
@@ -36,6 +36,8 @@
 ACT_NONE, ACT_GELU, ACT_SILU, ACT_QUICKGELU = 0, 1, 2, 3
 STEP_STRIDE = 8
 CAM_RECORD = 20
+PYRAMID_MAX_LEVELS = 4
+PROLOGUE_MAX_GATHERS = 16
 TOKEN_DIM, TOKEN_LD = 723, 736
 FUSE_FOREGROUND = 1
 FUSE_STAGE_AUTO, FUSE_STAGE_GLOBAL, FUSE_STAGE_LDS = 0, 1, 2
@@ -120,6 +122,8 @@
     "mvd_groupnorm_from_stats": (_i, [_vp, _vp, _vp, _vp, _vp, _i, _i, _i, _i, _f, _i, _vp]),
     "mvd_area_pool": (_i, [_vp, _vp, _i, _i, _i, _i, _i, _i, _vp]),
     "mvd_fill_zero": (_i, [_vp, _sz, _vp]),
+    "mvd_area_pool_pyramid": (_i, [_vp, _vp, _vp, _vp, _i, _i, _i, _i, _i, _vp]),
+    "mvd_step_prologue": (_i, [_vp, _sz, _vp, _i, _sz, _vp, _vp, _vp, _vp, _vp, _i, _vp, _vp, _vp, _i, _i, _i, _i, _i, _vp]),
     "mvd_pow2_scale": (_i, [_vp, _sz, _vp, _vp, _vp]),
     "mvd_split_planes_scaled": (_i, [_vp, _vp, _sz, _i, _i, _i, _vp, _vp]),
     "mvd_transpose_planes_scaled": (_i, [_vp, _i, _i, _i, _vp, _i, _vp, _vp]),
diff --git a/mvdfusion_amd/unet.py b/mvdfusion_amd/unet.py
--- a/mvdfusion_amd/unet.py
+++ b/mvdfusion_amd/unet.py
@@ -38,7 +38,7 @@
             wp = self._p
         if out is None:
             out = ctx.act((ctx.B * 4 * H * W, self.out_channels))
-        xp = hip.split_planes(x, ctx.ws.planes("updown.x", ctx.B * H * W, self.channels))
+        xp = ctx.planes_of(x, "updown.x", ctx.B * H * W, self.channels)
         ctx.gemm(xp, wp, out, conv=dict(B=ctx.B, Hin=H, Win=W, Cin=self.channels, Hout=2 * H, Wout=2 * W,
                                             stride=1, upsample=1), gn=(ctx.B, 4 * H * W), kind="conv")
         return out, 2 * H, 2 * W
@@ -57,7 +57,7 @@
         Ho, Wo = H // 2, W // 2
         if out is None:
             out = ctx.act((ctx.B * Ho * Wo, self.out_channels))
-        xp = hip.split_planes(x, ctx.ws.planes("updown.x", ctx.B * H * W, self.channels))
+        xp = ctx.planes_of(x, "updown.x", ctx.B * H * W, self.channels)
         ctx.gemm(xp, self._p, out, conv=dict(B=ctx.B, Hin=H, Win=W, Cin=self.channels, Hout=Ho, Wout=Wo, stride=2,
                                             upsample=0), gn=(ctx.B, Ho * Wo), kind="conv")
         return out, Ho, Wo
@@ -104,7 +104,7 @@
                  gn=(B, H * W), kind="conv",
                  gn_apply=(self.out_layers[0], a2, True, True))
         if (wsk is not None or w2.tail_cin) and x_planes is None:
-            x_planes = hip.split_planes(x, ctx.ws.planes("res.xp", M, Ci))
+            x_planes = ctx.planes_of(x, "res.xp", M, Ci)
         if out is None:
             out = ctx.act((M, Co))
         if w2.tail_cin:
@@ -131,6 +131,14 @@
     return None
 
 
+def planes_hint(layer, ctx, H, W):
+    if isinstance(layer, (Upsample, Downsample)):
+        return "updown.x", ctx.B * H * W, layer.channels
+    if isinstance(layer, ResBlock) and not isinstance(layer.skip_connection, nn.Identity):
+        return "res.xp", None, layer.channels
+    return None
+
+
 class TimestepEmbedSequential(nn.Sequential, TimestepBlock):
     def run(self, ctx, x, H, W, out=None, x_planes=None, next_layer=None, next_cat=None):
         n = len(self)
@@ -138,6 +146,7 @@
             dst = out if i == n - 1 else None
             ctx.next_gn = gn_hint(self[i + 1] if i + 1 < n else next_layer)
             ctx.next_cat = next_cat if i == n - 1 else None
+            ctx.next_planes = planes_hint(self[i + 1] if i + 1 < n else next_layer, ctx, H, W)
             if isinstance(layer, (Upsample, Downsample)):
                 x, H, W = layer.run(ctx, x, H, W, out=dst)
             elif isinstance(layer, ResBlock):
@@ -146,6 +155,7 @@
                 x = layer.run(ctx, x, H, W, out=dst)
             ctx.next_gn = None
             ctx.next_cat = None
+            ctx.next_planes = None
         return x, H, W
 
 
@@ -242,7 +252,7 @@
     def _resblocks(self):
         return [m for m in self.modules() if isinstance(m, ResBlock)]
 
-    def time_biases(self, ctx, t_sin):
+    def _temb_packed(self):
         if self._temb is None:
             blocks = self._resblocks()
             w = torch.cat([b.emb_layers[1].weight.detach() for b in blocks], 0).contiguous()
@@ -252,17 +262,30 @@
                 offs[b] = (o, o + b.out_channels)
                 o += b.out_channels
             self._temb = (w, bias, offs)
-        w, bias, offs = self._temb
+        return self._temb
+
+    def time_bias_width(self):
+        return int(self._temb_packed()[0].shape[0])
+
+    def time_biases(self, ctx, t_sin, out=None, bind=True):
+        w, bias, offs = self._temb_packed()
         ted = self.model_channels * 4
         R = t_sin.shape[0]
         e1, emb = ctx.ws.get("temb.e1", (R, ted)), ctx.ws.get("temb.emb", (R, ted))
-        out = ctx.ws.get("temb.bias", (R, w.shape[0]))
+        if out is None:
+            out = ctx.ws.get("temb.bias", (R, w.shape[0]))
         ctx.gemv_rows(self.time_embed[0].weight, self.time_embed[0].bias, t_sin, e1, act_out=hip.ACT_SILU)
         ctx.gemv_rows(self.time_embed[2].weight, self.time_embed[2].bias, e1, emb)
         ctx.gemv_rows(w, bias, emb, out, act_in=hip.ACT_SILU)
+        if bind:
+            self.bind_time_biases(ctx, out)
+        return out
+
+    def bind_time_biases(self, ctx, out):
+        offs = self._temb_packed()[2]
         ctx.emb_bias = {b: out[:, lo:hi] for b, (lo, hi) in offs.items()}
 
-    def cross_attn_vectors(self, ctx):
+    def _xattn_packed(self):
         if self._xattn is None:
             sts = [m for m in self.modules() if isinstance(m, SpatialTransformer)]
             ws, bs, offs, o = [], [], {}, 0
@@ -274,15 +297,23 @@
                 offs[st] = (o, o + st.in_channels)
                 o += st.in_channels
             self._xattn = (torch.cat(ws, 0).contiguous(), torch.cat(bs, 0).contiguous(), offs, o)
-        w, bias, offs, total = self._xattn
+        return self._xattn
+
+    def cross_attn_vectors(self, ctx, compute=True):
+        w, bias, offs, total = self._xattn_packed()
         out = ctx.ws.get("xattn.vec", (ctx.context.shape[0], total))
-        ctx.gemv_rows(w, bias, ctx.context, out)
+        if compute:
+            ctx.gemv_rows(w, bias, ctx.context, out)
         ctx.xattn_vec = {st: out[:, lo:hi] for st, (lo, hi) in offs.items()}
 
-    def run(self, ctx, x_in, t_sin, S):
+    def run(self, ctx, x_in, t_sin, S, *, precomputed=False):
         B = ctx.B
-        self.time_biases(ctx, t_sin)
-        self.cross_attn_vectors(ctx)
+        if precomputed:
+            self.bind_time_biases(ctx, ctx.ws.get("temb.bias", (1, self.time_bias_width())))
+            self.cross_attn_vectors(ctx, compute=False)
+        else:
+            self.time_biases(ctx, t_sin)
+            self.cross_attn_vectors(ctx)
         hs = []
         H = W = S
         h = x_in
@@ -387,6 +418,7 @@
         levels = [self.level0_operand(ctx, B, S, D)]
         Cc = vol.shape[-1]
         chans = self.level_channels()
+        outs, lds, fs = [], [], []
         for i in range(1, len(self.unet_model.channel_mult)):
             f = 2 ** i
             rows = B * (S // f) * (S // f) * D
@@ -396,6 +428,12 @@
             else:
                 ld, col = Cc, 0
                 o = ctx.ws.planes(f"vol{i}", rows, Cc)
-            hip.check(hip.lib().mvd_area_pool(hip.ptr(vol), hip.c_void_p(o.data_ptr() + 4 * col), B, S, D, Cc, f, ld, hip.stream()))
+            outs.append(o.data_ptr() + 4 * col)
+            lds.append(ld)
+            fs.append(f)
             levels.append((o, col))
+        for k in range(0, len(outs), hip.PYRAMID_MAX_LEVELS):
+            n = len(outs[k:k + hip.PYRAMID_MAX_LEVELS])
+            hip.check(hip.lib().mvd_area_pool_pyramid(hip.ptr(vol), (hip.c_void_p * n)(*outs[k:k + n]), (hip.C.c_int * n)(*lds[k:k + n]),
+                                                      (hip.C.c_int * n)(*fs[k:k + n]), n, B, S, D, Cc, hip.stream()))
         return levels
diff --git a/mvdfusion_amd/view_attn_efficient2.py b/mvdfusion_amd/view_attn_efficient2.py
--- a/mvdfusion_amd/view_attn_efficient2.py
+++ b/mvdfusion_amd/view_attn_efficient2.py
@@ -210,6 +210,9 @@
             self._fused = (stream.to(device), vecs.to(device))
         return self._fused
 
+    def adaln_slices(self, vecs):
+        return [vecs.view(-1)[bi * _G4_VEC_BLOCK:bi * _G4_VEC_BLOCK + 1536] for bi in range(len(self.aggregation_transformer.layer_list))]
+
     @property
     def window(self):
         return window_size(self.keep_top_k_views, self.top_k)
@@ -225,7 +228,8 @@
                 all(b.num_heads == 8 and b.mlp.fc1.out_features == 512 for b in blocks))
 
     def run(self, ctx, x, depth_noise, steps, it, cams_rec, in_cam_rec, input_latents, c, vol_out, V, S, D, q0=0, Vq=None,
-            vol_planes=None, vol_planes_col=0, fused=None, depth_src=None, depth_steps=None, scenes=1, steps_scene_stride=0):
+            vol_planes=None, vol_planes_col=0, fused=None, depth_src=None, depth_steps=None, scenes=1, steps_scene_stride=0, *,
+            feat_ready=False, in_feat_ready=False, mod_ready=False):
         Vq = V if Vq is None else Vq
         N = int(scenes)
         L = hip.lib()
@@ -236,9 +240,11 @@
         z = self.z_embedder[0]
         feat = ctx.ws.get("ga.feat", (N * V, S, S, 256))
         in_feat = ctx.ws.get("ga.infeat", (N, S, S, 256))
-        hip.check(L.mvd_zembed(hip.ptr(x), hip.ptr(z.weight), hip.ptr(z.bias), hip.ptr(feat), N * V, S, hip.stream()))
-        hip.check(L.mvd_zembed(hip.ptr(input_latents), hip.ptr(z.weight), hip.ptr(z.bias), hip.ptr(in_feat), N, S,
-                               hip.stream()))
+        if not feat_ready:
+            hip.check(L.mvd_zembed(hip.ptr(x), hip.ptr(z.weight), hip.ptr(z.bias), hip.ptr(feat), N * V, S, hip.stream()))
+        if not in_feat_ready:
+            hip.check(L.mvd_zembed(hip.ptr(input_latents), hip.ptr(z.weight), hip.ptr(z.bias), hip.ptr(in_feat), N, S,
+                                   hip.stream()))
         nseq = N * Vq * S * S * D
         W = self.window
         R = self.rows_per_point(V)
@@ -267,7 +273,8 @@
             vecs = vecs.view(1, nv)
             if sst:
                 vecs = ctx.ws.get("ga.vecs_scenes", (N, nv)).copy_(vecs.expand(N, nv))
-            for bi, blk in enumerate(self.aggregation_transformer.layer_list):
+            assert not (mod_ready and sst), "precomputed adaLN rows are per schedule row: not with per-scene timesteps"
+            for bi, blk in enumerate(() if mod_ready else self.aggregation_transformer.layer_list):
                 lin = blk.adaLN_modulation[1]
                 ctx.gemv_rows(lin.weight, lin.bias, c, vecs[:, bi * _G4_VEC_BLOCK:bi * _G4_VEC_BLOCK + 1536], act_in=hip.ACT_SILU)
             pool = ctx.ws.planes("ga.pool", nseq, self.hidden_size)
diff --git a/mvdfusion_amd/viewfusion_zero_depth_rgb.py b/mvdfusion_amd/viewfusion_zero_depth_rgb.py
--- a/mvdfusion_amd/viewfusion_zero_depth_rgb.py
+++ b/mvdfusion_amd/viewfusion_zero_depth_rgb.py
@@ -15,6 +15,10 @@
 
 PREFETCH_WEIGHTS = os.environ.get("MVD_PREFETCH", "ws")
 PREFETCH_OPTIONS = {k: int(v) for k, v in (kv.split("=") for kv in os.environ.get("MVD_PREFETCH_OPTS", "").split(",") if kv)}
+
+
+def step_tables_enabled():
+    return os.environ.get("MVD_STEP_TABLES", "1") != "0"
 
 
 def _sinusoid_freqs(dim, max_period=10000):
@@ -65,6 +69,16 @@
         self.n_rows = 1
         self.steps_scene_stride = 0
         self.done = 0
+        self._iter0 = torch.zeros(1, dtype=torch.int32, device=dev)
+        self._t_col = (0.0,)
+        self._tab = None
+        self._tab_key = None
+        self._cond_ok = False
+        self._gather = torch.zeros(hip.PROLOGUE_MAX_GATHERS, 4, dtype=torch.int64, device=dev)
+        self._gather_host = None
+        self.table_builds = 0
+        self._fused_flag = None
+        self._n_gather = (0, 0)
 
     def set_conditioning(self, batch_cameras, input_latents, input_cameras, clip_v_embed):
         self.set_conditioning_scenes([(batch_cameras, input_latents, input_cameras, clip_v_embed)])
@@ -78,6 +92,9 @@
             self.in_cam[n:n + 1].copy_(pack_cameras(ic).to(self.cams.device))
             self.input_latents[n:n + 1].copy_(il.reshape(1, 5, S, S))
             self.clip_v_embed[n * V:(n + 1) * V].copy_(ce.reshape(V, 796))
+        self._cond_ok = False
+        if self._table_graph_exists():
+            self._build_conditioning()
 
     def set_schedule(self, steps_table, depth_noise, ddim_noise):
         self._set_tables(steps_table, depth_noise, ddim_noise, scene_stride=0)
@@ -98,6 +115,7 @@
         if self.steps.shape != steps_table.shape:
             self.graphs.clear()
             self.prefetchers.clear()
+            self._tab = self._tab_key = None
             self.steps = steps_table.to(dev).contiguous()
             self.steps_nodiv = self.steps.clone()
             self.depth_noise = depth_noise.to(dev).contiguous()
@@ -110,7 +128,10 @@
         self.steps_nodiv[:, 1] = 1.0
         self.steps_scene_stride = scene_stride
         self.n_rows = int(steps_table.shape[0]) - (self.N - 1) * scene_stride
+        self._t_col = tuple(float(t) for t in steps_table[:, 0].tolist())
         self.rewind()
+        if self._table_graph_exists():
+            self._build_tables()
 
     def set_pin(self, mode, known, noise=None):
         dev = self.ctx.device
@@ -140,6 +161,84 @@
     def clear_pin(self):
         self.pin = None
 
+    def tables_wanted(self):
+        return step_tables_enabled() and self.steps_scene_stride == 0 and self.drop_masks is None and not self.ctx.keep_fp32
+
+    def _table_graph_exists(self):
+        return self.tables_wanted() and any(k[-1] for k in self.graphs)
+
+    def drop_derived(self):
+        self.graphs.clear()
+        self.prefetchers.clear()
+        self._cond_ok = False
+        self._tab_key = None
+
+    def _gridattn_fused(self):
+        if self._fused_flag is None:
+            va = self.m.view_attn
+            self._fused_flag = bool(va.fused_supported(self.V, self.Vq * self.S * self.S * self.D * va.rows_per_point(self.V)))
+        return self._fused_flag
+
+    def _derived_current(self):
+        return self._cond_ok and self._tab is not None and self._tab_key == (self._t_col, self._gridattn_fused())
+
+    def _build_conditioning(self):
+        m, ctx, L = self.m, self.ctx, hip.lib()
+        N, S, q0, NVq = self.N, self.S, self.q0, self.N * self.Vq
+        p = m.cc_projection
+        c1 = ctx.ws.get("vf.cc1", (NVq, 768))
+        c2 = ctx.ws.get("vf.cc2", (NVq, 768))
+        ctx.gemv_rows(p[0].weight, p[0].bias, self.clip_v_embed[q0:q0 + NVq], c1, act_out=hip.ACT_SILU)
+        ctx.gemv_rows(p[2].weight, p[2].bias, c1, c2, act_out=hip.ACT_SILU)
+        ctx.gemv_rows(p[4].weight, p[4].bias, c2, self.context[:NVq])
+        ctx.context = self.context
+        m.unet_model.unet_model.cross_attn_vectors(ctx)
+        z = m.view_attn.z_embedder[0]
+        in_feat = ctx.ws.get("ga.infeat", (N, S, S, 256))
+        hip.check(L.mvd_zembed(hip.ptr(self.input_latents), hip.ptr(z.weight), hip.ptr(z.bias), hip.ptr(in_feat), N, S, hip.stream()))
+        self._cond_ok = True
+
+    def _build_tables(self):
+        m, ctx, L = self.m, self.ctx, hip.lib()
+        fused = self._gridattn_fused()
+        key = (self._t_col, fused)
+        if self._tab is not None and self._tab_key == key:
+            return
+        unet = m.unet_model.unet_model
+        T, dev = int(self.steps.shape[0]), ctx.device
+        if self._tab is None:
+            e = lambda w: torch.empty(T, w, dtype=torch.float32, device=dev)
+            self._tab = dict(ts=e(256), te1=e(256), c=e(256), tsu=e(unet.model_channels), temb=e(unet.time_bias_width()),
+                             mod=[e(1536) for _ in m.view_attn.aggregation_transformer.layer_list])
+        tab = self._tab
+        for freqs, out, dim in ((self.f256, tab["ts"], 256), (self.funet, tab["tsu"], unet.model_channels)):
+            hip.check(L.mvd_timestep_embedding_scenes(hip.ptr(self.steps), hip.ptr(self._iter0), hip.ptr(freqs), hip.ptr(out), dim, T,
+                                                      1 if T > 1 else 0, hip.stream()))
+        ctx.gemv_rows(m.time_embed[0].weight, m.time_embed[0].bias, tab["ts"], tab["te1"], act_out=hip.ACT_SILU)
+        ctx.gemv_rows(m.time_embed[2].weight, m.time_embed[2].bias, tab["te1"], tab["c"])
+        if fused:
+            for blk, mod in zip(m.view_attn.aggregation_transformer.layer_list, tab["mod"]):
+                lin = blk.adaLN_modulation[1]
+                ctx.gemv_rows(lin.weight, lin.bias, tab["c"], mod, act_in=hip.ACT_SILU)
+        unet.time_biases(ctx, tab["tsu"], out=tab["temb"], bind=False)
+        self._tab_key = key
+        self.table_builds += 1
+
+    def _prepare_derived(self):
+        if not self._cond_ok:
+            self._build_conditioning()
+        self._build_tables()
+        m, ctx, tab = self.m, self.ctx, self._tab
+        recs = [(tab["c"], ctx.ws.get("vf.c", (1, 256))),
+                (tab["temb"], ctx.ws.get("temb.bias", (1, tab["temb"].shape[1])))]
+        if self._tab_key[1]:
+            recs += list(zip(tab["mod"], m.view_attn.adaln_slices(m.view_attn.packed_fused(ctx.device)[1])))
+        host = [[src.data_ptr(), dst.data_ptr(), src.shape[1], src.stride(0)] for src, dst in recs]
+        if host != self._gather_host:
+            self._gather[:len(host)].copy_(torch.tensor(host, dtype=torch.int64))
+            self._gather_host = host
+        return len(host), sum(h[2] for h in host)
+
     def rewind(self, it=0):
         assert 0 <= it < self.n_rows
         self.iter.fill_(it)
@@ -155,7 +254,8 @@
         V, S, D, B, q0, Vq, N = self.V, self.S, self.D, self.B, self.q0, self.Vq, self.N
         NVq = N * Vq
         ctx.B, ctx.D = B, D
-        ctx.begin_step()
+        tab = self.tables_wanted()
+        ctx.begin_step(zero_arena=not tab)
         st = hip.stream
         sst, R = self.steps_scene_stride, self.t_rows
         if sst and do_update:
@@ -165,24 +265,37 @@
             pn = self.pin_noise if mode == 1 else None
             hip.check(L.mvd_pin_views(hip.ptr(self.x), hip.ptr(self.x0), hip.ptr(self.known), hip.ptr(pn), N * K * 5 * S * S,
                                       hip.ptr(self.steps), hip.ptr(self.iter), N, V, K, S, mode, st()))
-        ts = ctx.ws.get("vf.tsin", (R, 256))
-        te1 = ctx.ws.get("vf.te1", (R, 256))
+        xq, x0q, epsq = self.x[q0:q0 + NVq], self.x0[q0:q0 + NVq], self.eps[q0:q0 + NVq]
         c = ctx.ws.get("vf.c", (R, 256))
-        hip.check(L.mvd_timestep_embedding_scenes(hip.ptr(self.steps), hip.ptr(self.iter), hip.ptr(self.f256), hip.ptr(ts), 256, R, sst,
-                                                  st()))
-        ctx.gemv_rows(m.time_embed[0].weight, m.time_embed[0].bias, ts, te1, act_out=hip.ACT_SILU)
-        ctx.gemv_rows(m.time_embed[2].weight, m.time_embed[2].bias, te1, c)
+        if tab:
+            if not ctx.ws.frozen:
+                self._n_gather = self._prepare_derived()
+            z = m.view_attn.z_embedder[0]
+            feat = ctx.ws.get("ga.feat", (N * V, S, S, 256))
+            hip.check(L.mvd_step_prologue(*ctx.arena_span(), hip.ptr(self._gather), self._n_gather[0], self._n_gather[1], hip.ptr(self.iter),
+                                          hip.ptr(self.x), hip.ptr(z.weight), hip.ptr(z.bias), hip.ptr(feat), N * V, hip.ptr(xq),
+                                          hip.ptr(self.input_latents), hip.ptr(self.x_in), N, Vq, 32, int(self.cfg), S, st()))
+        else:
+            self._cond_ok = False
+            ts = ctx.ws.get("vf.tsin", (R, 256))
+            te1 = ctx.ws.get("vf.te1", (R, 256))
+            hip.check(L.mvd_timestep_embedding_scenes(hip.ptr(self.steps), hip.ptr(self.iter), hip.ptr(self.f256), hip.ptr(ts), 256, R, sst,
+                                                      st()))
+            ctx.gemv_rows(m.time_embed[0].weight, m.time_embed[0].bias, ts, te1, act_out=hip.ACT_SILU)
+            ctx.gemv_rows(m.time_embed[2].weight, m.time_embed[2].bias, te1, c)
         dsrc, dsteps = self.depth_geo()
         m.view_attn.run(ctx, self.x, self.depth_noise, self.steps, self.iter, self.cams, self.in_cam,
                         self.input_latents, c, self.vol, V, S, D, q0=q0, Vq=Vq, vol_planes=self.vol_planes,
                         vol_planes_col=self.vol_col, depth_src=None if self.depth_mode == 0 else dsrc,
-                        depth_steps=None if self.depth_mode == 0 else dsteps, scenes=N, steps_scene_stride=sst)
-        p = m.cc_projection
-        c1 = ctx.ws.get("vf.cc1", (NVq, 768))
-        c2 = ctx.ws.get("vf.cc2", (NVq, 768))
-        ctx.gemv_rows(p[0].weight, p[0].bias, self.clip_v_embed[q0:q0 + NVq], c1, act_out=hip.ACT_SILU)
-        ctx.gemv_rows(p[2].weight, p[2].bias, c1, c2, act_out=hip.ACT_SILU)
-        ctx.gemv_rows(p[4].weight, p[4].bias, c2, self.context[:NVq])
+                        depth_steps=None if self.depth_mode == 0 else dsteps, scenes=N, steps_scene_stride=sst,
+                        feat_ready=tab, in_feat_ready=tab, mod_ready=tab and self._tab_key[1])
+        if not tab:
+            p = m.cc_projection
+            c1 = ctx.ws.get("vf.cc1", (NVq, 768))
+            c2 = ctx.ws.get("vf.cc2", (NVq, 768))
+            ctx.gemv_rows(p[0].weight, p[0].bias, self.clip_v_embed[q0:q0 + NVq], c1, act_out=hip.ACT_SILU)
+            ctx.gemv_rows(p[2].weight, p[2].bias, c1, c2, act_out=hip.ACT_SILU)
+            ctx.gemv_rows(p[4].weight, p[4].bias, c2, self.context[:NVq])
         if self.drop_masks is not None:
             clip_m, vol_m, cat_m = self.drop_masks
             self.context[:NVq] *= clip_m[:, None]
@@ -190,9 +303,9 @@
             vp = self.vol_planes.view(B, S * S * D, -1)
             vp[:NVq, :, 2 * self.vol_col:] *= vol_m.to(torch.int16)[:, None, None]
         ctx.context = self.context
-        xq, x0q, epsq = self.x[q0:q0 + NVq], self.x0[q0:q0 + NVq], self.eps[q0:q0 + NVq]
-        hip.check(L.mvd_unet_input_scenes(hip.ptr(xq), hip.ptr(self.input_latents), hip.ptr(self.x_in), N, Vq, S, 32,
-                                          int(self.cfg), st()))
+        if not tab:
+            hip.check(L.mvd_unet_input_scenes(hip.ptr(xq), hip.ptr(self.input_latents), hip.ptr(self.x_in), N, Vq, S, 32,
+                                              int(self.cfg), st()))
         if self.drop_masks is not None:
             xin = self.x_in.view(B, S * S, 64)
             cm = self.drop_masks[2].to(torch.int16)[:, None, None]
@@ -200,10 +313,12 @@
             xin[:NVq, :, 37:42] *= cm
         unet = m.unet_model.unet_model
         ctx.vol_levels = m.unet_model.volume_pyramid(ctx, self.vol.view(B, S, S, D, 768), B, S, D)
-        tsu = ctx.ws.get("vf.tsin_unet", (R, unet.model_channels))
-        hip.check(L.mvd_timestep_embedding_scenes(hip.ptr(self.steps), hip.ptr(self.iter), hip.ptr(self.funet), hip.ptr(tsu),
-                                                  unet.model_channels, R, sst, st()))
-        y = unet.run(ctx, self.x_in, tsu, S)
+        tsu = None
+        if not tab:
+            tsu = ctx.ws.get("vf.tsin_unet", (R, unet.model_channels))
+            hip.check(L.mvd_timestep_embedding_scenes(hip.ptr(self.steps), hip.ptr(self.iter), hip.ptr(self.funet), hip.ptr(tsu),
+                                                      unet.model_channels, R, sst, st()))
+        y = unet.run(ctx, self.x_in, tsu, S, precomputed=tab)
         hip.check(L.mvd_cfg_ddim_update(hip.ptr(y), 8, hip.ptr(xq), hip.ptr(x0q), hip.ptr(epsq),
                                         hip.ptr(self.ddim_noise[:, q0:q0 + NVq]), N * V * 5 * S * S, hip.ptr(self.steps),
                                         hip.ptr(self.iter), NVq, S, int(self.cfg), float(cfg_scale), int(do_update), st()))
@@ -215,7 +330,7 @@
         return self.N if self.steps_scene_stride else 1
 
     def step(self, cfg_scale, do_update, use_graph=True):
-        key = (float(cfg_scale), bool(do_update), int(self.depth_mode), self.steps_scene_stride, self.pin)
+        key = (float(cfg_scale), bool(do_update), int(self.depth_mode), self.steps_scene_stride, self.pin, self.tables_wanted())
         if self.done >= self.n_rows:
             raise IndexError(f"StepEngine.step: iteration {self.done} is past the {self.n_rows}-row step table "
                              "(set_schedule() / rewind() before stepping again)")
@@ -224,6 +339,8 @@
         if not use_graph:
             return self.enqueue(cfg_scale, do_update)
         g = self.graphs.get(key)
+        if g is not None and key[-1] and not self._derived_current():
+            self._n_gather = self._prepare_derived()
         if g is None:
             it0 = self.iter.clone()
             x_keep, x0_keep = self.x.clone(), self.x0.clone()
@@ -369,8 +486,7 @@
         hip.forget_param_maxima()
         if keep_engines:
             for e in self._engines.values():
-                e.graphs.clear()
-                e.prefetchers.clear()
+                e.drop_derived()
         else:
             self._engines.clear()
 
```

Result: faster. 126.3 steps/s, median of 6 (+2.0%).
